# shg8/3DGS.cpp

Hardware: AMD Instinct MI355X
Metric: frames/sec at 1920×1080, 1M Gaussians (higher is better)
Workload: dtype f32

## Files before the change

3dgs.cpp_amd/binding.py:

```python
import ctypes as C
import os

import numpy as np

_HERE = os.path.dirname(os.path.abspath(__file__))
LIB_PATH = os.environ.get("GS3D_HIP_LIB", os.path.join(_HERE, "libgs3d_hip.so"))

UNIFORMS_DT = np.dtype([("camera_position", "<f4", 4), ("proj_mat", "<f4", 16), ("view_mat", "<f4", 16),
                        ("width", "<u4"), ("height", "<u4"), ("tan_fovx", "<f4"), ("tan_fovy", "<f4")])
CAMERA_DT = np.dtype([("position", "<f4", 3), ("rotation", "<f4", 4), ("fov", "<f4"),
                      ("near_plane", "<f4"), ("far_plane", "<f4")])
VERTEX_FLOATS = 60
RECORD_FLOATS = 62
BLOB_PLANES = 59


KERNEL_SOURCES = ("gs_device.h", "gs_bin.h", "gs_scene.hip", "gs_preprocess.hip", "gs_radix.hip", "gs_bin_l1.hip", "gs_bin_l2.hip",
                  "gs_blend.hip", "gs_contrib.hip", "gs_features.hip", "gs_kernels.h")


def library_source_hash():
    import hashlib
    import re
    h = hashlib.sha256()
    for name in KERNEL_SOURCES + ("Makefile",):
        with open(os.path.join(_HERE, "csrc", name), "r") as f:
            text = f.read()
        if name != "Makefile":
            text = re.sub(r"/\*.*?\*/", " ", text, flags=re.S)
            text = re.sub(r"//[^\n]*", " ", text)
        else:
            text = re.sub(r"#[^\n]*", " ", text)
        h.update(name.encode() + b"\0" + " ".join(text.split()).encode())
    return h.hexdigest()


STAGES = dict(tiles=(0, np.uint32), depth=(1, np.float32), radius=(2, np.float32), aabb=(3, np.uint16),
              conic_opacity=(4, np.float32), uv_rg=(5, np.float32), b=(6, np.float32),
              depth_order=(7, np.uint32), alpha_cut=(8, np.float32), sorted_tile=(11, np.uint32), sorted_gid=(12, np.uint32),
              ranges=(13, np.uint32), lists_raw=(14, np.uint32), ranges_raw=(15, np.uint32))

SYMBOLS = ["gs_last_error", "gs_device_count", "gs_read_ply", "gs_activate_records", "gs_scene_load_ply", "gs_scene_from_records",
           "gs_scene_from_vertices", "gs_scene_from_device_blob", "gs_scene_blob_floats", "gs_scene_blob",
           "gs_scene_from_device_arrays", "gs_scene_update_from_device_arrays", "gs_debug_activation_expf_scan",
           "gs_scene_transform", "gs_transform_sh_matrices", "gs_transform_camera",
           "gs_scene_num_vertices", "gs_scene_quantize_sh", "gs_scene_sh_bits", "gs_scene_download_vertex_range",
           "gs_scene_download_vertices", "gs_scene_download_cov3d",
           "gs_deactivate_vertices", "gs_write_ply", "gs_scene_to_device_arrays", "gs_scene_download_records", "gs_scene_save_ply",
           "gs_scene_destroy", "gs_renderer_create", "gs_renderer_destroy", "gs_camera_uniforms",
           "gs_render", "gs_render_host", "gs_synchronize", "gs_set_timing", "gs_set_frames_in_flight", "gs_set_sort_path", "gs_set_exp_mode", "gs_set_graph_mode", "gs_set_blend_lockstep", "gs_get_blend_lockstep", "gs_set_blend_contraction", "gs_set_antialiased", "gs_get_antialiased", "gs_get_timing_totals",
           "gs_get_frame_intervals", "gs_get_stats", "gs_poll_stats", "gs_debug_download", "gs_accumulate_contributions", "gs_blend_features", "gs_debug_expf_scan", "gs_debug_alpha_cut_scan", "gs_renderer_stream",
           "gs_dist_unique_id", "gs_dist_create", "gs_dist_rank", "gs_dist_world", "gs_dist_pose_count",
           "gs_dist_broadcast_scene", "gs_dist_broadcast_scene_ex", "gs_dist_verify", "gs_dist_destroy"]


class FrameStats(C.Structure):
    _fields_ = [("num_gaussians", C.c_uint64), ("num_visible", C.c_uint64), ("num_instances", C.c_uint64),
                ("instance_capacity", C.c_uint64), ("ms_preprocess", C.c_float), ("ms_prefix_sum", C.c_float),
                ("ms_preprocess_sort", C.c_float), ("ms_sort", C.c_float), ("ms_tile_boundary", C.c_float),
                ("ms_render", C.c_float), ("ms_total", C.c_float), ("retries", C.c_uint32),
                ("num_bin_entries", C.c_uint32), ("max_bin_entries", C.c_uint32), ("sort_path", C.c_uint32),
                ("bin_tiles", C.c_uint32), ("sort_level", C.c_uint32), ("blend_redo", C.c_uint32), ("blend_resolved", C.c_uint32), ("pad_", C.c_uint32)]

    def as_dict(self):
        return {k: getattr(self, k) for k, _ in self._fields_}


def debug_alpha_cut_scan(first_bits, count, device=0):
    bad, first = C.c_uint64(0), C.c_uint32(0)
    _check(lib().gs_debug_alpha_cut_scan(C.c_int(device), C.c_uint32(first_bits), C.c_uint64(count), C.byref(bad), C.byref(first)))
    return int(bad.value), (None if bad.value == 0 else int(first.value))


def debug_expf_scan(first_bits, count, device=0):
    blocks = (count + (1 << 20) - 1) >> 20
    sums = np.zeros(blocks, np.uint64)
    guard = np.zeros(4, np.float64)
    _check(lib().gs_debug_expf_scan(C.c_int(device), C.c_uint32(first_bits), C.c_uint64(count), _p(sums), C.c_uint64(blocks), _p(guard)))
    return sums, guard


def debug_activation_expf_scan(first_bits, count, device=0):
    blocks = (count + (1 << 20) - 1) >> 20
    sums = np.zeros(blocks, np.uint64)
    _check(lib().gs_debug_activation_expf_scan(C.c_int(device), C.c_uint32(first_bits), C.c_uint64(count), _p(sums), C.c_uint64(blocks)))
    return sums


class DeviceArrays(C.Structure):
    _fields_ = [("means", C.c_void_p), ("log_scales", C.c_void_p), ("quats", C.c_void_p), ("opacity_logits", C.c_void_p),
                ("sh_dc", C.c_void_p), ("sh_rest", C.c_void_p), ("sh_rest_coeffs", C.c_uint32)]


class Transform(C.Structure):
    _fields_ = [("rotation", C.c_float * 4), ("translation", C.c_float * 3), ("scale", C.c_float)]


def _transform(rotation, translation, scale):
    t = Transform()
    t.rotation[:] = [float(v) for v in rotation]
    t.translation[:] = [float(v) for v in translation]
    t.scale = float(scale)
    return t


def _tensor_rows(name, t, trailing, device):
    if not all(hasattr(t, a) for a in ("data_ptr", "shape", "dtype", "is_contiguous", "device")):
        raise TypeError(f"{name}: a device tensor is needed (data_ptr, shape, dtype, is_contiguous, device), got {type(t).__name__}")
    if str(t.dtype).rsplit(".", 1)[-1] != "float32":
        raise TypeError(f"{name}: dtype must be float32, not {t.dtype}")
    shape = tuple(int(d) for d in t.shape)
    if len(shape) < 1:
        raise ValueError(f"{name}: shape {shape} has no row axis")
    if not t.is_contiguous():
        raise ValueError(f"{name}: the tensor must be contiguous (dense rows); call .contiguous()")
    rows, rest = shape[0], tuple(d for d in shape[1:] if d != 1) if trailing is not None else shape[1:]
    if trailing is None:
        if len(rest) != 2 or rest[1] != 3 or rest[0] not in (0, 3, 8, 15):
            raise ValueError(f"{name}: shape {shape} is not (rows, k, 3) with k in 0, 3, 8, 15")
        rows = (rows, rest[0])
    elif rest != tuple(d for d in trailing if d != 1):
        raise ValueError(f"{name}: shape {shape} is not (rows, {', '.join(map(str, trailing))})")
    dev = t.device
    kind, index = getattr(dev, "type", str(dev).split(":")[0]), getattr(dev, "index", None)
    if kind == "cpu":
        raise ValueError(f"{name}: the tensor is on the CPU; Scene.from_records takes host data")
    if (0 if index is None else int(index)) != int(device):
        raise ValueError(f"{name}: the tensor is on device {index}, the scene on device {device}")
    return rows


def _device_arrays(tensors, device, require):
    trailing = dict(means=(3,), log_scales=(3,), quats=(4,), opacity_logits=(1,), sh_dc=(3,), sh_rest=None)
    a, rows = DeviceArrays(), None
    for name, t in tensors.items():
        if t is None:
            if require and name != "sh_rest":
                raise TypeError(f"{name} is required")
            continue
        r = _tensor_rows(name, t, trailing[name], device)
        if name == "sh_rest":
            r, a.sh_rest_coeffs = r
            if a.sh_rest_coeffs == 0:
                continue
        if rows is not None and r != rows:
            raise ValueError(f"{name} has {r} rows, the arrays before it {rows}")
        rows = r
        setattr(a, name, t.data_ptr() if r else None)
    return a, (rows or 0)


class Contributions(C.Structure):
    _fields_ = [("mask", C.c_void_p), ("weight", C.c_void_p), ("pixels", C.c_void_p), ("top_id", C.c_void_p)]


class FeatureMaps(C.Structure):
    _fields_ = [("features", C.c_void_p), ("channels", C.c_uint32), ("out_features", C.c_void_p), ("out_alpha", C.c_void_p),
                ("out_depth", C.c_void_p), ("out_depth_median", C.c_void_p)]


FEATURE_CHANNELS_MAX = 256


def _tensor_exact(name, t, dtypes, shape, device, owner="Renderer.contributions"):
    if not all(hasattr(t, a) for a in ("data_ptr", "shape", "dtype", "is_contiguous", "device")):
        raise TypeError(f"{name}: a device tensor is needed (data_ptr, shape, dtype, is_contiguous, device), got {type(t).__name__}")
    if str(t.dtype).rsplit(".", 1)[-1] not in dtypes:
        raise TypeError(f"{name}: dtype must be {' or '.join(dtypes)}, not {t.dtype}")
    got = tuple(int(d) for d in t.shape)
    if len(got) != len(shape) or any(w is not None and g != w for g, w in zip(got, shape)):
        raise ValueError(f"{name}: shape {got} is not ({', '.join('?' if w is None else str(w) for w in shape)})")
    if not t.is_contiguous():
        raise ValueError(f"{name}: the tensor must be contiguous; call .contiguous()")
    dev = t.device
    kind, index = getattr(dev, "type", str(dev).split(":")[0]), getattr(dev, "index", None)
    if kind == "cpu":
        raise ValueError(f"{name}: the tensor is on the CPU; the arrays of {owner} live on the renderer's device")
    if (0 if index is None else int(index)) != int(device):
        raise ValueError(f"{name}: the tensor is on device {index}, the renderer on device {device}")
    return t.data_ptr() if all(got) else None


def _stream_handle(stream):
    import sys
    if stream is None:
        torch = sys.modules.get("torch")
        if torch is None or not torch.cuda.is_available():
            return None
        stream = torch.cuda.current_stream()
    return C.c_void_p(int(getattr(stream, "cuda_stream", stream)) or None)


class GsError(RuntimeError):
    def __init__(self, code, msg):
        super().__init__(f"[{code}] {msg}")
        self.code = code


_LIB = None


def lib():
    global _LIB
# ... 179 lines not shown
        return lib().gs_scene_num_vertices(self._h)

    def blob(self):
        p = C.c_void_p()
        n = C.c_uint64()
        _check(lib().gs_scene_blob(self._h, C.byref(p), C.byref(n)))
        return p.value, n.value

    def download_vertices(self):
        out = np.zeros((self.num_vertices, VERTEX_FLOATS), np.float32)
        _check(lib().gs_scene_download_vertices(self._h, _p(out)))
        return out

    def quantize_sh(self):
        _check(lib().gs_scene_quantize_sh(self._h))

    @property
    def sh_bits(self):
        return lib().gs_scene_sh_bits(self._h)

    def download_vertex_range(self, first, count):
        out = np.zeros((count, VERTEX_FLOATS), np.float32)
        _check(lib().gs_scene_download_vertex_range(self._h, C.c_uint64(first), C.c_uint64(count), _p(out)))
        return out

    def download_cov3d(self):
        out = np.zeros((self.num_vertices, 6), np.float32)
        _check(lib().gs_scene_download_cov3d(self._h, _p(out)))
        return out

    def close(self):
        if self._h:
            lib().gs_scene_destroy(self._h)
            self._h = None

    def __del__(self):
        try:
            self.close()
        except Exception:
            pass


class Renderer:

    def __init__(self, scene):
        self.scene = scene
        self._h = C.c_void_p()
        self._frame_hw = None
        _check(lib().gs_renderer_create(scene._h, C.byref(self._h)))

    def render(self, uniforms, rgba_ptr=0, bgra_ptr=0):
        _check(lib().gs_render(self._h, _p(uniforms), C.c_void_p(rgba_ptr), C.c_void_p(bgra_ptr)))
        self._frame_hw = (int(uniforms["height"][0]), int(uniforms["width"][0]))

    def contributions(self, weight=None, pixels=None, top_id=None, mask=None):
        n = int(self.scene.num_vertices)
        h, w = self._frame_hw if self._frame_hw is not None else (None, None)
        dev = self.scene.device
        c = Contributions()
        if weight is not None:
            c.weight = _tensor_exact("weight", weight, ("int64",), (n,), dev)
        if pixels is not None:
            c.pixels = _tensor_exact("pixels", pixels, ("int32",), (n,), dev)
        if top_id is not None:
            c.top_id = _tensor_exact("top_id", top_id, ("int32",), (h, w), dev)
        if mask is not None:
            c.mask = _tensor_exact("mask", mask, ("uint8", "bool"), (h, w), dev)
        _check(lib().gs_accumulate_contributions(self._h, C.byref(c)))

    def feature_maps(self, features=None, out=None, alpha=None, depth=None, median_depth=None):
        owner = "Renderer.feature_maps"
        n = int(self.scene.num_vertices)
        dev = self.scene.device
        asked = dict(out=out, alpha=alpha, depth=depth, median_depth=median_depth)
        if self._frame_hw is None and any(v is True for v in asked.values()):
            _check(lib().gs_blend_features(self._h, C.byref(FeatureMaps())))
        h, w = self._frame_hw if self._frame_hw is not None else (None, None)
        m = FeatureMaps()
        channels = 0
        if features is not None:
            m.features = _tensor_exact("features", features, ("float32",), (n, None), dev, owner)
            channels = int(features.shape[1])
            if channels > FEATURE_CHANNELS_MAX:
                raise ValueError(f"features: {channels} channels, at most {FEATURE_CHANNELS_MAX} are blended in one call")
            if out is None:
                raise ValueError("out: features are given but no output for them (pass a tensor or True)")
        elif out is not None:
            raise ValueError("out: an output for blended features needs features")
        m.channels = channels
        shapes = dict(out=(h, w, channels), alpha=(h, w), depth=(h, w), median_depth=(h, w))
        members = dict(out="out_features", alpha="out_alpha", depth="out_depth", median_depth="out_depth_median")
        result = {}
        for name, t in asked.items():
            if t is None:
                continue
            if t is True:
                import torch
                t = torch.empty(shapes[name], dtype=torch.float32, device=f"cuda:{int(dev)}")
            setattr(m, members[name], _tensor_exact(name, t, ("float32",), shapes[name], dev, owner))
            result[name] = t
        _check(lib().gs_blend_features(self._h, C.byref(m)))
        return result

    def render_host(self, uniforms, want_rgba=True, want_bgra=False):
        h, w = int(uniforms["height"][0]), int(uniforms["width"][0])
        rgba = np.zeros((h, w, 4), np.float32) if want_rgba else None
        bgra = np.zeros((h, w, 4), np.uint8) if want_bgra else None
        _check(lib().gs_render_host(self._h, _p(uniforms), _p(rgba) if want_rgba else None,
                                    _p(bgra) if want_bgra else None))
        self._frame_hw = (h, w)
        return rgba, bgra

    def synchronize(self):
        _check(lib().gs_synchronize(self._h))

    def set_timing(self, enabled):
        _check(lib().gs_set_timing(self._h, C.c_int(int(enabled))))

    def set_frames_in_flight(self, frames):
        _check(lib().gs_set_frames_in_flight(self._h, C.c_int(int(frames))))

    def set_exp_mode(self, mode):
        _check(lib().gs_set_exp_mode(self._h, C.c_int(int(mode))))

    def set_blend_contraction(self, enabled):
        _check(lib().gs_set_blend_contraction(self._h, C.c_int(int(bool(enabled)))))

    def set_antialiased(self, enabled):
        _check(lib().gs_set_antialiased(self._h, C.c_int(int(bool(enabled)))))

    @property
    def antialiased(self):
        rc = lib().gs_get_antialiased(self._h)
        _check(min(rc, 0))
        return bool(rc)

    def set_fast_blend(self, fast):
        self.set_exp_mode(0 if fast else 2)
        self.set_blend_contraction(bool(fast))

    def set_graph_mode(self, enabled):
        _check(lib().gs_set_graph_mode(self._h, C.c_int(int(bool(enabled)))))

    def set_blend_lockstep(self, mode):
        _check(lib().gs_set_blend_lockstep(self._h, C.c_int(int(mode))))

    def blend_lockstep(self):
        settled = C.c_int(0)
        now = lib().gs_get_blend_lockstep(self._h, C.byref(settled))
        if now < 0:
            _check(now)
        return bool(now), bool(settled.value)

    def set_sort_path(self, mode):
        _check(lib().gs_set_sort_path(self._h, C.c_int(int(mode))))

    def timing_totals(self, reset=True):
        st = FrameStats()
        n = C.c_uint64()
        _check(lib().gs_get_timing_totals(self._h, C.byref(st), C.byref(n), C.c_int(int(reset))))
        return st, n.value

    def frame_intervals(self, reset=True, capacity=8192):
        out = np.zeros(capacity, np.float32)
        n = C.c_uint64()
        _check(lib().gs_get_frame_intervals(self._h, _p(out), C.c_uint64(capacity), C.byref(n), C.c_int(int(reset))))
        return out[:min(capacity, n.value)].copy()

    def stats(self):
        st = FrameStats()
        _check(lib().gs_get_stats(self._h, C.byref(st)))
        return st

    def poll_stats(self):
        st = FrameStats()
        n = C.c_uint64()
        _check(lib().gs_poll_stats(self._h, C.byref(st), C.byref(n)))
        return st, n.value

    def stage(self, name, uniforms=None):
        code, dt = STAGES[name]
        st = self.stats()
        n, v, d = st.num_gaussians, st.num_visible, min(st.num_instances, st.instance_capacity)
        count = {"tiles": n, "depth": n, "radius": n, "aabb": 4 * n, "conic_opacity": 4 * n, "uv_rg": 4 * n,
                 "b": n, "alpha_cut": n, "depth_order": v, "sorted_tile": d, "sorted_gid": d, "lists_raw": d}.get(name)
        if name in ("ranges", "ranges_raw"):
            w, h = int(uniforms["width"][0]), int(uniforms["height"][0])
            count = 2 * ((w + 15) // 16) * ((h + 15) // 16)
        out = np.zeros(max(int(count), 1), dt)
        _check(lib().gs_debug_download(self._h, C.c_int(code), _p(out), C.c_uint64(int(count) * out.itemsize)))
        return out[:int(count)]

    @property
    def stream(self):
        return lib().gs_renderer_stream(self._h)

    def close(self):
        if self._h:
            lib().gs_renderer_destroy(self._h)
            self._h = None

    def __del__(self):
        try:
            self.close()
        except Exception:
            pass


class Dist:

    ID_BYTES = 128

    @staticmethod
    def unique_id():
        buf = (C.c_uint8 * Dist.ID_BYTES)()
        _check(lib().gs_dist_unique_id(buf))
        return bytes(buf)

    def __init__(self, unique_id, rank, world, device=0):
        h = C.c_void_p()
        buf = (C.c_uint8 * Dist.ID_BYTES).from_buffer_copy(unique_id)
        _check(lib().gs_dist_create(buf, C.c_int(rank), C.c_int(world), C.c_int(device), C.byref(h)))
        self._h = h
        lib().gs_dist_pose_count.restype = C.c_uint64

    @property
    def rank(self):
        return lib().gs_dist_rank(self._h)

    @property
    def world(self):
        return lib().gs_dist_world(self._h)

    def pose_count(self, poses):
        return int(lib().gs_dist_pose_count(self._h, C.c_uint64(poses)))

    def broadcast_scene(self, scene=None, root=0, copy_on_root=False):
        out = C.c_void_p()
        _check(lib().gs_dist_broadcast_scene_ex(self._h, scene._h if scene is not None else None, C.c_int(root),
                                                C.c_uint(1 if copy_on_root else 0), C.byref(out)))
        if scene is not None and out.value == scene._h.value:
            return scene
        return Scene(out)

    def close(self):
        if self._h:
            lib().gs_dist_destroy(self._h)
            self._h = None

    def __del__(self):
        try:
            self.close()
        except Exception:
            pass
```

3dgs.cpp_amd/csrc/gs_bin_l2.hip:

```cpp
#include "gs_bin.h"

namespace gs {

struct SlabDesc {
    uint32_t off, c_total;
    uint32_t kmin;
    int32_t sh;
    uint32_t b_lo, b_hi;
    uint32_t ready;
    uint32_t pad;
    uint32_t cur[64];
};
static_assert(sizeof(SlabDesc) == 288, "descriptor layout");

struct BuildArgs {
    BinGrid g;
    uint32_t* cand;
    const uint32_t* bin_count;
    const float* depth;
    const ushort4* aabb;
    uint32_t* ranges;
    uint32_t* sorted_gid;
    Counters* counters;
    uint32_t capacity;
    uint32_t cand_capacity;
    SlabDesc* slabs;
    uint32_t slab_capacity;
    uint32_t epoch;
    uint64_t* stamps;
};

__device__ __forceinline__ uint32_t bin_local_box(const BinGrid& g, uint32_t bin, ushort4 box) {
    const int S = 1 << g.bin_shift;
    const int ox = (int)(bin & ((1u << g.grid_shift) - 1u)) << g.bin_shift, oy = (int)(bin >> g.grid_shift) << g.bin_shift;
    const int lx0 = max((int)box.x, ox) - ox, ly0 = max((int)box.y, oy) - oy;
    const int lx1 = min((int)box.z, ox + S) - ox, ly1 = min((int)box.w, oy + S) - oy;
    return (uint32_t)lx0 | ((uint32_t)ly0 << 8) | ((uint32_t)lx1 << 16) | ((uint32_t)ly1 << 24);
}

constexpr int kBuildSlots = 16;

#ifdef GS_BUILD_TIMING
__device__ unsigned long long g_build_t[1024][10];
#define BUILD_ROW(v) uint32_t build_row = (v)
#define BUILD_ROW_SET(v) build_row = (v)
#define BUILD_T(i) do { if (threadIdx.x == 0) g_build_t[build_row][i] = wall_clock64(); } while (0)
#else
#define BUILD_ROW(v) do { } while (0)
#define BUILD_ROW_SET(v) do { } while (0)
#define BUILD_T(i) do { } while (0)
#endif

template <int R2, int THREADS, bool SORT>
struct BuildLayout {
    static constexpr int NW = THREADS / WAVE;
    static constexpr int MAXC = SORT ? THREADS * 16 : 0;
    static constexpr int SS = 64 * R2;
    static constexpr bool CACHE_BOX = SORT && R2 <= 4;
    static constexpr int TABLES = 3 * SS + kBuildSlots * SS / 2 + (SORT ? 0 : kBuildSlots * WAVE);
    static constexpr int WCNT = SORT ? NW * 256 : 0;
    static constexpr int T_OFF = (SORT && (CACHE_BOX || TABLES > MAXC)) ? 2 * MAXC : 0;
    static constexpr int WORDS = (T_OFF + TABLES > 2 * MAXC + WCNT) ? T_OFF + TABLES : 2 * MAXC + WCNT;
};

template <int R2, int THREADS, bool SORT>
__global__ __launch_bounds__(THREADS) void k_bin_build(BuildArgs a) {
    frame_stamp(a.stamps, ST_L2);
    BUILD_ROW(blockIdx.x);
    using L = BuildLayout<R2, THREADS, SORT>;
    constexpr int NW = L::NW, MAXC = L::MAXC, SS = L::SS, PER = kBuildSlots / NW;
    extern __shared__ uint32_t smem[];
    uint32_t* const s_key = smem;
    uint32_t* const s_id = smem + MAXC;
    uint32_t (*const s_wcnt)[256] = reinterpret_cast<uint32_t(*)[256]>(smem + 2 * MAXC);
    uint32_t* const t_cnt = smem + L::T_OFF;
    uint32_t* const t_cur = t_cnt + SS;
    uint16_t (*const r_cnt)[SS] = reinterpret_cast<uint16_t(*)[SS]>(t_cnt + 3 * SS);
    uint32_t* const w_ids = t_cnt + 3 * SS + kBuildSlots * SS / 2;
    __shared__ uint32_t scratch[NW];
    __shared__ uint32_t s_seg;

    const int tid = threadIdx.x, lane = tid & (WAVE - 1), w = tid / WAVE;
    const uint32_t bin = ((blockIdx.x / a.g.bins_x) << a.g.grid_shift) | (blockIdx.x % a.g.bins_x);
    BUILD_T(0);
    uint32_t c, off;
    c = a.bin_count[bin];
    off = a.bin_count[kBinOffsets + bin];
    if ((uint64_t)off + c > a.cand_capacity) c = 0;
    if (SORT && c > (uint32_t)MAXC) {
        if (tid == 0) atomicOr(&a.counters->overflow, 2u);
        c = 0;
    }
    BUILD_T(1);
    if (SORT && c != 0) {
        constexpr int kRounds = 16;
        {
            uint32_t g[kRounds], k[kRounds];
#pragma unroll
            for (int r = 0; r < kRounds; ++r) {
                const uint32_t e = r * THREADS + tid;
                g[r] = e < c ? a.cand[off + e] : 0u;
            }
#pragma unroll
            for (int r = 0; r < kRounds; ++r) {
                const uint32_t e = r * THREADS + tid;
                k[r] = e < c ? __float_as_uint(a.depth[g[r]]) : 0u;
            }
#pragma unroll
            for (int r = 0; r < kRounds; ++r) {
                const uint32_t e = r * THREADS + tid;
                if (e < c) {
                    s_id[e] = g[r];
                    s_key[e] = k[r];
                }
            }
        }
        BUILD_T(2);
        const uint64_t lt_mask = (1ull << lane) - 1ull;
        const int rounds = (int)((c + THREADS - 1) / THREADS);
        const uint32_t wbase = (uint32_t)w * (uint32_t)rounds * WAVE;
#pragma unroll 1
        for (int pass = 0; pass < 4; ++pass) {
            const int shift = pass * 8;
            for (int k = tid; k < NW * 256; k += THREADS) s_wcnt[k >> 8][k & 255] = 0;
            __syncthreads();
            uint32_t key[kRounds], id[kRounds], rank[kRounds];
#pragma unroll
            for (int r = 0; r < kRounds; ++r) {
                key[r] = 0;
                id[r] = 0;
                rank[r] = 0;
                if (r < rounds) {
                    const uint32_t e = wbase + r * WAVE + lane;
                    const bool ok = e < c;
                    if (ok) {
                        key[r] = s_key[e];
                        id[r] = s_id[e];
                    }
                    const uint32_t d = (key[r] >> shift) & 255u;
                    const uint64_t okm = __ballot(ok);
                    uint32_t mlo = (uint32_t)okm, mhi = (uint32_t)(okm >> 32);
#pragma unroll
                    for (int bit = 0; bit < 8; ++bit) {
                        const uint32_t mine = (d >> bit) & 1u;
                        const uint64_t b = __builtin_amdgcn_ballot_w64(mine != 0);
                        const uint32_t splat = 0u - mine;
                        mlo &= ~((uint32_t)b ^ splat);
                        mhi &= ~((uint32_t)(b >> 32) ^ splat);
                    }
                    const uint64_t m = ((uint64_t)mhi << 32) | mlo;
                    uint32_t old = 0;
                    const int leader = m ? (__ffsll((unsigned long long)m) - 1) : 0;
                    if (ok && lane == leader) {
                        old = s_wcnt[w][d];
                        s_wcnt[w][d] = old + (uint32_t)__popcll(m);
                    }
                    old = __shfl(old, leader, WAVE);
                    rank[r] = old + (uint32_t)__popcll(m & lt_mask);
                }
            }
            __syncthreads();
            {
                uint32_t cw[NW], cnt = 0;
                if (tid < 256) {
#pragma unroll
                    for (int k = 0; k < NW; ++k) {
                        cw[k] = s_wcnt[k][tid];
                        cnt += cw[k];
                    }
                }
                uint32_t all;
                uint32_t excl = block_excl_scan<THREADS>(cnt, scratch, &all);
                if (tid < 256) {
#pragma unroll
                    for (int k = 0; k < NW; ++k) {
                        s_wcnt[k][tid] = excl;
                        excl += cw[k];
                    }
                }
            }
            __syncthreads();
#pragma unroll
            for (int r = 0; r < kRounds; ++r) {
                if (r < rounds) {
                    const uint32_t e = wbase + r * WAVE + lane;
                    if (e < c) {
                        const uint32_t d = (key[r] >> shift) & 255u;
                        const uint32_t pos = s_wcnt[w][d] + rank[r];
                        s_key[pos] = key[r];
                        s_id[pos] = id[r];
                    }
                }
            }
            __syncthreads();
        }
        BUILD_T(3);
        if (L::CACHE_BOX) {
            ushort4 box[kRounds];
#pragma unroll
            for (int r = 0; r < kRounds; ++r) {
                const uint32_t e = r * THREADS + tid;
                box[r] = e < c ? a.aabb[s_id[e]] : make_ushort4(0, 0, 0, 0);
            }
#pragma unroll
            for (int r = 0; r < kRounds; ++r) {
                const uint32_t e = r * THREADS + tid;
                if (e < c) s_key[e] = bin_local_box(a.g, bin, box[r]);
            }
        }
    }
    BUILD_T(4);
    for (int t = tid; t < SS; t += THREADS) t_cnt[t] = 0;
    __syncthreads();
    const uint32_t nch = (c + WAVE - 1) / WAVE;
    auto chunk_columns = [&](uint32_t ch, uint64_t (&col)[R2], uint32_t& gid) {
        const uint32_t e = ch * WAVE + lane;
        uint32_t box = 0;
        gid = 0;
        if (e < c) {
            gid = SORT ? s_id[e] : a.cand[off + e];
            box = L::CACHE_BOX ? s_key[e] : bin_local_box(a.g, bin, a.aabb[gid]);
        }
        packed_cover_masks<R2>(a.g.bin_shift, box, col);
#pragma unroll
        for (int r = 0; r < R2; ++r)
            col[r] = (R2 == 1 || __builtin_amdgcn_ballot_w64(col[r] != 0) != 0) ? wave_transpose64(col[r], lane) : 0ull;
    };
    {
        uint32_t acc[R2];
#pragma unroll
        for (int r = 0; r < R2; ++r) acc[r] = 0;
        for (uint32_t ch = w; ch < nch; ch += NW) {
            uint64_t col[R2];
            uint32_t gid;
            chunk_columns(ch, col, gid);
#pragma unroll
            for (int r = 0; r < R2; ++r) acc[r] += (uint32_t)__popcll(col[r]);
        }
#pragma unroll
        for (int r = 0; r < R2; ++r)
            if (acc[r]) atomicAdd(&t_cnt[r * 64 + lane], acc[r]);
    }
    __syncthreads();
    BUILD_T(5);
    {
        uint32_t v[(SS + THREADS - 1) / THREADS], sum = 0;
#pragma unroll
        for (int k = 0; k < (SS + THREADS - 1) / THREADS; ++k) {
            const int t = tid * ((SS + THREADS - 1) / THREADS) + k;
            v[k] = t < SS ? t_cnt[t] : 0u;
            sum += v[k];
        }
        uint32_t d_bin;
        uint32_t excl = block_excl_scan<THREADS>(sum, scratch, &d_bin);
        if (tid == 0) {
            const uint32_t seg = d_bin ? atomicAdd(&a.counters->instances, d_bin) : 0u;
            s_seg = seg;
            if ((uint64_t)seg + d_bin > a.capacity) atomicOr(&a.counters->overflow, 1u);
        }
        __syncthreads();
        const uint32_t S = 1u << a.g.bin_shift;
        const uint32_t ox = (bin & ((1u << a.g.grid_shift) - 1u)) << a.g.bin_shift, oy = (bin >> a.g.grid_shift) << a.g.bin_shift;
#pragma unroll
        for (int k = 0; k < (SS + THREADS - 1) / THREADS; ++k) {
            const int t = tid * ((SS + THREADS - 1) / THREADS) + k;
            if (t < SS) {
                const uint32_t lx = (uint32_t)t & (S - 1), ly = (uint32_t)t >> a.g.bin_shift;
                const uint32_t x = ox + lx, y = oy + ly;
                const uint64_t start64 = (uint64_t)s_seg + excl;
                const uint32_t start = start64 > a.capacity ? a.capacity : (uint32_t)start64;
                const uint32_t end = start64 + v[k] > a.capacity ? a.capacity : (uint32_t)(start64 + v[k]);
                if (ly < S && x < a.g.tiles_x && y < a.g.tiles_y) {
                    a.ranges[2 * (y * a.g.tiles_x + x)] = v[k] ? start : 0u;
                    a.ranges[2 * (y * a.g.tiles_x + x) + 1] = v[k] ? end : 0u;
                }
                t_cur[t] = start;
            }
            excl += v[k];
        }
    }
    __syncthreads();
    BUILD_T(6);
    const __amdgpu_buffer_rsrc_t out = __builtin_amdgcn_make_buffer_rsrc(a.sorted_gid, 0, a.capacity * 4u, 0x27000);
    int par = 0;
    for (uint32_t rb = 0; rb < nch; rb += kBuildSlots, par ^= 1) {
        uint64_t col[PER][R2];
#pragma unroll
        for (int j = 0; j < PER; ++j) {
            const int slot = w * PER + j;
            uint32_t gid;
            chunk_columns(rb + slot, col[j], gid);
#pragma unroll
            for (int r = 0; r < R2; ++r) r_cnt[slot][r * 64 + lane] = (uint16_t)__popcll(col[j][r]);
            if (!SORT) w_ids[slot * WAVE + lane] = gid;
        }
        __syncthreads();
        for (int t = tid; t < SS; t += THREADS) {
            uint32_t run = 0;
#pragma unroll
            for (int k = 0; k < kBuildSlots; ++k) {
                const uint32_t v = r_cnt[k][t];
                r_cnt[k][t] = (uint16_t)run;
                run += v;
            }
            t_cur[(par ^ 1) * SS + t] = t_cur[par * SS + t] + run;
        }
        __syncthreads();
#pragma unroll
        for (int j = 0; j < PER; ++j) {
            const int slot = w * PER + j;
            const uint32_t ch = rb + slot;
            const uint32_t* ids = SORT ? s_id + (ch < nch ? ch : 0u) * WAVE : w_ids + slot * WAVE;
#pragma unroll
            for (int r = 0; r < R2; ++r) {
                if (__builtin_amdgcn_ballot_w64(col[j][r] != 0) == 0) continue;
                walk_column(col[j][r], t_cur[par * SS + r * 64 + lane] + r_cnt[slot][r * 64 + lane], out, ids);
            }
        }
    }
    BUILD_T(7);
}

#ifdef GS_BUILD_TIMING
extern "C" int gs_debug_build_timing(unsigned long long* out ) {
    return hipMemcpyFromSymbol(out, HIP_SYMBOL(g_build_t), sizeof(unsigned long long) * 1024 * 10) == hipSuccess ? 0 : -1;
}
#endif

__device__ __forceinline__ __amdgpu_buffer_rsrc_t uniform_rsrc(const void* p, uint32_t bytes) {
    const uint64_t addr = reinterpret_cast<uint64_t>(p);
    const uint32_t lo = (uint32_t)__builtin_amdgcn_readfirstlane((int)(uint32_t)addr);
    const uint32_t hi = (uint32_t)__builtin_amdgcn_readfirstlane((int)(uint32_t)(addr >> 32));
    return __builtin_amdgcn_make_buffer_rsrc(reinterpret_cast<void*>(((uint64_t)hi << 32) | lo), 0,
                                             __builtin_amdgcn_readfirstlane((int)bytes), 0x27000);
}

__device__ __forceinline__ uint32_t cover16(uint32_t pb) {
    const uint32_t lx0 = pb & 15u, ly0 = (pb >> 4) & 15u, lx1 = (pb >> 8) & 15u, ly1 = (pb >> 12) & 15u;
    const uint32_t xm = ((2u << lx1) - (1u << lx0)) & 15u;
    const uint32_t rows = (16u << (4u * ly1)) - (1u << (4u * ly0));
    return (xm * 0x1111u) & rows;
}

template <int ROUNDS>
struct FastLayout {
    static constexpr int THREADS = 1024, NW = THREADS / WAVE, MAXC = THREADS * ROUNDS;
    static constexpr int WCNT_WORDS = NW * 512 / 2;
    static constexpr int MISC_WORDS = 64 + 64 + NW * 64;
    static constexpr int TAIL = WCNT_WORDS > MISC_WORDS ? WCNT_WORDS : MISC_WORDS;
    static constexpr int WORDS = 2 * MAXC + TAIL;
};

template <int ROUNDS, int MODE = 0>
__device__ __forceinline__ void bin_fast_body(const BuildArgs& a) {
    constexpr bool SLABS = MODE != 0;
    using L = FastLayout<ROUNDS>;
    constexpr int THREADS = L::THREADS, NW = L::NW, MAXC = L::MAXC;
    extern __shared__ uint32_t smem[];
    uint32_t* const s_pay = smem;
    uint32_t* const s_key = smem + MAXC;
    uint16_t (*const s_wcnt)[512] = reinterpret_cast<uint16_t(*)[512]>(smem + 2 * MAXC);
    uint32_t* const s_id = smem + MAXC;
    uint16_t* const s_box = reinterpret_cast<uint16_t*>(smem);
    uint16_t (*const s_tbl)[64] = reinterpret_cast<uint16_t(*)[64]>(smem + MAXC / 2);
    uint32_t* const t_cnt = smem + 2 * MAXC;
    uint32_t* const t_cur = t_cnt + 64;
    uint32_t (*const s_seg)[64] = reinterpret_cast<uint32_t(*)[64]>(t_cnt + 128);
    __shared__ uint32_t scratch[NW], scratch_hi[NW];
    __shared__ uint32_t s_seg0, s_flag;
    constexpr int kSlotBits = SLABS ? 16 : 14;
    constexpr uint32_t kSlotMask = (1u << kSlotBits) - 1u;
    constexpr uint32_t kMaxInBin = SLABS ? 65535u : (uint32_t)MAXC;
    constexpr int kMaxSlabs = 16;
    __shared__ uint32_t g_cur[SLABS ? 64 : 1], t_tot[SLABS ? 64 : 1];
    __shared__ uint32_t slab_first[SLABS ? kMaxSlabs + 1 : 1];
    __shared__ uint32_t cnt2[(MODE == 1 || MODE == 3) ? kMaxSlabs : 1][64];
    __shared__ uint32_t s_fill;
    __shared__ uint16_t q_order[MODE == 3 ? 1024 : 1];
    __shared__ uint32_t q_item, q_planned;

    BUILD_ROW(MODE == 2 ? 1023u : blockIdx.x);
    if constexpr (MODE != 2) frame_stamp(a.stamps, ST_L2);
    int tid = threadIdx.x, lane = tid & (WAVE - 1), w = tid / WAVE;
    auto screen_bin = [&](uint32_t i) { return ((i / a.g.bins_x) << a.g.grid_shift) | (i % a.g.bins_x); };
    uint32_t bin = screen_bin(MODE == 3 ? 0u : blockIdx.x);
    bool slab_item = MODE == 2;
    BUILD_T(0);
    uint32_t c_total = 0, off = 0;
    auto bin_extent = [&]() {
        c_total = (uint32_t)__builtin_amdgcn_readfirstlane((int)a.bin_count[bin]);
        off = (uint32_t)__builtin_amdgcn_readfirstlane((int)a.bin_count[kBinOffsets + bin]);
        if ((uint64_t)off + c_total > a.cand_capacity) c_total = 0;
        if (c_total > kMaxInBin) {
            if (tid == 0) atomicOr(&a.counters->overflow, 2u);
            c_total = 0;
        }
    };
    if constexpr (MODE == 0 || MODE == 1) bin_extent();
    if (tid == 0) s_flag = 0;
    BUILD_T(1);
#define multi (MODE == 2 ? true : (MODE == 1 ? c_total > (uint32_t)MAXC : (MODE == 3 ? (slab_item || c_total > (uint32_t)MAXC) : false)))
    uint32_t c = multi ? 0u : c_total;
    int rounds = (int)((c + THREADS - 1) / THREADS);
    typedef uint32_t u32x3 __attribute__((ext_vector_type(3)));
#define recs uniform_rsrc(a.cand + (size_t)kCandWords * off, c_total * 12u)
    uint64_t lt_mask = (1ull << lane) - 1ull;
    uint32_t wbase = (uint32_t)w * (uint32_t)rounds * WAVE;
    auto refresh = [&]() {
        int t = threadIdx.x;
        asm volatile("" : "+v"(t));
        tid = t;
        lane = t & (WAVE - 1);
        w = t / WAVE;
        lt_mask = (1ull << lane) - 1ull;
        wbase = (uint32_t)w * (uint32_t)rounds * WAVE;
    };
    auto radix_pass = [&](int shift, int db, uint32_t sub) {
        const uint32_t dmask = (1u << db) - 1u;
        for (int k = tid; k < NW * 512 / 2; k += THREADS) reinterpret_cast<uint32_t*>(&s_wcnt[0][0])[k] = 0;
        __syncthreads();
        uint32_t key[ROUNDS], pay[ROUNDS], rank[ROUNDS];
#pragma unroll
        for (int r = 0; r < ROUNDS; ++r) {
            key[r] = 0;
            pay[r] = 0;
            rank[r] = 0;
            if (r < rounds) {
                const uint32_t e = wbase + r * WAVE + lane;
                const bool ok = e < c;
                if (ok) {
                    key[r] = s_key[e] - sub;
                    pay[r] = s_pay[e];
                }
                const uint32_t d = (key[r] >> shift) & dmask;
                const uint64_t okm = __ballot(ok);
                uint32_t mlo = (uint32_t)okm, mhi = (uint32_t)(okm >> 32);
#pragma unroll
                for (int bit = 0; bit < 9; ++bit) {
                    if (bit < db) {
                        const uint32_t mine = (d >> bit) & 1u;
                        const uint64_t b = __builtin_amdgcn_ballot_w64(mine != 0);
                        const uint32_t splat = 0u - mine;
                        mlo &= ~((uint32_t)b ^ splat);
                        mhi &= ~((uint32_t)(b >> 32) ^ splat);
                    }
                }
                const uint64_t m = ((uint64_t)mhi << 32) | mlo;
                uint32_t old = 0;
                const int leader = m ? (__ffsll((unsigned long long)m) - 1) : 0;
                if (ok && lane == leader) {
                    old = s_wcnt[w][d];
                    s_wcnt[w][d] = (uint16_t)(old + (uint32_t)__popcll(m));
                }
                old = __shfl(old, leader, WAVE);
                rank[r] = old + (uint32_t)__popcll(m & lt_mask);
            }
        }
        __syncthreads();
        {
            uint32_t cw[NW], cnt = 0;
            if (tid < 512) {
#pragma unroll
                for (int k = 0; k < NW; ++k) {
                    cw[k] = s_wcnt[k][tid];
                    cnt += cw[k];
                }
            }
            uint32_t all;
            uint32_t excl = block_excl_scan<THREADS>(cnt, scratch, &all);
            if (tid < 512) {
#pragma unroll
                for (int k = 0; k < NW; ++k) {
                    s_wcnt[k][tid] = (uint16_t)excl;
                    excl += cw[k];
                }
            }
        }
        __syncthreads();
#pragma unroll
        for (int r = 0; r < ROUNDS; ++r) {
            if (r < rounds) {
                const uint32_t e = wbase + r * WAVE + lane;
                if (e < c) {
                    const uint32_t d = (key[r] >> shift) & dmask;
                    const uint32_t pos = (uint32_t)s_wcnt[w][d] + rank[r];
                    s_key[pos] = key[r];
                    s_pay[pos] = pay[r];
                }
            }
        }
        __syncthreads();
    };
    auto block_minmax = [&](uint32_t lo, uint32_t hi, uint32_t& kmin, uint32_t& span) {
#pragma unroll
        for (int d = 1; d < WAVE; d <<= 1) {
            lo = min(lo, (uint32_t)__shfl_xor((int)lo, d, WAVE));
            hi = max(hi, (uint32_t)__shfl_xor((int)hi, d, WAVE));
        }
        __syncthreads();
        if (lane == 0) {
            scratch[w] = lo;
            scratch_hi[w] = hi;
        }
        __syncthreads();
#pragma unroll
        for (int k = 0; k < NW; ++k) {
            lo = min(lo, scratch[k]);
            hi = max(hi, scratch_hi[k]);
        }
        kmin = (uint32_t)__builtin_amdgcn_readfirstlane((int)lo);
        span = (uint32_t)__builtin_amdgcn_readfirstlane((int)hi) - kmin;
    };
    auto key_range = [&](uint32_t& kmin, uint32_t& span) {
        uint32_t lo = 0xFFFFFFFFu, hi = 0u;
#pragma unroll
        for (int r = 0; r < ROUNDS; ++r) {
            const uint32_t e = r * THREADS + tid;
            if (r < rounds && e < c) {
                const uint32_t k = s_key[e];
                lo = min(lo, k);
                hi = max(hi, k);
            }
        }
        block_minmax(lo, hi, kmin, span);
    };
    auto sort_by_key_lsd = [&](uint32_t kmin, uint32_t span) {
        const int bits = span ? 32 - __builtin_clz(span) : 0;
        const int npass = (bits + 8) / 9;
        const int db = npass ? (bits + npass - 1) / npass : 0;
#pragma unroll 1
        for (int pass = 0; pass < npass; ++pass) radix_pass(pass * db, db, pass == 0 ? kmin : 0u);
        return npass ? kmin : 0u;
    };
    constexpr uint32_t kMsdBuckets = 4096, kMsdBucketMax = 64;
    uint32_t* const m_cnt = smem + 2 * MAXC;
    uint16_t* const m_start = reinterpret_cast<uint16_t*>(smem + 2 * MAXC + kMsdBuckets / 2);
    static_assert(kMsdBuckets * 4 <= L::TAIL * 4, "the bucket tables live in the counters' area");
    auto sort_by_key_msd = [&](uint32_t kmin, uint32_t span) -> bool {
        const int bits = 32 - __builtin_clz(span);
        const int sh = bits > 12 ? bits - 12 : 0;
        for (uint32_t k = tid; k < kMsdBuckets / 2; k += THREADS) m_cnt[k] = 0;
        __syncthreads();
        uint32_t key[ROUNDS], pay[ROUNDS];
#pragma unroll
// ... 391 lines not shown
                        s_pay[j] = vp;
                    }
                }
            }
            __syncthreads();
            break;
        }
        const uint32_t id_base = sort_by_key(false);
        uint32_t nk[ROUNDS], ni[ROUNDS], nb[ROUNDS];
#pragma unroll
        for (int r = 0; r < ROUNDS; ++r) {
            const uint32_t e = r * THREADS + tid;
            nk[r] = ni[r] = nb[r] = 0;
            if (r < rounds && e < c) {
                const uint32_t pw = s_pay[e];
                nk[r] = __builtin_amdgcn_raw_buffer_load_b32(recs, (pw & kSlotMask) * 12u, 0, 0);
                ni[r] = s_id[e] + id_base;
                nb[r] = pw >> kSlotBits;
            }
        }
        __syncthreads();
#pragma unroll
        for (int r = 0; r < ROUNDS; ++r) {
            const uint32_t e = r * THREADS + tid;
            if (r < rounds && e < c) {
                u32x3 rec = {nk[r], ni[r], nb[r]};
                __builtin_amdgcn_raw_buffer_store_b96(rec, recs, e * 12u, 0, 0);
            }
        }
        __threadfence_block();
        if (tid == 0) s_flag = 0;
        __syncthreads();
    }
#undef recs
    BUILD_T(3);
    refresh();
    const uint32_t nch = (c + WAVE - 1) / WAVE;
    {
        uint32_t pb16[ROUNDS];
#pragma unroll
        for (int r = 0; r < ROUNDS; ++r) {
            const uint32_t e = r * THREADS + tid;
            pb16[r] = e < c ? s_pay[e] >> kSlotBits : 0u;
        }
        __syncthreads();
        for (uint32_t k = tid; k < (uint32_t)MAXC / 2; k += THREADS) smem[MAXC / 2 + k] = 0;
        if (tid < 64) t_cnt[tid] = 0;
        __syncthreads();
#pragma unroll
        for (int r = 0; r < ROUNDS; ++r) {
            const uint32_t e = r * THREADS + tid;
            const uint32_t pb = pb16[r];
            if (e < c) s_box[e] = (uint16_t)pb;
            if (S == 4) {
                const uint32_t ch = (uint32_t)r * NW + (uint32_t)__builtin_amdgcn_readfirstlane(w);
                if (ch < nch) {
                    const uint32_t cm = e < c ? cover16(pb) : 0u;
                    uint32_t mine = 0;
#pragma unroll
                    for (int t = 0; t < 16; ++t) {
                        const uint64_t bal = __builtin_amdgcn_ballot_w64(((cm >> t) & 1u) != 0);
                        mine = lane == t ? (uint32_t)__popcll(bal) : mine;
                    }
                    s_tbl[ch][lane] = (uint16_t)mine;
                }
            }
        }
        if (S != 4) {
            __syncthreads();
            for (uint32_t ch = w; ch < nch; ch += NW) {
                const uint32_t e = ch * WAVE + lane;
                const uint32_t pb = e < c ? (uint32_t)s_box[e] : 0xFFFFu;
                uint64_t m[1];
                cover_masks<1>(3, (int)(pb & 15u), (int)((pb >> 4) & 15u), (int)((pb >> 8) & 15u) + 1, (int)(pb >> 12) + 1, m);
                if (e >= c) m[0] = 0;
                s_tbl[ch][lane] = (uint16_t)__popcll(wave_transpose64(m[0], lane));
            }
        }
    }
    __syncthreads();
    BUILD_T(4);
    {
        const int t = tid & 63, g = tid >> 6;
        const uint32_t per = (nch + NW - 1) / NW;
        const uint32_t q0 = min(nch, (uint32_t)g * per), q1 = min(nch, q0 + per);
        uint32_t sum = 0;
        for (uint32_t q = q0; q < q1; ++q) sum += s_tbl[q][t];
        s_seg[g][t] = sum;
        __syncthreads();
        if (tid < 64) {
            uint32_t run = 0;
#pragma unroll
            for (int k = 0; k < NW; ++k) {
                const uint32_t v = s_seg[k][tid];
                s_seg[k][tid] = run;
                run += v;
            }
            t_cnt[tid] = run;
        }
        __syncthreads();
        uint32_t run = s_seg[g][t];
        for (uint32_t q = q0; q < q1; ++q) {
            const uint32_t v = s_tbl[q][t];
            s_tbl[q][t] = (uint16_t)run;
            run += v;
        }
    }
    __syncthreads();
    BUILD_T(5);
    if (!multi) {
        place_lists(tid < 64 ? t_cnt[tid] : 0u, t_cur);
    } else if (tid < 64) {
        t_cur[tid] = g_cur[tid];
    }
    __syncthreads();
    BUILD_T(6);
    refresh();
    const __amdgpu_buffer_rsrc_t out = __builtin_amdgcn_make_buffer_rsrc(a.sorted_gid, 0, a.capacity * 4u, 0x27000);
    for (uint32_t ch = w; ch < nch; ch += NW) {
        const uint32_t e = ch * WAVE + lane;
        const bool valid = e < c;
        const uint32_t id = valid ? s_id[e] : 0u;
        const uint32_t pb = valid ? (uint32_t)s_box[e] : 0u;
        const int lx0 = (int)(pb & 15u), ly0 = (int)((pb >> 4) & 15u), lx1 = (int)((pb >> 8) & 15u), ly1 = (int)(pb >> 12);
        const uint32_t base = t_cur[lane] + (uint32_t)s_tbl[ch][lane];
        if (S == 4) {
            const uint32_t cm = valid ? cover16(pb) : 0u;
#pragma unroll
            for (int t = 0; t < 16; ++t) {
                const bool covered = ((cm >> t) & 1u) != 0;
                const uint64_t bal = __builtin_amdgcn_ballot_w64(covered);
                if (bal == 0) continue;
                const uint32_t rank = __builtin_amdgcn_mbcnt_hi((uint32_t)(bal >> 32), __builtin_amdgcn_mbcnt_lo((uint32_t)bal, 0u));
                const uint32_t pos = (uint32_t)__builtin_amdgcn_readlane((int)base, t) + rank;
                __builtin_amdgcn_raw_buffer_store_b32(id, out, covered ? pos * 4u : 0xFFFFFFFFu, 0, 0);
            }
        } else {
            uint64_t m[1];
            cover_masks<1>(3, lx0, ly0, lx1 + 1, ly1 + 1, m);
            if (!valid) m[0] = 0;
            walk_column(wave_transpose64(m[0], lane), base, out, s_id + ch * WAVE);
        }
    }
    if (multi && tid < 64) g_cur[tid] += t_cnt[tid];
    };
    if constexpr (MODE == 0) {
        slab_body(0u);
    } else if constexpr (MODE == 1) {
        if (n_slabs != 0) slab_body(0u);
    } else if constexpr (MODE == 3) {
        const uint32_t n_bins = a.g.bins_x * a.g.bins_y;
        {
            uint32_t* const cnt = smem;
            const uint32_t mine = (uint32_t)tid < n_bins ? a.bin_count[screen_bin((uint32_t)tid)] : 0u;
            cnt[tid] = mine;
            if (tid == 0) q_planned = 0;
            __syncthreads();
            if (mine > (uint32_t)MAXC) atomicAdd(&q_planned, 1u);
            if ((uint32_t)tid < n_bins) {
                uint32_t before = 0;
                for (uint32_t j = 0; j < n_bins; ++j) {
                    const uint32_t v = cnt[j];
                    before += (v > mine || (v == mine && j < (uint32_t)tid)) ? 1u : 0u;
                }
                q_order[before] = (uint16_t)tid;
            }
            __syncthreads();
        }
        const uint32_t n_planned = (uint32_t)__builtin_amdgcn_readfirstlane((int)q_planned);
        for (;;) {
            __syncthreads();
            refresh();
            if (tid == 0) {
                q_item = atomicAdd(&a.counters->q_head, 1u);
                s_flag = 0;
            }
            __syncthreads();
            const uint32_t item = (uint32_t)__builtin_amdgcn_readfirstlane((int)q_item);
            if (item < n_bins) {
                slab_item = false;
                bin = screen_bin((uint32_t)q_order[item]);
                bin_extent();
                c = multi ? 0u : c_total;
                rounds = (int)((c + THREADS - 1) / THREADS);
                wbase = (uint32_t)w * (uint32_t)rounds * WAVE;
                n_slabs = 1;
                g_kmin = 0;
                g_sh = 0;
                plan_bin();
            } else {
            const uint32_t d = item - n_bins;
            if (tid == 0) {
                uint32_t have = 0;
                if (d < a.slab_capacity) {
                    for (uint32_t spin = 0;; ++spin) {
                        if (__hip_atomic_load(&a.slabs[d].ready, __ATOMIC_RELAXED, __HIP_MEMORY_SCOPE_AGENT) == a.epoch) {
                            have = 1;
                            break;
                        }
                        if (__hip_atomic_load(&a.counters->q_bins_done, __ATOMIC_RELAXED, __HIP_MEMORY_SCOPE_AGENT) >= n_planned) {
                            asm volatile("s_waitcnt vmcnt(0)" ::: "memory");
                            have = __hip_atomic_load(&a.slabs[d].ready, __ATOMIC_RELAXED, __HIP_MEMORY_SCOPE_AGENT) == a.epoch ? 1u : 0u;
                            if (!have && d < min(__hip_atomic_load(&a.counters->slabs, __ATOMIC_RELAXED, __HIP_MEMORY_SCOPE_AGENT), a.slab_capacity) &&
                                !(__hip_atomic_load(&a.counters->overflow, __ATOMIC_RELAXED, __HIP_MEMORY_SCOPE_AGENT) & 2u))
                                atomicOr(&a.counters->overflow, 2u);
                            break;
                        }
                        if (spin > (1u << 20)) {
                            atomicOr(&a.counters->overflow, 2u);
                            break;
                        }
                        __builtin_amdgcn_s_sleep(64);
                    }
                }
                q_item = have;
            }
            __syncthreads();
            if (__builtin_amdgcn_readfirstlane((int)q_item) == 0) break;
            SlabDesc* desc = a.slabs + d;
            slab_item = true;
            auto get = [&](uint32_t* p) { return __hip_atomic_load(p, __ATOMIC_RELAXED, __HIP_MEMORY_SCOPE_AGENT); };
            off = (uint32_t)__builtin_amdgcn_readfirstlane((int)get(&desc->off));
            c_total = (uint32_t)__builtin_amdgcn_readfirstlane((int)get(&desc->c_total));
            g_kmin = (uint32_t)__builtin_amdgcn_readfirstlane((int)get(&desc->kmin));
            g_sh = __builtin_amdgcn_readfirstlane((int)get(reinterpret_cast<uint32_t*>(&desc->sh)));
            if (tid < 64) g_cur[tid] = get(&desc->cur[tid]);
            if (tid == 0) {
                slab_first[0] = get(&desc->b_lo);
                slab_first[1] = get(&desc->b_hi);
            }
            __syncthreads();
            c = 0;
            n_slabs = 1;
            }
            if (!slab_item && item < n_planned) {
                __syncthreads();
                if (tid == 0) __hip_atomic_fetch_add(&a.counters->q_bins_done, 1u, __ATOMIC_RELAXED, __HIP_MEMORY_SCOPE_AGENT);
            }
            if (n_slabs != 0) slab_body(0u);
        }
    } else {
        const uint32_t n_desc = min(a.counters->slabs, a.slab_capacity);
        for (uint32_t d = blockIdx.x; d < n_desc; d += gridDim.x) {
            const SlabDesc* desc = a.slabs + d;
            __syncthreads();
            refresh();
            off = (uint32_t)__builtin_amdgcn_readfirstlane((int)desc->off);
            c_total = (uint32_t)__builtin_amdgcn_readfirstlane((int)desc->c_total);
            g_kmin = (uint32_t)__builtin_amdgcn_readfirstlane((int)desc->kmin);
            g_sh = __builtin_amdgcn_readfirstlane(desc->sh);
            if (tid < 64) g_cur[tid] = desc->cur[tid];
            if (tid == 0) {
                slab_first[0] = desc->b_lo;
                slab_first[1] = desc->b_hi;
                s_flag = 0;
            }
            __syncthreads();
            BUILD_ROW_SET(512u + (d & 511u));
            BUILD_T(1);
            slab_body(0u);
            BUILD_T(7);
        }
        BUILD_ROW_SET(1023u);
    }
    BUILD_T(7);
}
#undef multi
template <int ROUNDS> __global__ void k_bin_fast(BuildArgs a);
template <> __global__ __launch_bounds__(1024, 4) void k_bin_fast<4>(BuildArgs a) { bin_fast_body<4>(a); }
template <> __global__ __launch_bounds__(1024, 4) void k_bin_fast<8>(BuildArgs a) { bin_fast_body<8>(a); }
template <> __global__ __launch_bounds__(1024, 4) void k_bin_fast<12>(BuildArgs a) { bin_fast_body<12>(a); }
template <> __global__ __launch_bounds__(1024, 4) void k_bin_fast<16>(BuildArgs a) { bin_fast_body<16>(a); }
constexpr int kSlabRounds = 12;
__global__ __launch_bounds__(1024, 4) void k_bin_slabs(BuildArgs a) { bin_fast_body<kSlabRounds, 1>(a); }
__global__ __launch_bounds__(1024, 4) void k_slab_work(BuildArgs a) { bin_fast_body<kSlabRounds, 2>(a); }
__global__ __launch_bounds__(1024, 4) void k_bin_queue(BuildArgs a) { bin_fast_body<kSlabRounds, 3>(a); }

template <int R2, int THREADS, bool SORT>
static hipError_t build_prepare() {
    return hipFuncSetAttribute(reinterpret_cast<const void*>(&k_bin_build<R2, THREADS, SORT>),
                               hipFuncAttributeMaxDynamicSharedMemorySize,
                               (int)(BuildLayout<R2, THREADS, SORT>::WORDS * sizeof(uint32_t)));
}
template <int ROUNDS>
static hipError_t fast_prepare() {
    return hipFuncSetAttribute(reinterpret_cast<const void*>(&k_bin_fast<ROUNDS>), hipFuncAttributeMaxDynamicSharedMemorySize,
                               (int)(FastLayout<ROUNDS>::WORDS * sizeof(uint32_t)));
}
void bin_debug_occupancy() {
    int n4 = -1, n8 = -1, n16 = -1;
    (void)hipOccupancyMaxActiveBlocksPerMultiprocessor(&n4, reinterpret_cast<const void*>(&k_bin_fast<4>), 1024,
                                                       FastLayout<4>::WORDS * sizeof(uint32_t));
    (void)hipOccupancyMaxActiveBlocksPerMultiprocessor(&n8, reinterpret_cast<const void*>(&k_bin_fast<8>), 1024,
                                                       FastLayout<8>::WORDS * sizeof(uint32_t));
    (void)hipOccupancyMaxActiveBlocksPerMultiprocessor(&n16, reinterpret_cast<const void*>(&k_bin_fast<16>), 1024,
                                                       FastLayout<16>::WORDS * sizeof(uint32_t));
    hipFuncAttributes a4{}, a8{};
    (void)hipFuncGetAttributes(&a4, reinterpret_cast<const void*>(&k_bin_fast<4>));
    (void)hipFuncGetAttributes(&a8, reinterpret_cast<const void*>(&k_bin_fast<8>));
    std::fprintf(stderr, "[occupancy] k_bin_fast<4>: %d blocks/CU (regs %d, static lds %zu, dyn %zu); <8>: %d (regs %d); <16>: %d\n", n4,
                 a4.numRegs, a4.sharedSizeBytes, FastLayout<4>::WORDS * sizeof(uint32_t), n8, a8.numRegs, n16);
}

hipError_t bin_prepare_device() {
    hipError_t e = build_prepare<4, 1024, true>();
    if (e == hipSuccess) e = build_prepare<16, 1024, true>();
    if (e == hipSuccess) e = fast_prepare<8>();
    if (e == hipSuccess) e = fast_prepare<12>();
    if (e == hipSuccess) e = fast_prepare<16>();
    if (e == hipSuccess)
        e = hipFuncSetAttribute(reinterpret_cast<const void*>(&k_bin_slabs), hipFuncAttributeMaxDynamicSharedMemorySize,
                                (int)(FastLayout<kSlabRounds>::WORDS * sizeof(uint32_t)));
    if (e == hipSuccess)
        e = hipFuncSetAttribute(reinterpret_cast<const void*>(&k_slab_work), hipFuncAttributeMaxDynamicSharedMemorySize,
                                (int)(FastLayout<kSlabRounds>::WORDS * sizeof(uint32_t)));
    if (e == hipSuccess)
        e = hipFuncSetAttribute(reinterpret_cast<const void*>(&k_bin_queue), hipFuncAttributeMaxDynamicSharedMemorySize,
                                (int)(FastLayout<kSlabRounds>::WORDS * sizeof(uint32_t)));
    return e;
}

template <int R2>
static void launch_build(const BuildArgs& a, bool sort, uint32_t bins, hipStream_t s) {
    constexpr size_t lds1 = BuildLayout<R2, 1024, true>::WORDS * sizeof(uint32_t);
    constexpr size_t lds2 = BuildLayout<R2, 1024, false>::WORDS * sizeof(uint32_t);
    if (sort) hipLaunchKernelGGL((k_bin_build<R2, 1024, true>), dim3(bins), dim3(1024), lds1, s, a);
    else hipLaunchKernelGGL((k_bin_build<R2, 1024, false>), dim3(bins), dim3(1024), lds2, s, a);
}

void launch_bin_level2(const BinLaunch& b, int level, hipStream_t s) {
    BuildArgs a;
    a.g = BinGrid{b.tiles_x, b.tiles_y, b.bins_x, b.bins_y, b.bin_shift, b.grid_shift};
    a.cand = b.cand;
    a.bin_count = b.bin_count;
    a.depth = b.depth;
    a.aabb = b.aabb;
    a.ranges = b.ranges;
    a.sorted_gid = b.sorted_gid;
    a.counters = b.counters;
    a.capacity = b.capacity;
    a.cand_capacity = b.cand_capacity;
    a.slabs = reinterpret_cast<SlabDesc*>(b.slabs);
    a.slab_capacity = b.slab_capacity;
    a.epoch = b.slab_epoch;
    a.stamps = b.stamps;
    const uint32_t bins = b.bins_x * b.bins_y;
    const bool sort = level < kBinSortLevels;
    if (sort && b.bin_shift <= 3) {
        if (level == 0) hipLaunchKernelGGL(k_bin_fast<4>, dim3(bins), dim3(1024), FastLayout<4>::WORDS * sizeof(uint32_t), s, a);
        else if (level == 1) hipLaunchKernelGGL(k_bin_fast<8>, dim3(bins), dim3(1024), FastLayout<8>::WORDS * sizeof(uint32_t), s, a);
        else if (level == 2) hipLaunchKernelGGL(k_bin_fast<12>, dim3(bins), dim3(1024), FastLayout<12>::WORDS * sizeof(uint32_t), s, a);
        else if (level == 3) hipLaunchKernelGGL(k_bin_fast<16>, dim3(bins), dim3(1024), FastLayout<16>::WORDS * sizeof(uint32_t), s, a);
        else if (b.slab_epoch != 0) {
            hipLaunchKernelGGL(k_bin_queue, dim3(bins < kQueueWorkGroups ? bins : kQueueWorkGroups), dim3(1024), FastLayout<kSlabRounds>::WORDS * sizeof(uint32_t), s, a);
        } else {
            hipLaunchKernelGGL(k_bin_slabs, dim3(bins), dim3(1024), FastLayout<kSlabRounds>::WORDS * sizeof(uint32_t), s, a);
            hipLaunchKernelGGL(k_slab_work, dim3(kSlabWorkGroups), dim3(1024), FastLayout<kSlabRounds>::WORDS * sizeof(uint32_t), s, a);
        }
    } else if (b.bin_shift <= 3) {
        launch_build<1>(a, sort, bins, s);
    } else if (b.bin_shift == 4) {
        launch_build<4>(a, sort, bins, s);
    } else {
        launch_build<16>(a, sort, bins, s);
    }
}
}
```

3dgs.cpp_amd/csrc/gs_blend.hip:

```cpp
#include "gs_device.h"

namespace gs {



#if defined(GS_BLEND_STATS) || defined(GS_BLEND_CLOCK)
__device__ unsigned long long g_blend_stats[12];
constexpr uint32_t kClockSlots = 1u << 18;
__device__ uint2 g_blend_clock[kClockSlots];
#endif
#ifdef GS_BLEND_STATS
#define STAT_ADD(i, v) do { const unsigned long long v_ = (unsigned long long)(v); const bool first_ = (__ffsll((unsigned long long)__ballot(true)) - 1) == lane; if (first_) atomicAdd(&g_blend_stats[i], v_); } while (0)
#else
#define STAT_ADD(i, v) do { } while (0)
#endif

struct BlendEntry {
    float4 co;
    float4 uv;
    float4 bc;
};

__device__ __forceinline__ void blend_fetch(BlendEntry& e, uint32_t g, const AttrRecord* __restrict__ rec) {
    const AttrRecord* r = rec + g;
// ... 371 lines not shown
            float power;
            if (CONTRACT) {
                const float s = __builtin_fmaf(co.z * dy, dy, co.x * dx * dx);
                power = __builtin_fmaf(co.y * dx, dy, s);
            } else {
                const float s = co.x * dx * dx + co.z * dy * dy;
                power = s + co.y * dx * dy;
            }
            const uint64_t m2 = alive & __builtin_amdgcn_ballot_w64(power <= 0.0f) &
                                __builtin_amdgcn_ballot_w64(!(power < bp.y));
            if (m2 != 0) {
                STAT_ADD(4, 1);
                STAT_ADD(5, __popcll(m2));
                const float ex = EXP == 1   ? __builtin_amdgcn_exp2f(power * 1.44269502162933349609375f)
                                 : EXP == 2 ? gs_expf_libm(power, exptab)
                                            : gs_exp_blend(power);
                const float alpha = fminf(0.99f, co.w * ex);
                const float test_T = T * (1 - alpha);
                const uint64_t mk = m2 & __builtin_amdgcn_ballot_w64(test_T < 0.0001f);
                STAT_ADD(8, __popcll(m2 & ~mk));
                STAT_ADD(7, (unsigned long long)__popcll(mk) * ((base - range.x) + (uint32_t)k + 1u));
                const bool upd = __builtin_amdgcn_inverse_ballot_w64(m2 & ~mk);
                if (upd) {
                    if (CONTRACT) {
                        c0 = __builtin_fmaf(uv.z * alpha, T, c0);
                        c1 = __builtin_fmaf(uv.w * alpha, T, c1);
                        c2 = __builtin_fmaf(bp.x * alpha, T, c2);
                    } else {
                        c0 = c0 + uv.z * alpha * T;
                        c1 = c1 + uv.w * alpha * T;
                        c2 = c2 + bp.x * alpha * T;
                    }
                    T = test_T;
                }
                asm volatile("s_andn2_b64 %0, %0, %2\n\ts_cmp_eq_u64 %0, 0\n\ts_cselect_b64 %1, 0, %1" : "+s"(alive), "+s"(bm) : "s"(mk) : "scc");
            }
        }
        }
        if (alive == 0) break;
        if (GUARD) {
            S += __builtin_fmaf(T_cs * 1.00001f, __builtin_amdgcn_rcpf(T), -1.0f);
            T_cs = T;
        }
    }
    STAT_ADD(7, (unsigned long long)__popcll(alive) * (range.y - range.x));
    return !abandon;
}

template <int EXP, bool CONTRACT, bool GUARD>
__global__ __launch_bounds__(BLOCK) __attribute__((amdgpu_waves_per_eu(8, 8))) void k_blend(const uint2* __restrict__ ranges,
                                                 const uint32_t* __restrict__ sorted_gid,
                                                 const uint32_t* __restrict__ tile_order,
                                                 const AttrRecord* __restrict__ rec,
                                                 uint32_t width, uint32_t height, uint32_t tiles_x,
                                                 float4* __restrict__ rgba, uchar4* __restrict__ bgra,
                                                 Counters* __restrict__ counters, Counters* host_counters,
                                                 const FrameParams* __restrict__ fp, uint32_t* __restrict__ vis_count, uint32_t lockstep,
                                                 uint64_t* __restrict__ stamps) {
    frame_stamp(stamps, ST_BLEND);
#if defined(GS_BLEND_STATS) || defined(GS_BLEND_CLOCK)
    const long long stat_c0 = clock64();
    const unsigned long long stat_w0 = wall_clock64();
#endif
    static_assert(!GUARD || (EXP != 2 && !CONTRACT), "the guard belongs to a fast exp on the uncontracted arithmetic");
    if (fp) host_counters = fp->host_counters;
    __shared__ float4 s_rec[4][3][WAVE];
    __shared__ uint2 s_exptab[(EXP == 2 || GUARD) ? 4 : 1][32];
    __shared__ uint32_t s_klist[GUARD ? 4 : 1][GUARD ? kGuardList : 1];

    const int tid = threadIdx.x, lane = tid & (WAVE - 1), w = tid / WAVE;
    if (EXP == 2) {
        if (lane < 32) {
            const uint64_t v = kExpfTab[lane];
            s_exptab[w][lane] = make_uint2((uint32_t)v, (uint32_t)(v >> 32));
        }
        __builtin_amdgcn_wave_barrier();
    }
    if (host_counters && blockIdx.x == 0 && tid == 0) *host_counters = *counters;
    if (vis_count && blockIdx.x == 0 && (uint32_t)tid < kVisRegions) {
        vis_count[(uint32_t)tid * kVisCounterStride + 1] = vis_count[(uint32_t)tid * kVisCounterStride];
        vis_count[(uint32_t)tid * kVisCounterStride] = 0;
    }
    const uint32_t tile = tile_order[blockIdx.x];
    const uint32_t tile_x = tile % tiles_x, tile_y = tile / tiles_x;
    const uint32_t qx0 = tile_x * kTile + (w & 1) * 8, qy0 = tile_y * kTile + (w >> 1) * 8;
    const uint32_t px = qx0 + (lane & 7), py = qy0 + (lane >> 3);
    const bool inside = px < width && py < height;
    const float fx = (float)px, fy = (float)py;
    const float rx0 = (float)qx0, ry0 = (float)qy0, rx1 = (float)qx0 + 7.0f, ry1 = (float)qy0 + 7.0f;

    const uint2 range = ranges[tile];
    float c0 = 0.0f, c1 = 0.0f, c2 = 0.0f;
    const uint64_t alive = __builtin_amdgcn_ballot_w64(inside);

    if (alive != 0 && range.x < range.y) {
        uint32_t resolved = 0, unused;
        bool table_ready = EXP == 2;
        const bool done = blend_walk<EXP, CONTRACT, GUARD>(range, sorted_gid, rec, s_rec[w], s_exptab[(EXP == 2 || GUARD) ? w : 0],
                                                           s_klist[GUARD ? w : 0], lane, fx, fy, rx0, rx1, ry0, ry1, alive, c0, c1, c2, resolved,
                                                           table_ready, lockstep != 0);
        if (GUARD && resolved != 0 && lane == 0) atomicAdd(&counters->blend_resolved, resolved);
        if (GUARD && !done) {
            if (!table_ready) {
                if (lane < 32) {
                    const uint64_t v = kExpfTab[lane];
                    s_exptab[w][lane] = make_uint2((uint32_t)v, (uint32_t)(v >> 32));
                }
                __builtin_amdgcn_wave_barrier();
                table_ready = true;
            }
            if (lane == 0) atomicAdd(&counters->blend_redo, 1u);
            uint2 range_again = range;
            asm volatile("" : "+s"(range_again.x), "+s"(range_again.y));
            (void)blend_walk<2, false, false>(range_again, sorted_gid, rec, s_rec[w], s_exptab[w], nullptr, lane, fx, fy, rx0, rx1, ry0, ry1, alive, c0, c1,
                                              c2, unused, table_ready, false);
        }
    }
#if defined(GS_BLEND_STATS) || defined(GS_BLEND_CLOCK)
    {
        const uint32_t slot = blockIdx.x * (BLOCK / WAVE) + threadIdx.x / WAVE;
        if ((threadIdx.x & (WAVE - 1)) == 0 && slot < kClockSlots)
            g_blend_clock[slot] = make_uint2((uint32_t)(clock64() - stat_c0), (uint32_t)(wall_clock64() - stat_w0));
    }
#endif
    if (fp) {
        rgba = reinterpret_cast<float4*>(fp->rgba);
        bgra = reinterpret_cast<uchar4*>(fp->bgra);
    }
    float fx_end = fx, fy_end = fy;
    asm volatile("" : "+v"(fx_end), "+v"(fy_end));
    const uint32_t px_end = (uint32_t)fx_end, py_end = (uint32_t)fy_end;
    if (px_end < width && py_end < height) {
        const size_t p = (size_t)py_end * width + px_end;
        if (rgba) rgba[p] = make_float4(c0, c1, c2, 1.0f);
        if (bgra) {
            const float r = fminf(fmaxf(c0, 0.0f), 1.0f), g = fminf(fmaxf(c1, 0.0f), 1.0f),
                        b = fminf(fmaxf(c2, 0.0f), 1.0f);
            bgra[p] = make_uchar4((unsigned char)(int)__builtin_rintf(b * 255.0f),
                                  (unsigned char)(int)__builtin_rintf(g * 255.0f),
                                  (unsigned char)(int)__builtin_rintf(r * 255.0f), 255);
        }
    }
}

template <int EXP, bool CONTRACT, bool GUARD>
static void launch_blend_as(const uint32_t* ranges, const uint32_t* sorted_gid, const uint32_t* tile_order, const AttrView& av,
                            uint32_t width, uint32_t height, uint32_t tx, uint32_t ty, float* rgba, uint8_t* bgra,
                            Counters* counters, Counters* host_counters, const FrameParams* fp, bool lockstep, uint64_t* stamps, hipStream_t s) {
    hipLaunchKernelGGL((k_blend<EXP, CONTRACT, GUARD>), dim3(tx * ty), dim3(BLOCK), 0, s, reinterpret_cast<const uint2*>(ranges),
                       sorted_gid, tile_order, av.rec, width, height, tx, reinterpret_cast<float4*>(rgba),
                       reinterpret_cast<uchar4*>(bgra), counters, host_counters, fp, av.vis_count, lockstep ? 1u : 0u, stamps);
}

__global__ __launch_bounds__(WAVE) void k_frame_end(uint64_t* __restrict__ stamps, uint64_t* host_stamps, const FrameParams* __restrict__ fp) {
    if (fp) host_stamps = fp->host_stamps;
    const uint64_t now = wall_clock64();
    const int t = threadIdx.x;
    if (t < ST_COUNT) {
        const uint64_t v = t == ST_END ? now : stamps[t];
        if (t == ST_END) stamps[t] = now;
        if (host_stamps) host_stamps[t] = v;
    }
}
void launch_frame_end(uint64_t* stamps, uint64_t* host_stamps, const FrameParams* fp, hipStream_t s) {
    if (!stamps) return;
    hipLaunchKernelGGL(k_frame_end, dim3(1), dim3(WAVE), 0, s, stamps, host_stamps, fp);
}

void launch_blend(const uint32_t* ranges, const uint32_t* sorted_gid, const uint32_t* tile_order, const AttrView& av,
                  uint32_t width,
                  uint32_t height, float* rgba, uint8_t* bgra, Counters* counters,
                  Counters* host_counters, int exp_mode, bool contract, const FrameParams* fp, bool lockstep, uint64_t* stamps, hipStream_t s) {
    if (width == 0 || height == 0) return;
    const uint32_t tx = (width + kTile - 1) / kTile, ty = (height + kTile - 1) / kTile;
    if (exp_mode == 3 && !contract)
        return launch_blend_as<1, false, true>(ranges, sorted_gid, tile_order, av, width, height, tx, ty, rgba, bgra, counters,
                                               host_counters, fp, lockstep, stamps, s);
    if (exp_mode == 3) exp_mode = 1;
#define GS_BLEND_CASE(E, C)                                                                                              \
    if (exp_mode == E && contract == C)                                                                                  \
        return launch_blend_as<E, C, false>(ranges, sorted_gid, tile_order, av, width, height, tx, ty, rgba, bgra,       \
                                            counters, host_counters, fp, lockstep, stamps, s)
    GS_BLEND_CASE(0, true);
    GS_BLEND_CASE(0, false);
    GS_BLEND_CASE(1, true);
    GS_BLEND_CASE(1, false);
    GS_BLEND_CASE(2, true);
    GS_BLEND_CASE(2, false);
#undef GS_BLEND_CASE
}


__global__ __launch_bounds__(BLOCK) void k_expf_scan(uint32_t first_bits, uint64_t count, unsigned long long* __restrict__ block_sums,
                                                     unsigned long long* __restrict__ guard_max ) {
    const uint64_t base = (uint64_t)blockIdx.x << 20;
    unsigned long long sum = 0;
    double worst = 0.0, worst_near = 0.0;
    for (uint32_t j = threadIdx.x; j < (1u << 20); j += BLOCK) {
        const uint64_t at = base + j;
        if (at >= count) break;
        const uint32_t xb = first_bits + (uint32_t)at;
        const float x = __uint_as_float(xb);
        const float y = gs_expf_libm_full(x, reinterpret_cast<const uint2*>(kExpfTab));
        sum += (unsigned long long)__float_as_uint(y) * (unsigned long long)((xb * 0x9E3779B1u) | 1u);
        if (x >= -16.0f && x <= 0.0f) {
            const float fast = __builtin_amdgcn_exp2f(x * 1.44269502162933349609375f);
            const double rel = fabs((double)fast - (double)y) / (double)y;
            worst = fmax(worst, rel - (double)kGuardE1 * fabs((double)x));
            if (x >= -1.0f) worst_near = fmax(worst_near, rel);
        }
    }
    for (int d = 32; d >= 1; d >>= 1) {
        sum += __shfl_xor(sum, d, WAVE);
        worst = fmax(worst, __shfl_xor(worst, d, WAVE));
        worst_near = fmax(worst_near, __shfl_xor(worst_near, d, WAVE));
    }
    if ((threadIdx.x & (WAVE - 1)) == 0) {
        atomicAdd(&block_sums[blockIdx.x], sum);
        atomicMax(&guard_max[0], (unsigned long long)__double_as_longlong(worst));
        atomicMax(&guard_max[1], (unsigned long long)__double_as_longlong(worst_near));
    }
}

extern "C" int gs_debug_expf_scan(int device, uint32_t first_bits, uint64_t count, uint64_t* block_sums, uint64_t blocks_capacity,
                                  double* guard ) {
    const uint64_t blocks = (count + (1u << 20) - 1) >> 20;
    if (blocks == 0 || blocks > blocks_capacity || !block_sums || blocks > 0x7FFFFFFFull) return GS_ERR_INVALID;
    if (hipSetDevice(device) != hipSuccess) return GS_ERR_DEVICE;
    unsigned long long* d = nullptr;
    if (hipMalloc(reinterpret_cast<void**>(&d), (blocks + 2) * sizeof(unsigned long long)) != hipSuccess) return GS_ERR_NOMEM;
    int rc = GS_OK;
    if (hipMemset(d, 0, (blocks + 2) * sizeof(unsigned long long)) != hipSuccess) rc = GS_ERR_DEVICE;
    if (rc == GS_OK) {
        hipLaunchKernelGGL(k_expf_scan, dim3((uint32_t)blocks), dim3(BLOCK), 0, nullptr, first_bits, count, d, d + blocks);
        if (hipGetLastError() != hipSuccess || hipDeviceSynchronize() != hipSuccess) rc = GS_ERR_DEVICE;
    }
    unsigned long long g[2] = {0, 0};
    if (rc == GS_OK && (hipMemcpy(block_sums, d, blocks * sizeof(unsigned long long), hipMemcpyDeviceToHost) != hipSuccess ||
                        hipMemcpy(g, d + blocks, sizeof g, hipMemcpyDeviceToHost) != hipSuccess))
        rc = GS_ERR_DEVICE;
    (void)hipFree(d);
    if (rc == GS_OK && guard) {
        guard[0] = __builtin_bit_cast(double, g[0]);
        guard[1] = __builtin_bit_cast(double, g[1]);
        guard[2] = (double)kGuardE0;
        guard[3] = (double)kGuardE1;
    }
    return rc;
}

#if defined(GS_BLEND_STATS) || defined(GS_BLEND_CLOCK)
extern "C" int gs_debug_blend_stats(unsigned long long* out, int reset) {
    unsigned long long z[12] = {0, 0, 0, 0, 0, 0, 0, 0, 0, 0, 0, 0};
    if (hipMemcpyFromSymbol(out, HIP_SYMBOL(g_blend_stats), sizeof z) != hipSuccess) return -1;
    if (reset && hipMemcpyToSymbol(HIP_SYMBOL(g_blend_stats), z, sizeof z) != hipSuccess) return -1;
    return 0;
}
extern "C" int gs_debug_blend_clock(unsigned long long* out, unsigned waves) {
    if (waves > kClockSlots) waves = kClockSlots;
    uint2* h = new uint2[waves];
    const hipError_t e = hipMemcpyFromSymbol(h, HIP_SYMBOL(g_blend_clock), sizeof(uint2) * waves);
    out[0] = out[1] = 0;
    for (unsigned i = 0; e == hipSuccess && i < waves; ++i) {
        out[0] += h[i].x;
        out[1] += h[i].y;
    }
    delete[] h;
    return e == hipSuccess ? 0 : -1;
}
#endif

}
```

3dgs.cpp_amd/csrc/gs_depth_policy.h:

```cpp
#pragma once

#include <algorithm>
#include <cstdint>

#include "gs_levels.h"

namespace gs_host {

inline uint32_t tiles_across(uint32_t pixels) { return (pixels + gs::kTile - 1) / gs::kTile; }

struct BinGeometry {
    int bin_shift, grid_shift;
    uint32_t bins_x, bins_y;
};

struct DepthPolicy {
    static constexpr int kGlobalLevel = gs::kBinSortLevels;
    static constexpr int kOneSizeShift = 4;
    static uint32_t level_limit(int lv) { return gs::kBinSortLimit[lv]; }

    int sort_mode = 0;
    int level = 0;
    uint32_t frames_since_fallback = 0;
    uint32_t slab_hold = 32, slab_clean_frames = 0;
    int min_bin_shift = 3;
    bool refined = false;
    bool settle_level = false;

    int frame_level() const { return sort_mode == 1 ? kGlobalLevel : level; }
    void set_sort_mode(int mode) {
        sort_mode = mode;
        level = 0;
        refined = false;
        frames_since_fallback = 0;
    }

    static bool grid_fits(uint32_t tx, uint32_t ty, int s) { return (((tx - 1) >> s) + 1) <= 32 && (((ty - 1) >> s) + 1) <= 32; }
    static int base_shift(uint32_t tx, uint32_t ty, int min_shift) {
        int s = std::max(2, min_shift);
        while (!grid_fits(tx, ty, s)) ++s;
        return s;
    }
    int bin_shift(uint32_t tx, uint32_t ty) const {
        int s = base_shift(tx, ty, min_bin_shift);
        if (refined && s > 2 && grid_fits(tx, ty, s - 1)) --s;
        return s;
    }
    bool bin_geometry(uint32_t tx, uint32_t ty, BinGeometry* g) const {
        if (base_shift(tx, ty, min_bin_shift) > 5) return false;
        const int s = bin_shift(tx, ty);
        g->bin_shift = s;
        g->bins_x = ((tx - 1) >> s) + 1;
        g->bins_y = ((ty - 1) >> s) + 1;
        g->grid_shift = (g->bins_x <= 16 && g->bins_y <= 16) ? 4 : 5;
        return true;
    }
    bool can_refine(uint32_t width, uint32_t height) const {
        const uint32_t tx = tiles_across(width), ty = tiles_across(height);
        const int s = base_shift(tx, ty, min_bin_shift);
        return !refined && s > 2 && s <= 5 && grid_fits(tx, ty, s - 1);
    }

    struct QueuedFrame {
        int level, bin_shift;
        uint32_t width, height;
        uint32_t overflow;
        uint32_t max_bin;
    };
    enum Verdict { kRerun = 0, kBinTooFull, kDepthsTooCrowded };
    Verdict frames_overflowed(const QueuedFrame* frames, int count) {
        bool bin_too_big = false;
        uint32_t fullest = 0;
        for (int k = 0; k < count; ++k) {
            const QueuedFrame& q = frames[k];
            const bool current = q.level == frame_level() && q.bin_shift == bin_shift(tiles_across(q.width), tiles_across(q.height));
            if (q.level < kGlobalLevel && (q.overflow & 2u) && current) bin_too_big = true;
            if (current) fullest = std::max(fullest, q.max_bin);
        }
        if (!bin_too_big) return kRerun;
        const int failed_level = frames[0].level;
        const bool one_size = frames[0].bin_shift >= kOneSizeShift;
        const bool slabs_unsuitable = !one_size && failed_level == gs::kBinSlabLevel && fullest <= level_limit(gs::kBinSlabLevel);
        if (slabs_unsuitable) {
            slab_hold = std::min<uint32_t>(slab_hold * 2, 8192);
            slab_clean_frames = 0;
        }
        int wanted = failed_level + 1;
        while (wanted < kGlobalLevel && fullest > level_limit(wanted)) ++wanted;
        if (one_size) wanted = kGlobalLevel;
        if (wanted >= gs::kBinSlabLevel && can_refine(frames[0].width, frames[0].height)) {
            refined = true;
            wanted = gs::kBinSlabLevel - 1;
            settle_level = true;
        } else {
            if (sort_mode == 2 && wanted >= kGlobalLevel) return slabs_unsuitable ? kDepthsTooCrowded : kBinTooFull;
            level = std::max(level, wanted);
        }
        if (refined) level = std::max(level, wanted);
        frames_since_fallback = 0;
        return kRerun;
    }

    void frame_retired(int ran_level, uint32_t max_bin, int ran_bin_shift = 3) {
        if (ran_level == gs::kBinSlabLevel && ++slab_clean_frames >= 64) slab_hold = 32;
        if (settle_level && sort_mode != 1 && ran_level == level && level < kGlobalLevel) {
            while (level > 0 && max_bin <= level_limit(level - 1) * 7 / 8) --level;
            frames_since_fallback = 0;
            settle_level = false;
        }
        if (sort_mode != 1 && level > 0) {
            const bool no_slabs_below = level == kGlobalLevel && ran_bin_shift >= kOneSizeShift;
            if (max_bin <= level_limit(no_slabs_below ? gs::kBinSlabLevel - 1 : level - 1) * 7 / 8) {
                if (++frames_since_fallback >= (level == kGlobalLevel ? slab_hold : 32u)) {
                    --level;
                    frames_since_fallback = 0;
                }
            } else {
                frames_since_fallback = 0;
            }
        } else if (sort_mode != 1 && refined) {
            if (max_bin <= level_limit(0) / 2) {
                if (++frames_since_fallback >= 32) {
                    refined = false;
                    level = gs::kBinSlabLevel - 1;
                    frames_since_fallback = 0;
                }
            } else {
                frames_since_fallback = 0;
            }
        }
    }
};

}
```

3dgs.cpp_amd/csrc/gs_kernels.h:

```cpp
#pragma once
#include <hip/hip_runtime.h>
#include <stdint.h>

#include "../../include/gs3d_hip.h"
#include "gs_levels.h"

namespace gs {

constexpr int kSortTileKeys = 2048;
constexpr int kSortMaxBlocks = 1024;

enum ScenePlane { P_POS = 0, P_SCALE = 3, P_ROT = 6, P_OPACITY = 10, P_SH = 11, P_COUNT = 59 };
constexpr uint64_t blob_stride(uint64_t n) { return (n + 15) & ~uint64_t(15); }
constexpr uint64_t blob_floats(uint64_t n) { return P_SH * blob_stride(n) + 48 * n; }

struct SceneView {
    const float* blob;
    const float* cov3d;
    uint32_t n;
    uint32_t stride;
    const uint16_t* sh16;
    const float* acut;
    const uint32_t* perm;
};

struct AttrRecord {
    float4 conic_op;
    float4 uv_rg;
    float4 b_cut_r;
    float4 depth_radius;
};
static_assert(sizeof(AttrRecord) == 64, "one line per Gaussian");

struct AttrView {
    uint32_t* tiles;
    float* depth;
    ushort4* aabb;
    AttrRecord* rec;
    uint4* vis;
    uint32_t* vis_count;
    uint32_t vis_region_slots;
};
constexpr uint32_t kVisRegions = 256, kVisCounterStride = 32;
uint32_t vis_region_slots(uint32_t n);

struct Counters {
    uint32_t visible;
    uint32_t instances;
    uint32_t overflow;
    uint32_t bin_entries;
    uint32_t max_bin;
    uint32_t slabs;
    uint32_t blend_resolved;
    uint32_t blend_redo;
    uint32_t q_head, q_bins_done;
};
enum FrameStamp { ST_PREPROCESS = 0, ST_ORDER = 1, ST_L1_COUNT = 2, ST_L1_SCATTER = 3, ST_L2 = 4, ST_BLEND = 5, ST_END = 6, ST_COUNT = 8 };

struct FrameParams {
    gs_uniforms u;
    float* rgba;
    uint8_t* bgra;
    Counters* host_counters;
    uint64_t* host_stamps;
};

constexpr int kBinSortMax = 16384;
constexpr uint32_t kSlabDescBytes = 288, kSlabCapacity = 8192, kSlabWorkGroups = 512, kQueueWorkGroups = 256;

void launch_cov3d(const float* blob, float* cov3d, uint32_t n, uint32_t stride, uint32_t first, uint32_t count, hipStream_t s);
void launch_alpha_cut(const float* blob, float* cut, uint32_t n, uint32_t stride, uint32_t* beyond_unit, hipStream_t s);
void launch_permute_blob(const float* src, const uint32_t* perm, float* dst, uint32_t n, uint32_t stride, hipStream_t s);
void launch_blob_checksum(const float* blob, uint64_t floats, uint64_t* out, hipStream_t s);
void launch_sh_to_half(const float* blob, uint16_t* sh16, uint32_t stride, uint32_t first, uint32_t count, hipStream_t s);
void launch_ingest_arrays(const gs_device_arrays& a, float* blob, uint32_t stride, uint32_t first, uint32_t count, bool replace_rest,
                          hipStream_t s);
struct SceneTransform {
    float R[9];
    float t[3];
    float s;
    float q[4];
    float M[9 + 25 + 49];
};
void launch_scene_transform(const SceneTransform& x, float* blob, uint32_t stride, uint32_t first, uint32_t count, hipStream_t s);
void launch_scene_export(const gs_device_arrays_out& a, const float* blob, uint32_t stride, uint32_t first, uint32_t count, hipStream_t s);
void launch_scene_export_records(float* records, const float* blob, uint32_t stride, uint32_t first, uint32_t count, hipStream_t s);
void launch_preprocess(const SceneView& sv, const gs_uniforms& u, const AttrView& av, Counters* counters,
                       const FrameParams* fp, uint64_t* stamps, bool antialiased, hipStream_t s);
void launch_frame_end(uint64_t* stamps, uint64_t* host_stamps, const FrameParams* fp, hipStream_t s);

struct RadixPass {
    const uint32_t* keys_in;
    const uint32_t* vals_in;
    uint32_t* keys_out;
    uint32_t* vals_out;
    const uint32_t* n_in;
    uint32_t n_static;
    const uint32_t* tiles;
    uint32_t* n_out;
    uint32_t* block_hist;
    uint32_t* digit_total;
    int shift;
    int bits;
    int blocks;
    int first;
    uint64_t* stamps;
};
void launch_radix_pass(const RadixPass& p, hipStream_t s);

struct BinLaunch {
    const uint32_t* order;
    const uint32_t* n_items;
    uint32_t n_bound;
    const uint32_t* tiles;
    const ushort4* aabb;
    const float* depth;
    const uint4* vis;
    uint32_t* vis_count;
    uint32_t vis_region_slots;
    uint32_t* hist;
    uint32_t* bin_count;
    uint32_t* cand;
    uint32_t* ranges;
    uint32_t* sorted_gid;
    Counters* counters;
    uint32_t capacity;
    uint32_t cand_capacity;
    void* slabs;
    uint32_t slab_capacity;
    uint32_t slab_epoch;
    uint32_t tiles_x, tiles_y, bins_x, bins_y;
    int bin_shift;
    int grid_shift;
    uint64_t* stamps;
};
void launch_vis_to_planes(const AttrView& av, uint32_t n, hipStream_t s);
uint32_t bin_level1_blocks(uint32_t n_items);
uint32_t bin_level1_columns(uint32_t n_items);
void bin_debug_occupancy();
hipError_t bin_prepare_device();
void launch_bin_level1_count(const BinLaunch& b, hipStream_t s);
void launch_bin_level1_scatter(const BinLaunch& b, bool any_order, hipStream_t s);
void launch_bin_level2(const BinLaunch& b, int level, hipStream_t s);

void launch_blend(const uint32_t* ranges, const uint32_t* sorted_gid, const uint32_t* tile_order, const AttrView& av,
                  uint32_t width,
                  uint32_t height, float* rgba, uint8_t* bgra, Counters* counters,
                  Counters* host_counters ,
                  int exp_mode ,
                  bool contract ,
                  const FrameParams* fp,
                  bool lockstep ,
                  uint64_t* stamps ,
                  hipStream_t s);

void launch_contributions(const uint32_t* ranges, const uint32_t* sorted_gid, const uint32_t* tile_order, const AttrRecord* rec,
                          uint32_t width, uint32_t height, const uint8_t* mask, uint64_t* weight, uint32_t* pixels, uint32_t* top_id,
                          hipStream_t s);

constexpr int kFeatureGroup = 16;
void launch_features(const uint32_t* ranges, const uint32_t* sorted_gid, const uint32_t* tile_order, const AttrRecord* rec,
                     uint32_t width, uint32_t height, const float* features, uint32_t channels, float* out_features, float* out_alpha,
                     float* out_depth, float* out_median, hipStream_t s);

}
```

3dgs.cpp_amd/csrc/gs_preprocess.hip:

```cpp
#include "gs_device.h"

namespace gs {

constexpr float SH_C0 = 0.28209479177387814f;
constexpr float SH_C1 = 0.4886025119029199f;

__device__ __forceinline__ float ndc2pix(float v, int S) { return ((v + 1.0f) * (float)S - 1.0f) * 0.5f; }

struct PreUniforms {
    gs_uniforms u;
    Counters* counters;
    const FrameParams* fp;
    uint64_t* stamps;
};

constexpr int kPrePlane = 68, kPreStage = 4 * kPrePlane + 16;
constexpr int kPreShHalf = 32;
constexpr int kPreWaveLds = kPreShHalf * 12 + 4;
static_assert(kPreWaveLds >= kPreStage, "the record stage must fit the wave's LDS slab");

template <class SH>
__device__ __forceinline__ void sh_to_rgb(const SH& S, float x, float y, float z, float (&rgb)[3]) {
    const float C2_0 = 1.0925484305920792f, C2_1 = -1.0925484305920792f, C2_2 = 0.31539156525252005f,
                C2_3 = -1.0925484305920792f, C2_4 = 0.5462742152960396f;
    const float C3_0 = -0.5900435899266435f, C3_1 = 2.890611442640554f, C3_2 = -0.4570457994644658f,
                C3_3 = 0.3731763325901154f, C3_4 = -0.4570457994644658f, C3_5 = 1.445305721320277f,
                C3_6 = -0.5900435899266435f;
    float c[3];
#define GS_SH_FENCE() asm volatile("" : "+v"(c[0]), "+v"(c[1]), "+v"(c[2]) :: "memory")
#pragma unroll
    for (int k = 0; k < 3; ++k) c[k] = SH_C0 * S(0, k);
#pragma unroll
    for (int k = 0; k < 3; ++k) c[k] -= SH_C1 * S(1, k) * y;
#pragma unroll
    for (int k = 0; k < 3; ++k) c[k] += SH_C1 * S(2, k) * z;
#pragma unroll
    for (int k = 0; k < 3; ++k) c[k] -= SH_C1 * S(3, k) * x;
    GS_SH_FENCE();
#pragma unroll
    for (int k = 0; k < 3; ++k) c[k] += C2_0 * S(4, k) * x * y;
#pragma unroll
    for (int k = 0; k < 3; ++k) c[k] += C2_1 * S(5, k) * y * z;
#pragma unroll
    for (int k = 0; k < 3; ++k) c[k] += C2_2 * S(6, k) * (2.0f * z * z - x * x - y * y);
#pragma unroll
    for (int k = 0; k < 3; ++k) c[k] += C2_3 * S(7, k) * z * x;
    GS_SH_FENCE();
#pragma unroll
    for (int k = 0; k < 3; ++k) c[k] += C2_4 * S(8, k) * (x * x - y * y);
#pragma unroll
    for (int k = 0; k < 3; ++k) c[k] += C3_0 * S(9, k) * (3.0f * x * x - y * y) * y;
#pragma unroll
    for (int k = 0; k < 3; ++k) c[k] += C3_1 * S(10, k) * x * y * z;
#pragma unroll
    for (int k = 0; k < 3; ++k) c[k] += C3_2 * S(11, k) * (4.0f * z * z - x * x - y * y) * y;
    GS_SH_FENCE();
#pragma unroll
    for (int k = 0; k < 3; ++k) c[k] += C3_3 * S(12, k) * z * (2.0f * z * z - 3.0f * x * x - 3.0f * y * y);
#pragma unroll
    for (int k = 0; k < 3; ++k) c[k] += C3_4 * S(13, k) * x * (4.0f * z * z - x * x - y * y);
#pragma unroll
    for (int k = 0; k < 3; ++k) c[k] += C3_5 * S(14, k) * (x * x - y * y) * z;
#pragma unroll
    for (int k = 0; k < 3; ++k) c[k] += C3_6 * S(15, k) * x * (x * x - 3.0f * y * y);
#pragma unroll
    for (int k = 0; k < 3; ++k) rgb[k] = c[k] + 0.5f;
#undef GS_SH_FENCE
    if (rgb[0] < 0.0f) rgb[0] = 0.0f;
}
struct ShFromLds {
    const float* p;
    __device__ __forceinline__ float operator()(int j, int k) const { return p[j * 3 + k]; }
};
struct ShFromLds16 {
    const uint16_t* p;
    __device__ __forceinline__ float operator()(int j, int k) const { return __half2float(__ushort_as_half(p[j * 3 + k])); }
};

template <bool AA>
__device__ __forceinline__ void preprocess_one(const SceneView& sv, const gs_uniforms& u, const AttrView& av, uint32_t i,
                                               bool valid, float4* __restrict__ stage) {
    const size_t N = sv.stride, NC = sv.n;
    const float* __restrict__ blob = sv.blob;
    const uint32_t lane = threadIdx.x & (WAVE - 1);
    const uint32_t oid = sv.perm ? (valid ? sv.perm[i] : 0u) : i;

    const int tile_w = (int)((u.width + kTile - 1) / kTile);
    const int tile_h = (int)((u.height + kTile - 1) / kTile);

    uint32_t num_tiles = 0;
    float px = 0, py = 0, pz = 0, depth = 0, c00 = 0, c01 = 0, c11 = 0, opacity = 0, acut = 0, radii = 0, uvx = 0, uvy = 0;
    int bx0 = 0, by0 = 0, bx1 = 0, by1 = 0;
    if (valid) do {
        px = blob[(P_POS + 0) * N + i];
        py = blob[(P_POS + 1) * N + i];
        pz = blob[(P_POS + 2) * N + i];
        float p_hom[4], p_view[3];
#pragma unroll
        for (int r = 0; r < 4; ++r) {
            float s = u.proj_mat[0 * 4 + r] * px;
            s = s + u.proj_mat[1 * 4 + r] * py;
            s = s + u.proj_mat[2 * 4 + r] * pz;
            s = s + u.proj_mat[3 * 4 + r] * 1.0f;
            p_hom[r] = s;
        }
#pragma unroll
        for (int r = 0; r < 3; ++r) {
            float s = u.view_mat[0 * 4 + r] * px;
            s = s + u.view_mat[1 * 4 + r] * py;
            s = s + u.view_mat[2 * 4 + r] * pz;
            s = s + u.view_mat[3 * 4 + r] * 1.0f;
            p_view[r] = s;
        }
        const float p_w = 1.0f / p_hom[3];
        const float ndc_x = p_hom[0] * p_w, ndc_y = p_hom[1] * p_w;
        if (p_view[2] <= 0.2f) break;

        float tx = p_view[0], ty = p_view[1];
        const float tz = p_view[2];
        const float limx = 1.3f * u.tan_fovx;
        const float limy = 1.3f * u.tan_fovy;
        const float txtz = tx / tz;
        const float tytz = ty / tz;
        tx = fminf(limx, fmaxf(-limx, txtz)) * tz;
        ty = fminf(limy, fmaxf(-limy, tytz)) * tz;
        const float focal_x = (float)u.width / (2 * u.tan_fovx);
        const float focal_y = (float)u.height / (2 * u.tan_fovy);
        M3 J;
        J.c[0][0] = focal_x / tz;
        J.c[0][1] = 0;
        J.c[0][2] = -(focal_x * tx) / (tz * tz);
        J.c[1][0] = 0;
        J.c[1][1] = focal_y / tz;
        J.c[1][2] = -(focal_y * ty) / (tz * tz);
        J.c[2][0] = 0;
        J.c[2][1] = 0;
        J.c[2][2] = 0;

        M3 W;
#pragma unroll
        for (int c = 0; c < 3; ++c)
#pragma unroll
            for (int r = 0; r < 3; ++r) W.c[c][r] = u.view_mat[r * 4 + c];
        const float* __restrict__ cv = sv.cov3d;
        const float s0 = cv[0 * NC + i], s1 = cv[1 * NC + i], s2 = cv[2 * NC + i];
        const float s3 = cv[3 * NC + i], s4 = cv[4 * NC + i], s5 = cv[5 * NC + i];
        M3 Sigma;
        Sigma.c[0][0] = s0;
        Sigma.c[0][1] = s1;
        Sigma.c[0][2] = s2;
        Sigma.c[1][0] = s1;
        Sigma.c[1][1] = s3;
        Sigma.c[1][2] = s4;
        Sigma.c[2][0] = s2;
        Sigma.c[2][1] = s4;
        Sigma.c[2][2] = s5;
        M3 T = m3_mul(W, J);
        M3 cov = m3_mul(m3_mul(m3_transpose(T), Sigma), T);
        const float m00 = cov.c[0][0] + 0.3f;
        const float m11 = cov.c[1][1] + 0.3f;
        const float m01 = cov.c[0][1], m10 = cov.c[1][0];

        const float det = m00 * m11 - m10 * m01;
        if (det <= 0.0f) break;
        const float inv_det = 1.0f / det;
        c00 = m11 * inv_det;
        c01 = -m01 * inv_det;
        c11 = m00 * inv_det;

        const float mid = 0.5f * (m00 + m11);
        const float sq = sqrtf(fmaxf(0.1f, mid * mid - det));
        const float lambda1 = mid + sq;
        const float lambda2 = mid - sq;
        const float lambda = fmaxf(lambda1, lambda2);
        radii = ceilf(3.0f * sqrtf(lambda));

        uvx = ndc2pix(ndc_x, (int)u.width);
        uvy = ndc2pix(ndc_y, (int)u.height);

        bx0 = clampi(f2i_sat((uvx - radii) / kTile), 0, tile_w);
        by0 = clampi(f2i_sat((uvy - radii) / kTile), 0, tile_h);
        bx1 = clampi(f2i_sat((uvx + radii + kTile - 1) / kTile), 0, tile_w);
        by1 = clampi(f2i_sat((uvy + radii + kTile - 1) / kTile), 0, tile_h);
        const uint32_t nt = (uint32_t)(bx1 - bx0) * (uint32_t)(by1 - by0);
        if (nt == 0) break;
        depth = p_view[2];
        opacity = blob[(size_t)P_OPACITY * N + i];
        if (AA) {
            const float det_raw = cov.c[0][0] * cov.c[1][1] - cov.c[1][0] * cov.c[0][1];
            opacity = opacity * fminf(1.0f, sqrtf(fmaxf(0.0f, det_raw / det)));
            acut = alpha_cut_seeded(opacity, reinterpret_cast<const uint2*>(kExpfTab));
        } else {
            acut = sv.acut[i];
        }
        num_tiles = nt;
    } while (false);
    const bool vis = num_tiles != 0;

    uint32_t vis_base = 0;
    if (av.vis) {
        const uint64_t m = __ballot(vis);
        const uint32_t region = (i / BLOCK) % kVisRegions;
        if (lane == 0 && m != 0)
            vis_base = region * av.vis_region_slots + atomicAdd(av.vis_count + region * kVisCounterStride, (uint32_t)__popcll(m));
    }

    float rgb[3] = {0.0f, 0.0f, 0.0f};
    const uint64_t vm_sh = __ballot(vis);
    const uint32_t n_vis = (uint32_t)__popcll(vm_sh);
    const uint32_t my_rank = (uint32_t)__popcll(vm_sh & ((1ull << lane) - 1ull));
    uint8_t* const s_src = reinterpret_cast<uint8_t*>(stage + kPreShHalf * 12);
    if (vis) s_src[my_rank] = (uint8_t)lane;
    __builtin_amdgcn_wave_barrier();
    const int chunks = sv.sh16 ? 6 : 12;
    const uint32_t per_inst = sv.sh16 ? 10u : 5u;
    const uint32_t slot = sv.sh16 ? lane / 6u : lane / 12u, q = sv.sh16 ? lane % 6u : lane % 12u;
    const char* const sh_bytes = sv.sh16 ? reinterpret_cast<const char*>(sv.sh16) : reinterpret_cast<const char*>(blob + (size_t)P_SH * N);
    const size_t sh_stride = sv.sh16 ? 96 : 192;
    const uint32_t lds_base = (uint32_t)__builtin_amdgcn_readfirstlane((int)(uint32_t)(uintptr_t)stage);
    for (uint32_t half = 0; half * kPreShHalf < n_vis; ++half) {
        const uint32_t first = half * kPreShHalf, last = min(n_vis, first + (uint32_t)kPreShHalf);
        uint32_t dst = lds_base;
        for (uint32_t g0 = first; g0 < last; g0 += per_inst, dst += per_inst * (uint32_t)sh_stride) {
            const uint32_t g = g0 + slot;
            if (lane < 60u && g < last) {
                const uint32_t src_lane = s_src[g];
                const char* gsrc = sh_bytes + (size_t)(i - lane + src_lane) * sh_stride + q * 16u;
                unsigned keep;
                asm volatile("s_mov_b32 %0, m0\n\ts_mov_b32 m0, %2\n\ts_nop 0\n\tglobal_load_lds_dwordx4 %1, off\n\ts_mov_b32 m0, %0"
                             : "=&s"(keep) : "v"(gsrc), "s"(dst) : "memory");
            }
        }
        asm volatile("s_waitcnt vmcnt(0)" ::: "memory");
        __builtin_amdgcn_wave_barrier();
        if (vis && my_rank >= first && my_rank < last) {
            float dx = px - u.camera_position[0];
            float dy = py - u.camera_position[1];
            float dz = pz - u.camera_position[2];
            const float len = sqrtf(dx * dx + dy * dy + dz * dz);
            const float x = dx / len, y = dy / len, z = dz / len;
            const float4* blk = stage + (size_t)(my_rank - first) * chunks;
            if (sv.sh16) {
                sh_to_rgb(ShFromLds16{reinterpret_cast<const uint16_t*>(blk)}, x, y, z, rgb);
            } else {
                sh_to_rgb(ShFromLds{reinterpret_cast<const float*>(blk)}, x, y, z, rgb);
            }
            if (!av.vis) {
                av.depth[oid] = depth;
                av.aabb[oid] = make_ushort4((unsigned short)bx0, (unsigned short)by0, (unsigned short)bx1, (unsigned short)by1);
            }
        }
        __builtin_amdgcn_wave_barrier();
    }
    if (valid && !av.vis) av.tiles[oid] = num_tiles;

    const uint64_t vm = __ballot(vis);
    if (av.vis) {
        const uint32_t base = (uint32_t)__builtin_amdgcn_readfirstlane((int)vis_base);
        if (vis)
            av.vis[base + (uint32_t)__popcll(vm & ((1ull << lane) - 1ull))] =
                make_uint4(oid, __float_as_uint(depth), (uint32_t)bx0 | ((uint32_t)by0 << 16), (uint32_t)bx1 | ((uint32_t)by1 << 16));
    }
    if (vis) {
        stage[0 * kPrePlane + lane] = make_float4(c00, c01, c11, opacity);
        stage[1 * kPrePlane + lane] = make_float4(uvx, uvy, rgb[0], rgb[1]);
        const float r11 = -c01 * __builtin_amdgcn_rcpf(c11), r00 = -c01 * __builtin_amdgcn_rcpf(c00);
        stage[2 * kPrePlane + lane] = make_float4(rgb[2], acut, r11, r00);
        stage[3 * kPrePlane + lane] = make_float4(depth, radii, 0.0f, 0.0f);
    }
    uint32_t* const s_oid = reinterpret_cast<uint32_t*>(stage + 4 * kPrePlane);
    if (sv.perm) s_oid[lane] = oid;
    __builtin_amdgcn_wave_barrier();
    {
        float4* const rec0 = reinterpret_cast<float4*>(av.rec + (i - lane));
        const uint32_t c = lane & 3u;
#pragma unroll
        for (int t = 0; t < 4; ++t) {
            const uint32_t r = (uint32_t)t * 16u + (lane >> 2);
            if ((vm >> r) & 1ull) {
                const float4 val = stage[c * kPrePlane + r];
                float4* const dst = sv.perm ? reinterpret_cast<float4*>(av.rec + s_oid[r]) + c : rec0 + (size_t)r * 4 + c;
                *dst = val;
            }
        }
    }
}

template <bool AA>
__global__ __launch_bounds__(BLOCK) void k_preprocess(SceneView sv, PreUniforms pu, AttrView av) {
    __shared__ float4 s_stage[BLOCK / WAVE][kPreWaveLds];
    const gs_uniforms& u = pu.fp ? pu.fp->u : pu.u;
    const uint32_t i = blockIdx.x * BLOCK + threadIdx.x;
    frame_stamp(pu.stamps, ST_PREPROCESS);
    if (i == 0 && pu.counters) {
        pu.counters->visible = 0;
        pu.counters->instances = 0;
        pu.counters->overflow = 0;
        pu.counters->bin_entries = 0;
        pu.counters->max_bin = 0;
        pu.counters->slabs = 0;
        pu.counters->blend_resolved = 0;
        pu.counters->blend_redo = 0;
        pu.counters->q_head = 0;
        pu.counters->q_bins_done = 0;
    }
    preprocess_one<AA>(sv, u, av, i, i < sv.n, s_stage[threadIdx.x / WAVE]);
}

void launch_preprocess(const SceneView& sv, const gs_uniforms& u, const AttrView& av, Counters* counters,
                       const FrameParams* fp, uint64_t* stamps, bool antialiased, hipStream_t s) {
    if (sv.n == 0) return;
    PreUniforms pu;
    pu.u = u;
    pu.counters = counters;
    pu.fp = fp;
    pu.stamps = stamps;
    if (antialiased)
        hipLaunchKernelGGL(k_preprocess<true>, dim3((sv.n + BLOCK - 1) / BLOCK), dim3(BLOCK), 0, s, sv, pu, av);
    else
        hipLaunchKernelGGL(k_preprocess<false>, dim3((sv.n + BLOCK - 1) / BLOCK), dim3(BLOCK), 0, s, sv, pu, av);
}
}
```

3dgs.cpp_amd/csrc/gs_renderer.cpp:

```cpp
#include <algorithm>
#include <chrono>
#include <cstdio>
#include <cstdlib>
#include <cstring>
#include <limits>
#include <memory>
#include <vector>

#include "gs_blend_tuner.h"
#include "gs_depth_policy.h"
#include "gs_internal.h"

using namespace gs_host;

struct FrameBuffers {
    hipStream_t stream = nullptr;
    DevBuf<uint32_t> tiles;
    DevBuf<float> depth;
    DevBuf<ushort4> aabb;
    DevBuf<gs::AttrRecord> rec;
    DevBuf<uint4> vis;
    DevBuf<uint32_t> vis_count;
    bool planes_stale = false;
    uint32_t vis_region_slots = 0;
    DevBuf<uint32_t> dkeys[2], dvals[2];
    DevBuf<uint32_t> block_hist, digit_total;
    DevBuf<uint32_t> l1_hist, bin_count;
    DevBuf<uint32_t> cand;
    DevBuf<uint32_t> sorted;
    DevBuf<uint32_t> ranges;
    DevBuf<uint8_t> slabs;
    uint32_t slab_epoch = 0;
    DevBuf<gs::Counters> counters;
    DevBuf<uint64_t> stamps;
    DevBuf<gs::FrameParams> params;
    hipGraphExec_t graph_execs[2] = {nullptr, nullptr};
    struct GraphKey {
        int level = -1, bin_shift = -1, hw_exp = 0, contract = 1;
        bool antialiased = false, lockstep = false;
        uint32_t width = 0, height = 0, capacity = 0, cand_capacity = 0;
        const void *tile_order = nullptr, *ranges = nullptr, *sh16 = nullptr;
        bool operator==(const GraphKey& o) const {
            return level == o.level && bin_shift == o.bin_shift && hw_exp == o.hw_exp && contract == o.contract &&
                   antialiased == o.antialiased && lockstep == o.lockstep &&
                   width == o.width && height == o.height && capacity == o.capacity && cand_capacity == o.cand_capacity &&
                   tile_order == o.tile_order && ranges == o.ranges && sh16 == o.sh16;
        }
    } graph_keys[2];
    void drop_graph(int which) {
        if (graph_execs[which]) (void)hipGraphExecDestroy(graph_execs[which]);
        graph_execs[which] = nullptr;
        graph_keys[which] = GraphKey{};
    }
    void drop_graph() {
        drop_graph(0);
        drop_graph(1);
    }
    size_t n = 0;
    bool ready = false;

    void init(size_t n_, uint32_t capacity, uint32_t cand_capacity, bool dense_lists) {
        n = n_;
        HIP_CHECK(hipStreamCreateWithFlags(&stream, hipStreamNonBlocking));
        tiles.alloc(n);
        depth.alloc(n);
        aabb.alloc(n);
        rec.alloc(n);
        vis_region_slots = gs::vis_region_slots(static_cast<uint32_t>(n));
        if (dense_lists) ensure_dense_lists();
        l1_hist.alloc(1025 * static_cast<size_t>(gs::bin_level1_columns(static_cast<uint32_t>(n))));
        bin_count.alloc(2048);
        counters.alloc(1);
        stamps.alloc(gs::ST_COUNT);
        HIP_CHECK(hipMemset(stamps.p, 0, gs::ST_COUNT * sizeof(uint64_t)));
        params.alloc(1);
        set_capacity(capacity);
        set_cand_capacity(cand_capacity);
        ready = true;
    }
    void ensure_dense_lists() {
        if (vis.p) return;
        vis.alloc(static_cast<size_t>(gs::kVisRegions) * vis_region_slots);
        vis_count.alloc(gs::kVisRegions * gs::kVisCounterStride);
        HIP_CHECK(hipMemset(vis_count.p, 0, vis_count.n * sizeof(uint32_t)));
    }
    void ensure_depth_order() {
        if (dkeys[0].p) return;
        for (int k = 0; k < 2; ++k) {
            dkeys[k].alloc(n);
            dvals[k].alloc(n);
        }
        block_hist.alloc(256 * static_cast<size_t>(gs::kSortMaxBlocks));
        digit_total.alloc(256);
    }
    void set_capacity(uint32_t cap) {
        drop_graph();
        sorted.alloc(static_cast<size_t>(cap) + 4);
    }
    void set_cand_capacity(uint32_t ccap) {
        drop_graph();
        cand.alloc(3 * static_cast<size_t>(ccap));
        HIP_CHECK(hipMemset(cand.p, 0, 3 * static_cast<size_t>(ccap) * sizeof(uint32_t)));
    }
    void sync() const { HIP_CHECK(hipStreamSynchronize(stream)); }
    void sync_nothrow() const { (void)hipStreamSynchronize(stream); }
    ~FrameBuffers() {
        drop_graph();
        if (stream) (void)hipStreamDestroy(stream);
    }
};

struct FrameSlot {
    gs_uniforms u{};
    float* rgba = nullptr;
    uint8_t* bgra = nullptr;
    hipEvent_t done = nullptr;
    gs::Counters* h_counters = nullptr;
    uint64_t* h_stamps = nullptr;
    gs::FrameParams* h_params = nullptr;
    bool timed = false;
    int level = 0;
    int bin_shift = 3;
    bool lockstep = false;
    uint32_t tune_round = 0;
    int tune_shape = 0;
};

struct gs_renderer {
    static constexpr int kMaxInFlight = 8;
    static constexpr int kSlots = 2 * kMaxInFlight;

    gs_scene* scene = nullptr;
    bool timing = true;
    double tick_ms = 1e-5;

    FrameBuffers sets[kMaxInFlight];
    int num_sets = 1;
    uint32_t capacity = 0;
    uint32_t cand_capacity = 0;
    FrameBuffers* last_set = nullptr;
    uint32_t last_width = 0, last_height = 0;

    FrameSlot slots[kSlots];
    int in_flight_limit = 1;
    uint64_t frames_enqueued = 0;
    int pending = 0;

    gs_frame_stats last{};

    DepthPolicy policy;
    static constexpr int kGlobalLevel = DepthPolicy::kGlobalLevel;
    bool graph_mode = false;
    int exp_mode = 3;
    int blend_exp_mode() const { return exp_mode == 3 && !contract && !scene->unit_opacity ? 2 : exp_mode; }
    bool contract = false;
    bool antialiased = false;
    BlendTunerBank tuners;
    uint64_t dense_min = 4u << 20;
    bool debug_levels = std::getenv("GS_DEBUG_LEVELS") != nullptr;
    bool level2_queue = !(std::getenv("GS_L2_QUEUE") && std::atoi(std::getenv("GS_L2_QUEUE")) == 0);
    double stall_ms = std::getenv("GS_DEBUG_STALLS") ? std::atof(std::getenv("GS_DEBUG_STALLS")) : 0.0;
    static constexpr int kLaps = 10;
    std::chrono::steady_clock::time_point laps[kLaps];
    void lap(int k) {
        if (stall_ms > 0.0) laps[k] = std::chrono::steady_clock::now();
    }
    void report_stall() {
        if (stall_ms <= 0.0) return;
        auto ms = [&](int a, int b) { return std::chrono::duration<double, std::milli>(laps[b] - laps[a]).count(); };
        if (ms(0, 9) < stall_ms) return;
        std::fprintf(stderr, "[gs3d] stall: frame %llu held the host %.3f ms: wait-for-slot %.3f, setup %.3f, preprocess %.3f, order %.3f, level1 %.3f, "
                             "level2 %.3f, blend %.3f, closing events %.3f\n", (unsigned long long)(frames_enqueued - 1), ms(0, 9), ms(0, 1), ms(1, 2), ms(2, 3),
                     ms(3, 4), ms(4, 5), ms(5, 6), ms(6, 7), ms(7, 9));
    }
    bool have_frame = false;
    uint32_t retries = 0;
    uint32_t redo_chain = 0;
    double total_ms[7] = {0, 0, 0, 0, 0, 0, 0};
    uint64_t total_frames = 0;
    uint64_t lifetime_frames = 0;
    static constexpr size_t kIntervalRing = 8192;
    std::vector<float> intervals;
    bool prev_retired = false;
    uint64_t latest_done = 0;

    uint32_t* sorted_gid = nullptr;
    uint32_t* depth_order = nullptr;
    uint64_t num_tiles = 0;

    ~gs_renderer() {
        for (auto& sl : slots) {
            if (sl.done) (void)hipEventDestroy(sl.done);
            if (sl.h_counters) (void)hipHostFree(sl.h_counters);
            if (sl.h_stamps) (void)hipHostFree(sl.h_stamps);
            if (sl.h_params) (void)hipHostFree(sl.h_params);
        }
    }

    void set_capacity(uint32_t cap) {
        capacity = cap;
        for (auto& fb : sets)
            if (fb.ready) fb.set_capacity(cap);
    }
    void set_cand_capacity(uint32_t ccap) {
        cand_capacity = ccap;
        for (auto& fb : sets)
            if (fb.ready) fb.set_cand_capacity(ccap);
    }

    void init() {
        if (const char* e = std::getenv("GS_BLEND_LOCKSTEP")) tuners.pin(std::atoi(e) < 0 ? -1 : (std::atoi(e) != 0 ? 1 : 0));
        HIP_CHECK(hipSetDevice(scene->device));
        {
            int khz = 0;
            if (hipDeviceGetAttribute(&khz, hipDeviceAttributeWallClockRate, scene->device) == hipSuccess && khz > 0) tick_ms = 1.0 / khz;
        }
        HIP_CHECK(gs::bin_prepare_device());
        if (std::getenv("GS_DEBUG_OCCUPANCY")) gs::bin_debug_occupancy();
        for (auto& sl : slots) {
            HIP_CHECK(hipEventCreateWithFlags(&sl.done, hipEventDisableTiming));
            HIP_CHECK(hipHostMalloc(reinterpret_cast<void**>(&sl.h_stamps), gs::ST_COUNT * sizeof(uint64_t), hipHostMallocDefault));
            std::memset(sl.h_stamps, 0, gs::ST_COUNT * sizeof(uint64_t));
            HIP_CHECK(hipHostMalloc(reinterpret_cast<void**>(&sl.h_counters), sizeof(gs::Counters), hipHostMallocDefault));
            *sl.h_counters = gs::Counters{};
            HIP_CHECK(hipHostMalloc(reinterpret_cast<void**>(&sl.h_params), sizeof(gs::FrameParams), hipHostMallocDefault));
        }
        uint64_t want = std::max<uint64_t>(1u << 20, 8 * static_cast<uint64_t>(scene->n));
        if (const char* e = std::getenv("GS_INITIAL_CAPACITY")) want = std::max<uint64_t>(256, std::strtoull(e, nullptr, 10));
        capacity = static_cast<uint32_t>(std::min<uint64_t>(want, kMaxInstances));
        uint64_t want_cand = std::max<uint64_t>(1u << 18, 2 * static_cast<uint64_t>(scene->n));
        if (const char* e = std::getenv("GS_INITIAL_CAND_CAPACITY")) want_cand = std::max<uint64_t>(256, std::strtoull(e, nullptr, 10));
        else if (std::getenv("GS_INITIAL_CAPACITY")) want_cand = std::min<uint64_t>(want_cand, want);
        cand_capacity = static_cast<uint32_t>(std::min<uint64_t>(want_cand, capacity));
        sets[0].init(scene->n, capacity, cand_capacity, scene->n >= dense_min);
    }

    void set_num_sets(int k) {
        for (int i = 0; i < k; ++i)
            if (!sets[i].ready) sets[i].init(scene->n, capacity, cand_capacity, scene->n >= dense_min);
        num_sets = k;
    }

    DevBuf<uint32_t> tile_order;
    uint32_t order_tx = 0, order_ty = 0;
    void ensure_tile_order(uint32_t tx, uint32_t ty) {
        if (tx == order_tx && ty == order_ty && tile_order.p) return;
        drain();
        constexpr uint32_t B = 4;
        const uint64_t nt = static_cast<uint64_t>(tx) * ty;
        std::vector<std::vector<uint32_t>> per_xcd(8);
        const uint32_t nbx = (tx + B - 1) / B, nby = (ty + B - 1) / B;
        for (uint32_t by = 0; by < nby; ++by)
            for (uint32_t bx = 0; bx < nbx; ++bx) {
                auto& list = per_xcd[(bx + 3 * by) % 8];
                for (uint32_t y = by * B; y < std::min(ty, (by + 1) * B); ++y)
                    for (uint32_t x = bx * B; x < std::min(tx, (bx + 1) * B); ++x) list.push_back(y * tx + x);
            }
        std::vector<uint32_t> order(nt);
        size_t cursor[8] = {0, 0, 0, 0, 0, 0, 0, 0};
        for (uint64_t b = 0; b < nt; ++b) {
            int x = static_cast<int>(b % 8);
            if (cursor[x] >= per_xcd[x].size()) {
                size_t best = 0;
                for (int k = 0; k < 8; ++k)
                    if (per_xcd[k].size() - cursor[k] > best) best = per_xcd[k].size() - cursor[k], x = k;
            }
            order[b] = per_xcd[x][cursor[x]++];
        }
        tile_order.ensure(nt);
        if (nt) HIP_CHECK(hipMemcpy(tile_order.p, order.data(), nt * sizeof(uint32_t), hipMemcpyHostToDevice));
        order_tx = tx;
        order_ty = ty;
    }

    BinGeometry bin_geometry(uint32_t tx, uint32_t ty) const {
        BinGeometry g;
        if (!policy.bin_geometry(tx, ty, &g)) throw Error(GS_ERR_INVALID, "resolution too large for the tile binning (max 16384 x 16384)");
        return g;
    }

    void enqueue(const gs_uniforms& u, float* d_rgba, uint8_t* d_bgra) {
        HIP_CHECK(hipSetDevice(scene->device));
        FrameSlot& sl = slots[frames_enqueued % kSlots];
        FrameBuffers& fb = sets[frames_enqueued % num_sets];
        hipStream_t stream = fb.stream;
        const uint32_t n = static_cast<uint32_t>(scene->n);
        const uint32_t tx = tiles_across(u.width), ty = tiles_across(u.height);
        if (tx > 65535 || ty > 65535) throw Error(GS_ERR_INVALID, "resolution too large (tile box is 16-bit)");
        const uint64_t nt = static_cast<uint64_t>(tx) * ty;
        auto lacks_buffers = [&](int at_level) {
            return 2 * nt > fb.ranges.n || (at_level >= kGlobalLevel && !fb.dkeys[0].p) || (at_level == gs::kBinSlabLevel && !fb.slabs.p);
        };
        if (lacks_buffers(policy.frame_level())) {
            drain();
            const int at_level = policy.frame_level();
            fb.ranges.ensure(2 * nt);
            if (at_level >= kGlobalLevel) fb.ensure_depth_order();
            if (at_level == gs::kBinSlabLevel && !fb.slabs.p) {
                fb.slabs.alloc(static_cast<size_t>(gs::kSlabCapacity) * gs::kSlabDescBytes);
                HIP_CHECK(hipMemset(fb.slabs.p, 0, fb.slabs.n));
            }
        }
        last_set = &fb;
        last_width = u.width;
        last_height = u.height;
        const int tune_shape = tuners.select(u.width, u.height);
        const BlendTuner& tuner = tuners.current();
        const bool lockstep = tuner.current();
        const BinGeometry geo = bin_geometry(tx, ty);
        const int lv = policy.frame_level();
        const bool bin_local = lv < kGlobalLevel;
        num_tiles = nt;
        ensure_tile_order(tx, ty);
        lap(2);

        gs::SceneView sv{scene->render_blob(), scene->cov3d.p, n, static_cast<uint32_t>(gs::blob_stride(n)),
                          scene->sh_half ? scene->sh16.p : nullptr, scene->acut.p, scene->perm.p};
        gs::Counters* cnt = fb.counters.p;
        const bool l1_any_order = bin_local && geo.bin_shift <= 3;
        const bool dense_list = l1_any_order && n != 0 && n >= dense_min && fb.vis.p && u.width != 0 && u.height != 0;
        gs::AttrView av{fb.tiles.p, fb.depth.p, fb.aabb.p, fb.rec.p, dense_list ? fb.vis.p : nullptr, dense_list ? fb.vis_count.p : nullptr,
                        fb.vis_region_slots};
        fb.planes_stale = dense_list;

        const bool fused_counters = n != 0 && u.width != 0 && u.height != 0;
        if (!fused_counters) {
            HIP_CHECK(hipMemsetAsync(cnt, 0, sizeof(gs::Counters), stream));
            HIP_CHECK(hipMemsetAsync(fb.ranges.p, 0, 2 * nt * sizeof(uint32_t), stream));
        }
        uint64_t* const stamps = fb.stamps.p;
        auto passes = [&](const gs::FrameParams* fp) {
            gs::launch_preprocess(sv, u, av, cnt, fp, stamps, antialiased, stream);
            lap(3);
            if (!bin_local && n != 0) {
                const int blocks = std::max(1, std::min<int>(gs::kSortMaxBlocks, (n + gs::kSortTileKeys - 1) / gs::kSortTileKeys));
                const uint32_t* kin = reinterpret_cast<const uint32_t*>(fb.depth.p);
                const uint32_t* vin = nullptr;
                for (int pass = 0; pass < 4; ++pass) {
                    gs::RadixPass p{};
                    const int dst = pass & 1;
                    p.keys_in = kin;
                    p.vals_in = vin;
                    p.keys_out = fb.dkeys[dst].p;
                    p.vals_out = fb.dvals[dst].p;
                    p.n_in = &cnt->visible;
                    p.n_static = n;
                    p.tiles = fb.tiles.p;
                    p.n_out = &cnt->visible;
                    p.block_hist = fb.block_hist.p;
                    p.digit_total = fb.digit_total.p;
                    p.shift = pass * 8;
                    p.bits = 8;
                    p.blocks = blocks;
                    p.first = pass == 0;
                    p.stamps = pass == 0 ? stamps : nullptr;
                    gs::launch_radix_pass(p, stream);
                    kin = fb.dkeys[dst].p;
                    vin = fb.dvals[dst].p;
                }
            }
            lap(4);
            if (n != 0) {
                gs::BinLaunch b{};
                b.order = bin_local ? nullptr : fb.dvals[1].p;
                b.n_items = bin_local ? nullptr : &cnt->visible;
                b.n_bound = n;
                b.tiles = fb.tiles.p;
                b.aabb = fb.aabb.p;
                b.depth = fb.depth.p;
                b.vis = av.vis;
                b.vis_count = av.vis_count;
                b.vis_region_slots = av.vis_region_slots;
                b.hist = fb.l1_hist.p;
                b.bin_count = fb.bin_count.p;
                b.cand = fb.cand.p;
                b.ranges = fb.ranges.p;
                b.sorted_gid = fb.sorted.p;
                b.counters = cnt;
                b.capacity = capacity;
                b.cand_capacity = cand_capacity;
                b.slabs = fb.slabs.p;
                b.slab_capacity = fb.slabs.p ? gs::kSlabCapacity : 0u;
                b.slab_epoch = 0;
                if (level2_queue && !fp && lv == gs::kBinSlabLevel) {
                    if (++fb.slab_epoch == 0) ++fb.slab_epoch;
                    b.slab_epoch = fb.slab_epoch;
                }
                b.tiles_x = tx;
                b.tiles_y = ty;
                b.bins_x = geo.bins_x;
                b.bins_y = geo.bins_y;
                b.bin_shift = geo.bin_shift;
                b.grid_shift = geo.grid_shift;
                b.stamps = stamps;
                gs::launch_bin_level1_count(b, stream);
                gs::launch_bin_level1_scatter(b, l1_any_order, stream);
                lap(5);
                gs::launch_bin_level2(b, lv, stream);
            }
            lap(6);
            gs::launch_blend(fb.ranges.p, fb.sorted.p, tile_order.p, av, u.width, u.height, d_rgba, d_bgra, cnt,
                             fused_counters ? sl.h_counters : nullptr, blend_exp_mode(), contract, fp, lockstep, stamps, stream);
            gs::launch_frame_end(stamps, sl.h_stamps, fp, stream);
            lap(7);
        };
        depth_order = bin_local ? nullptr : fb.dvals[1].p;
        sorted_gid = fb.sorted.p;
        const bool replay = graph_mode && fused_counters;
        if (replay) {
            *sl.h_params = gs::FrameParams{u, d_rgba, d_bgra, sl.h_counters, sl.h_stamps};
            HIP_CHECK(hipMemcpyAsync(fb.params.p, sl.h_params, sizeof(gs::FrameParams), hipMemcpyHostToDevice, stream));
            const FrameBuffers::GraphKey key{lv, geo.bin_shift, blend_exp_mode(), contract ? 1 : 0,
                                             antialiased, lockstep,
                                             u.width, u.height, capacity, cand_capacity,
                                             tile_order.p, fb.ranges.p, sv.sh16};
            const int gi = lockstep ? 1 : 0;
            if (!fb.graph_execs[gi] || !(key == fb.graph_keys[gi])) {
                fb.drop_graph(gi);
                hipGraph_t graph = nullptr;
                HIP_CHECK(hipStreamBeginCapture(stream, hipStreamCaptureModeThreadLocal));
                try {
                    passes(fb.params.p);
                } catch (...) {
                    (void)hipStreamEndCapture(stream, &graph);
                    if (graph) (void)hipGraphDestroy(graph);
                    throw;
                }
                HIP_CHECK(hipStreamEndCapture(stream, &graph));
                const hipError_t e = hipGraphInstantiate(&fb.graph_execs[gi], graph, nullptr, nullptr, 0);
                (void)hipGraphDestroy(graph);
                HIP_CHECK(e);
                fb.graph_keys[gi] = key;
            }
            HIP_CHECK(hipGraphLaunch(fb.graph_execs[gi], stream));
        } else {
            passes(nullptr);
        }
        if (!fused_counters) HIP_CHECK(hipMemcpyAsync(sl.h_counters, cnt, sizeof(gs::Counters), hipMemcpyDeviceToHost, stream));
        HIP_CHECK(hipEventRecord(sl.done, stream));
        HIP_CHECK(hipGetLastError());

        sl.level = lv;
        sl.bin_shift = geo.bin_shift;
        sl.lockstep = lockstep;
        sl.tune_round = tuner.round;
        sl.tune_shape = tune_shape;
        sl.u = u;
        sl.rgba = d_rgba;
        sl.bgra = d_bgra;
        sl.timed = fused_counters;
        ++frames_enqueued;
        ++pending;
        lap(9);
    }

    FrameSlot& oldest() { return slots[(frames_enqueued - pending) % kSlots]; }
    FrameSlot& queued(int k) { return slots[(frames_enqueued - pending + k) % kSlots]; }

    void retire_oldest() {
        FrameSlot& sl = oldest();
        HIP_CHECK(hipEventSynchronize(sl.done));
        if (sl.h_counters->overflow) {
            rerun_queued();
            return;
        }
        redo_chain = 0;
        policy.frame_retired(sl.level, sl.h_counters->max_bin, sl.bin_shift);
        last = frame_stats(sl);
        have_frame = true;
        const float v[7] = {last.ms_preprocess, last.ms_prefix_sum, last.ms_preprocess_sort, last.ms_sort,
                            last.ms_tile_boundary, last.ms_render, last.ms_total};
        for (int k = 0; k < 7; ++k) total_ms[k] += v[k];
        ++total_frames;
        ++lifetime_frames;
        note_completion(sl, last.ms_total);
        --pending;
    }

    void rerun_queued() {
        for (auto& fb : sets)
            if (fb.ready) fb.sync();
        struct Redo {
            gs_uniforms u;
            float* rgba;
            uint8_t* bgra;
        };
        std::vector<Redo> redo;
        std::vector<DepthPolicy::QueuedFrame> ran;
        uint64_t need = 0, need_cand = 0;
        for (int k = 0; k < pending; ++k) {
            const FrameSlot& q = queued(k);
            const gs::Counters& c = *q.h_counters;
            redo.push_back({q.u, q.rgba, q.bgra});
            ran.push_back({q.level, q.bin_shift, q.u.width, q.u.height, c.overflow, c.max_bin});
            if (c.overflow & 1u) {
                if (c.bin_entries > cand_capacity) need_cand = std::max<uint64_t>(need_cand, c.bin_entries);
                else need = std::max<uint64_t>(need, c.instances);
            }
        }
        if (debug_levels) report_overflow();
        frames_enqueued -= pending;
        pending = 0;
        prev_retired = false;
        switch (policy.frames_overflowed(ran.data(), static_cast<int>(ran.size()))) {
            case DepthPolicy::kDepthsTooCrowded:
                throw Error(GS_ERR_OVERFLOW, "a bin's depths are too crowded for the bin-local order (one depth bucket beyond a slab, or more than 65 equal depths in one): needs the global depth-order path");
            case DepthPolicy::kBinTooFull:
                throw Error(GS_ERR_OVERFLOW, "a bin holds more candidates than the bin-local sort can order");
            case DepthPolicy::kRerun:
                break;
        }
        if (++redo_chain > 8) throw Error(GS_ERR_OVERFLOW, "instance buffers overflowed repeatedly");
        if (need_cand > cand_capacity) {
            need_cand = need_cand + need_cand / 2 + 4096;
            if (need_cand > kMaxInstances) throw Error(GS_ERR_OVERFLOW, "more than 2^30 level-1 candidates");
            set_cand_capacity(static_cast<uint32_t>(need_cand));
        }
        if (need > capacity) {
            need = need + need / 2 + 4096;
            if (need > kMaxInstances) throw Error(GS_ERR_OVERFLOW, "more than 2^30 tile instances");
            set_capacity(static_cast<uint32_t>(need));
        }
        ++retries;
        for (const Redo& f : redo) enqueue(f.u, f.rgba, f.bgra);
    }

    void report_overflow() {
        std::fprintf(stderr, "[gs3d] frame %llu overflowed at level %d (refined %d, hold %u):", (unsigned long long)(frames_enqueued - pending),
                     oldest().level, (int)policy.refined, policy.slab_hold);
        for (int k = 0; k < pending; ++k) {
            const FrameSlot& q = queued(k);
            std::fprintf(stderr, " [lvl %d bin 2^%d ovf %u max_bin %u E1 %u D %u slabs %u]", q.level, q.bin_shift, q.h_counters->overflow,
                         q.h_counters->max_bin, q.h_counters->bin_entries, q.h_counters->instances, q.h_counters->slabs);
        }
        std::fprintf(stderr, " capacity %u candidates %u\n", capacity, cand_capacity);
    }

    gs_frame_stats frame_stats(const FrameSlot& sl) const {
        gs_frame_stats st{};
        st.num_gaussians = scene->n;
        st.num_visible = sl.h_counters->visible;
        st.num_instances = sl.h_counters->instances;
        st.num_bin_entries = sl.h_counters->bin_entries;
        st.max_bin_entries = sl.h_counters->max_bin;
        st.sort_path = sl.level < kGlobalLevel ? 2u : 1u;
        st.sort_level = static_cast<uint32_t>(sl.level);
        st.bin_tiles = 1u << sl.bin_shift;
        st.instance_capacity = capacity;
        const uint64_t* const ts = sl.h_stamps;
        auto span = [&](int a, int b) {
            const int64_t d = static_cast<int64_t>(ts[b] - ts[a]);
            return d > 0 ? static_cast<float>(static_cast<double>(d) * tick_ms) : 0.0f;
        };
        if (sl.timed) st.ms_total = span(gs::ST_PREPROCESS, gs::ST_END);
        if (sl.timed && timing) {
            const bool global = sl.level >= kGlobalLevel;
            st.ms_preprocess = span(gs::ST_PREPROCESS, global ? gs::ST_ORDER : gs::ST_L1_COUNT);
            st.ms_prefix_sum = span(gs::ST_L1_COUNT, gs::ST_L1_SCATTER);
            st.ms_preprocess_sort = span(gs::ST_L1_SCATTER, gs::ST_L2);
            st.ms_sort = (global ? span(gs::ST_ORDER, gs::ST_L1_COUNT) : 0.0f) + span(gs::ST_L2, gs::ST_BLEND);
            st.ms_tile_boundary = 0.0f;
            st.ms_render = span(gs::ST_BLEND, gs::ST_END);
        }
        st.retries = retries;
        return st;
    }

    void note_completion(const FrameSlot& sl, float ms_total) {
        const uint64_t idx = frames_enqueued - pending;
        if (prev_retired) {
            const int64_t dticks = static_cast<int64_t>(sl.h_stamps[gs::ST_END] - slots[latest_done % kSlots].h_stamps[gs::ST_END]);
            const float dt = dticks > 0 ? static_cast<float>(static_cast<double>(dticks) * tick_ms) : 0.0f;
            if (intervals.size() >= kIntervalRing) intervals.erase(intervals.begin(), intervals.begin() + kIntervalRing / 2);
            intervals.push_back(dt);
            tuners.sample(sl.tune_shape, sl.u.width, sl.u.height, dt, ms_total, sl.lockstep, sl.tune_round);
            if (dt > 0.0f) latest_done = idx;
        } else {
            latest_done = idx;
        }
        prev_retired = true;
    }

    void latest_stats(gs_frame_stats* out) const {
        *out = last;
        out->num_gaussians = scene->n;
        out->instance_capacity = capacity;
        out->retries = retries;
        out->blend_redo = out->blend_resolved = 0;
    }

    void make_room() {
        while (pending >= in_flight_limit) retire_oldest();
    }
    void drain() {
        while (pending > 0) retire_oldest();
    }
};

extern "C" {

int gs_renderer_create(gs_scene* scene, gs_renderer** out) {
    return guarded([&] {
        if (!scene || !out) throw Error(GS_ERR_INVALID, "null argument");
        auto r = std::make_unique<gs_renderer>();
        r->scene = scene;
        if (const char* e = std::getenv("GS_L1_DENSE_MIN")) r->dense_min = std::strtoull(e, nullptr, 10);
        r->init();
        if (const char* e = std::getenv("GS_GRAPH")) r->graph_mode = std::atoi(e) != 0;
        if (const char* e = std::getenv("GS_EXP_MODE")) r->exp_mode = std::min(3, std::max(0, std::atoi(e)));
        if (const char* e = std::getenv("GS_BLEND_CONTRACTION")) r->contract = std::atoi(e) != 0;
        if (const char* e = std::getenv("GS_ANTIALIASED")) r->antialiased = std::atoi(e) != 0;
        if (const char* e = std::getenv("GS_BIN_SHIFT")) r->policy.min_bin_shift = std::min(5, std::max(2, std::atoi(e)));
        if (const char* e = std::getenv("GS_SORT_PATH")) {
            const int mode = std::atoi(e);
            if (mode < 0 || mode > 2) throw Error(GS_ERR_INVALID, "GS_SORT_PATH must be 0 (auto), 1 (global) or 2 (bin-local)");
            r->policy.sort_mode = mode;
        }
        *out = r.release();
    });
}

void gs_renderer_destroy(gs_renderer* r) {
    if (r)
        for (auto& fb : r->sets)
            if (fb.ready) fb.sync_nothrow();
    delete r;
}

int gs_render(gs_renderer* r, const gs_uniforms* u, float* d_rgba, uint8_t* d_bgra) {
    return guarded([&] {
        if (!r || !u) throw Error(GS_ERR_INVALID, "null argument");
        if (u->width == 0 || u->height == 0) throw Error(GS_ERR_INVALID, "empty framebuffer");
        r->lap(0);
        r->make_room();
        r->lap(1);
        if (r->stall_ms > 0.0)
            for (int k = 2; k < gs_renderer::kLaps; ++k) r->laps[k] = r->laps[1];
        r->enqueue(*u, d_rgba, d_bgra);
        r->report_stall();
    });
}

int gs_render_host(gs_renderer* r, const gs_uniforms* u, float* h_rgba, uint8_t* h_bgra) {
    return guarded([&] {
        if (!r || !u) throw Error(GS_ERR_INVALID, "null argument");
        if (u->width == 0 || u->height == 0) throw Error(GS_ERR_INVALID, "empty framebuffer");
        HIP_CHECK(hipSetDevice(r->scene->device));
        const size_t px = static_cast<size_t>(u->width) * u->height;
        DevBuf<float> d_rgba;
        DevBuf<uint8_t> d_bgra;
        if (h_rgba) d_rgba.alloc(px * 4);
        if (h_bgra) d_bgra.alloc(px * 4);
        r->drain();
        r->enqueue(*u, h_rgba ? d_rgba.p : nullptr, h_bgra ? d_bgra.p : nullptr);
        r->drain();
        if (h_rgba) HIP_CHECK(hipMemcpy(h_rgba, d_rgba.p, px * 4 * sizeof(float), hipMemcpyDeviceToHost));
        if (h_bgra) HIP_CHECK(hipMemcpy(h_bgra, d_bgra.p, px * 4, hipMemcpyDeviceToHost));
    });
}

int gs_synchronize(gs_renderer* r) {
    return guarded([&] {
        if (!r) throw Error(GS_ERR_INVALID, "null argument");
        r->drain();
    });
}

int gs_set_timing(gs_renderer* r, int enabled) {
    return guarded([&] {
        if (!r) throw Error(GS_ERR_INVALID, "null argument");
        r->drain();
        r->timing = enabled != 0;
    });
}

int gs_set_frames_in_flight(gs_renderer* r, int frames) {
    return guarded([&] {
        if (!r) throw Error(GS_ERR_INVALID, "null argument");
        if (frames < 1 || frames > gs_renderer::kMaxInFlight) throw Error(GS_ERR_INVALID, "frames in flight must be 1..8");
        r->drain();
        r->in_flight_limit = frames;
        r->set_num_sets(frames);
    });
}

int gs_get_stats(gs_renderer* r, gs_frame_stats* out) {
    return guarded([&] {
        if (!r || !out) throw Error(GS_ERR_INVALID, "null argument");
        r->drain();
        r->latest_stats(out);
        if (r->have_frame && r->last_set && r->last_set->counters.p) {
            gs::Counters c{};
            HIP_CHECK(hipMemcpy(&c, r->last_set->counters.p, sizeof c, hipMemcpyDeviceToHost));
            out->blend_redo = c.blend_redo;
            out->blend_resolved = c.blend_resolved;
        }
    });
}

int gs_poll_stats(gs_renderer* r, gs_frame_stats* out, uint64_t* frames_retired) {
    return guarded([&] {
        if (!r || !out) throw Error(GS_ERR_INVALID, "null argument");
        HIP_CHECK(hipSetDevice(r->scene->device));
        while (r->pending > 0) {
            const hipError_t e = hipEventQuery(r->oldest().done);
            if (e == hipErrorNotReady) break;
            HIP_CHECK(e);
            r->retire_oldest();
        }
        r->latest_stats(out);
        if (frames_retired) *frames_retired = r->lifetime_frames;
    });
}

int gs_get_timing_totals(gs_renderer* r, gs_frame_stats* sum, uint64_t* frames, int reset) {
    return guarded([&] {
        if (!r || !sum || !frames) throw Error(GS_ERR_INVALID, "null argument");
        r->drain();
        *sum = r->last;
        sum->ms_preprocess = static_cast<float>(r->total_ms[0]);
        sum->ms_prefix_sum = static_cast<float>(r->total_ms[1]);
        sum->ms_preprocess_sort = static_cast<float>(r->total_ms[2]);
        sum->ms_sort = static_cast<float>(r->total_ms[3]);
        sum->ms_tile_boundary = static_cast<float>(r->total_ms[4]);
        sum->ms_render = static_cast<float>(r->total_ms[5]);
        sum->ms_total = static_cast<float>(r->total_ms[6]);
        *frames = r->total_frames;
        if (reset) {
            for (double& v : r->total_ms) v = 0.0;
            r->total_frames = 0;
        }
    });
}

int gs_get_frame_intervals(gs_renderer* r, float* out_ms, uint64_t capacity, uint64_t* n_out, int reset) {
    return guarded([&] {
        if (!r || !n_out || (!out_ms && capacity)) throw Error(GS_ERR_INVALID, "null argument");
        r->drain();
        const uint64_t n = std::min<uint64_t>(capacity, r->intervals.size());
        if (n) std::memcpy(out_ms, r->intervals.data() + (r->intervals.size() - n), n * sizeof(float));
        *n_out = r->intervals.size();
        if (reset) {
            r->intervals.clear();
            r->prev_retired = false;
        }
    });
}

int gs_set_sort_path(gs_renderer* r, int mode) {
    return guarded([&] {
        if (!r) throw Error(GS_ERR_INVALID, "renderer is null");
        if (mode < 0 || mode > 2) throw Error(GS_ERR_INVALID, "sort path must be 0 (auto), 1 (global) or 2 (bin-local)");
        r->drain();
        r->policy.set_sort_mode(mode);
    });
}

int gs_set_exp_mode(gs_renderer* r, int mode) {
    return guarded([&] {
        if (!r) throw Error(GS_ERR_INVALID, "renderer is null");
        if (mode < 0 || mode > 3)
            throw Error(GS_ERR_INVALID, "exp mode must be 0 (pipeline polynomial), 1 (hardware v_exp_f32), 2 (libm's expf in binary64) or 3 (guarded v_exp_f32)");
        r->drain();
        r->exp_mode = mode;
    });
}

int gs_set_blend_contraction(gs_renderer* r, int enabled) {
    return guarded([&] {
        if (!r) throw Error(GS_ERR_INVALID, "renderer is null");
        r->drain();
        r->contract = enabled != 0;
    });
}

int gs_set_antialiased(gs_renderer* r, int enabled) {
    return guarded([&] {
        if (!r) throw Error(GS_ERR_INVALID, "renderer is null");
        r->drain();
        r->antialiased = enabled != 0;
    });
}

int gs_get_antialiased(gs_renderer* r) {
    int on = 0;
    const int rc = guarded([&] {
        if (!r) throw Error(GS_ERR_INVALID, "renderer is null");
        on = r->antialiased ? 1 : 0;
    });
    return rc != 0 ? rc : on;
}

int gs_set_blend_lockstep(gs_renderer* r, int mode) {
    return guarded([&] {
        if (!r) throw Error(GS_ERR_INVALID, "null argument");
        if (mode < -1 || mode > 1) throw Error(GS_ERR_INVALID, "blend lockstep: -1 automatic, 0 off, 1 on");
        r->drain();
        r->tuners.pin(mode);
    });
}

int gs_get_blend_lockstep(gs_renderer* r, int* settled) {
    int now = 0;
    const int rc = guarded([&] {
        if (!r) throw Error(GS_ERR_INVALID, "null argument");
        const BlendTuner& t = r->tuners.current();
        now = t.current() ? 1 : 0;
        if (settled) *settled = (t.forced >= 0 || t.phase == 3) ? 1 : 0;
    });
    return rc != 0 ? rc : now;
}

int gs_set_graph_mode(gs_renderer* r, int enabled) {
    return guarded([&] {
        if (!r) throw Error(GS_ERR_INVALID, "renderer is null");
        r->drain();
        r->graph_mode = enabled != 0;
        if (!r->graph_mode)
            for (auto& fb : r->sets) fb.drop_graph();
    });
}

int gs_debug_download(gs_renderer* r, int stage, void* dst, uint64_t bytes) {
    return guarded([&] {
        if (!r || !dst) throw Error(GS_ERR_INVALID, "null argument");
        r->drain();
        if (!r->have_frame) throw Error(GS_ERR_INVALID, "no frame rendered yet");
        if (stage == GS_STAGE_DEPTH_ORDER && !r->depth_order)
            throw Error(GS_ERR_INVALID, "the depth-order tap exists only on the global depth-order path (gs_set_sort_path(r, 1))");
        const uint64_t n = r->scene->n, v = r->last.num_visible;
        const uint64_t d = std::min<uint64_t>(r->last.num_instances, r->capacity);
        const void* src = nullptr;
        uint64_t size = 0;
        if (r->last_set->planes_stale && (stage == GS_STAGE_TILES || stage == GS_STAGE_DEPTH || stage == GS_STAGE_AABB)) {
            FrameBuffers& fb = *r->last_set;
            gs::launch_vis_to_planes(gs::AttrView{fb.tiles.p, fb.depth.p, fb.aabb.p, fb.rec.p, fb.vis.p, fb.vis_count.p, fb.vis_region_slots},
                                     static_cast<uint32_t>(n), fb.stream);
            HIP_CHECK(hipGetLastError());
            HIP_CHECK(hipStreamSynchronize(fb.stream));
            fb.planes_stale = false;
        }
        switch (stage) {
            case GS_STAGE_TILES: src = r->last_set->tiles.p; size = n * 4; break;
            case GS_STAGE_DEPTH: src = r->last_set->depth.p; size = n * 4; break;
            case GS_STAGE_RADIUS:
            case GS_STAGE_CONIC_OPACITY:
            case GS_STAGE_UV_RG:
            case GS_STAGE_B:
            case GS_STAGE_ALPHA_CUT:
                {
                    const size_t width = stage == GS_STAGE_RADIUS || stage == GS_STAGE_B || stage == GS_STAGE_ALPHA_CUT ? 1 : 4;
                    if (bytes < n * width * 4) throw Error(GS_ERR_INVALID, "destination too small for stage buffer");
                    std::vector<gs::AttrRecord> recs(n);
                    if (n) HIP_CHECK(hipMemcpy(recs.data(), r->last_set->rec.p, n * sizeof(gs::AttrRecord), hipMemcpyDeviceToHost));
                    float* out = static_cast<float*>(dst);
                    for (uint64_t i = 0; i < n; ++i) {
                        const gs::AttrRecord& a = recs[i];
                        if (stage == GS_STAGE_RADIUS) out[i] = a.depth_radius.y;
                        else if (stage == GS_STAGE_B) out[i] = a.b_cut_r.x;
                        else if (stage == GS_STAGE_ALPHA_CUT) out[i] = a.b_cut_r.y;
                        else std::memcpy(out + 4 * i, stage == GS_STAGE_CONIC_OPACITY ? &a.conic_op : &a.uv_rg, 16);
                    }
                    return;
                }
            case GS_STAGE_AABB: src = r->last_set->aabb.p; size = n * 8; break;
            case GS_STAGE_DEPTH_ORDER: src = r->depth_order; size = v * 4; break;
            case GS_STAGE_SORTED_TILE:
            case GS_STAGE_SORTED_GID:
            case GS_STAGE_RANGES:
                {
                    const uint64_t nt = r->num_tiles;
                    std::vector<uint32_t> rg(2 * nt);
                    if (nt) HIP_CHECK(hipMemcpy(rg.data(), r->last_set->ranges.p, rg.size() * 4, hipMemcpyDeviceToHost));
                    if (stage == GS_STAGE_RANGES) {
                        if (bytes < nt * 8) throw Error(GS_ERR_INVALID, "destination too small for stage buffer");
                        uint32_t* out = static_cast<uint32_t*>(dst);
                        uint64_t pos = 0;
                        for (uint64_t t = 0; t < nt; ++t) {
                            const uint32_t len = rg[2 * t + 1] - rg[2 * t];
                            out[2 * t] = len ? static_cast<uint32_t>(pos) : 0u;
                            out[2 * t + 1] = len ? static_cast<uint32_t>(pos + len) : 0u;
                            pos += len;
                        }
                        return;
                    }
                    if (bytes < d * 4) throw Error(GS_ERR_INVALID, "destination too small for stage buffer");
                    std::vector<uint32_t> lists;
                    if (stage == GS_STAGE_SORTED_GID) {
                        lists.resize(r->capacity);
                        HIP_CHECK(hipMemcpy(lists.data(), r->sorted_gid, lists.size() * 4, hipMemcpyDeviceToHost));
                    }
                    uint32_t* out = static_cast<uint32_t*>(dst);
                    uint64_t pos = 0;
                    for (uint64_t t = 0; t < nt; ++t)
                        for (uint64_t i = rg[2 * t]; i < rg[2 * t + 1] && pos < d; ++i)
                            out[pos++] = stage == GS_STAGE_SORTED_GID ? lists[i] : static_cast<uint32_t>(t);
                    return;
                }
            case GS_STAGE_LISTS_RAW: src = r->sorted_gid; size = d * 4; break;
            case GS_STAGE_RANGES_RAW: src = r->last_set->ranges.p; size = r->num_tiles * 8; break;
            default: throw Error(GS_ERR_INVALID, "unknown stage");
        }
        if (bytes < size) throw Error(GS_ERR_INVALID, "destination too small for stage buffer");
        if (size) HIP_CHECK(hipMemcpy(dst, src, size, hipMemcpyDeviceToHost));
    });
}

int gs_accumulate_contributions(gs_renderer* r, const gs_contributions* c) {
    return guarded([&] {
        if (!r || !c) throw Error(GS_ERR_INVALID, "null argument");
        if (reinterpret_cast<uintptr_t>(c->weight) % 8 != 0) throw Error(GS_ERR_INVALID, "weight must be 8-byte aligned");
        if (reinterpret_cast<uintptr_t>(c->pixels) % 4 != 0) throw Error(GS_ERR_INVALID, "pixels must be 4-byte aligned");
        if (reinterpret_cast<uintptr_t>(c->top_id) % 4 != 0) throw Error(GS_ERR_INVALID, "top_id must be 4-byte aligned");
        r->drain();
        if (!r->have_frame || !r->last_set) throw Error(GS_ERR_INVALID, "no frame rendered yet");
        if (!c->weight && !c->pixels && !c->top_id) return;
        HIP_CHECK(hipSetDevice(r->scene->device));
        const FrameBuffers& fb = *r->last_set;
        gs::launch_contributions(fb.ranges.p, fb.sorted.p, r->tile_order.p, fb.rec.p, r->last_width, r->last_height, c->mask, c->weight,
                                 c->pixels, c->top_id, fb.stream);
        HIP_CHECK(hipGetLastError());
        fb.sync();
    });
}

int gs_blend_features(gs_renderer* r, const gs_feature_maps* m) {
    return guarded([&] {
        if (!r || !m) throw Error(GS_ERR_INVALID, "null argument");
        if (m->channels > GS_FEATURE_CHANNELS_MAX) throw Error(GS_ERR_INVALID, "channels exceeds GS_FEATURE_CHANNELS_MAX (256)");
        if (m->channels > 0 && !m->features) throw Error(GS_ERR_INVALID, "channels > 0 needs features");
        if (m->channels > 0 && !m->out_features) throw Error(GS_ERR_INVALID, "features given without out_features");
        const struct { const void* p; const char* what; } ptrs[] = {
            {m->features, "features must be 4-byte aligned"},         {m->out_features, "out_features must be 4-byte aligned"},
            {m->out_alpha, "out_alpha must be 4-byte aligned"},       {m->out_depth, "out_depth must be 4-byte aligned"},
            {m->out_depth_median, "out_depth_median must be 4-byte aligned"}};
        for (const auto& q : ptrs)
            if (reinterpret_cast<uintptr_t>(q.p) % 4 != 0) throw Error(GS_ERR_INVALID, q.what);
        r->drain();
        if (!r->have_frame || !r->last_set) throw Error(GS_ERR_INVALID, "no frame rendered yet");
        float* out_features = m->channels > 0 ? m->out_features : nullptr;
        if (!out_features && !m->out_alpha && !m->out_depth && !m->out_depth_median) return;
        HIP_CHECK(hipSetDevice(r->scene->device));
        const FrameBuffers& fb = *r->last_set;
        gs::launch_features(fb.ranges.p, fb.sorted.p, r->tile_order.p, fb.rec.p, r->last_width, r->last_height, m->features, m->channels,
                            out_features, m->out_alpha, m->out_depth, m->out_depth_median, fb.stream);
        HIP_CHECK(hipGetLastError());
        fb.sync();
    });
}

void* gs_renderer_stream(gs_renderer* r) { return r ? r->sets[0].stream : nullptr; }

}
```

3dgs.cpp_amd/csrc/gs_scene_host.cpp:

```cpp
#include <cmath>
#include <cstdio>
#include <cstdlib>
#include <cstring>
#include <limits>
#include <memory>

#include "gs_internal.h"
#include "gs_sh_rotation.h"

using namespace gs_host;

void gs_scene::finish_load() {
    cov3d.alloc(6 * n);
    if (reinterpret_cast<uintptr_t>(blob) % 64 != 0)
        throw Error(GS_ERR_INVALID, "the scene blob must be 64-byte aligned (SH blocks are read as 16-byte vectors)");
    try {
        make_spatial_copy();
    } catch (const std::bad_alloc&) {
        drop_spatial_copy();
    } catch (const Error& e) {
        if (e.code != GS_ERR_NOMEM) throw;
        drop_spatial_copy();
    }
    gs::launch_cov3d(render_blob(), cov3d.p, static_cast<uint32_t>(n), static_cast<uint32_t>(gs::blob_stride(n)), 0, static_cast<uint32_t>(n), nullptr);
    acut.alloc(n);
    DevBuf<uint32_t> beyond;
    beyond.alloc(1);
    HIP_CHECK(hipMemset(beyond.p, 0, sizeof(uint32_t)));
    gs::launch_alpha_cut(render_blob(), acut.p, static_cast<uint32_t>(n), static_cast<uint32_t>(gs::blob_stride(n)), beyond.p, nullptr);
    HIP_CHECK(hipGetLastError());
    uint32_t flag = 0;
    HIP_CHECK(hipMemcpy(&flag, beyond.p, sizeof flag, hipMemcpyDeviceToHost));
    unit_opacity = flag == 0;
}

void gs_scene::drop_spatial_copy() {
    (void)hipGetLastError();
    perm.release();
    spatial_blob.release();
    std::fprintf(stderr, "[gs3d] no memory for the scene's copy in spatial order: rendering from the blob as loaded\n");
}
void gs_scene::make_spatial_copy() {
    uint64_t min_n = 4ull << 20;
    if (const char* e = std::getenv("GS_SPATIAL_MIN")) min_n = std::strtoull(e, nullptr, 10);
    if (n == 0 || n < min_n) return;
    const size_t st = gs::blob_stride(n);
    std::vector<float> pos(3 * n);
    for (int k = 0; k < 3; ++k)
        HIP_CHECK(hipMemcpy(pos.data() + static_cast<size_t>(k) * n, blob + static_cast<size_t>(gs::P_POS + k) * st, n * sizeof(float), hipMemcpyDeviceToHost));
    const float* const planes[3] = {pos.data(), pos.data() + n, pos.data() + 2 * n};
    const std::vector<uint32_t> order = gs::host::spatial_order(planes, n);
    perm.alloc(n);
    HIP_CHECK(hipMemcpy(perm.p, order.data(), n * sizeof(uint32_t), hipMemcpyHostToDevice));
    spatial_blob.alloc(gs::blob_floats(n));
    gs::launch_permute_blob(blob, perm.p, spatial_blob.p, static_cast<uint32_t>(n), static_cast<uint32_t>(st), nullptr);
    HIP_CHECK(hipGetLastError());
    HIP_CHECK(hipStreamSynchronize(nullptr));
}

namespace gs_host {

void quantize_sh(gs_scene* s) {
    if (s->sh_half) return;
    HIP_CHECK(hipSetDevice(s->device));
    s->sh16.alloc(48 * static_cast<size_t>(s->n));
    gs::launch_sh_to_half(s->render_blob(), s->sh16.p, static_cast<uint32_t>(gs::blob_stride(s->n)), 0, static_cast<uint32_t>(s->n), nullptr);
    HIP_CHECK(hipGetLastError());
    HIP_CHECK(hipStreamSynchronize(nullptr));
    s->sh_half = true;
}

void upload_vertices(gs_scene* s, const float* vertices, uint64_t n) {
    if (n >= kMaxGaussians) throw Error(GS_ERR_INVALID, "too many Gaussians (limit 2^31)");
    s->n = n;
    const size_t st = gs::blob_stride(n);
    std::vector<float> planes(gs::blob_floats(n));
    parallel_for(n, [&](uint64_t lo, uint64_t hi) {
        for (uint64_t i = lo; i < hi; ++i) {
            const float* v = vertices + i * gs::host::kVertexFloats;
            for (int k = 0; k < 3; ++k) planes[(gs::P_POS + k) * st + i] = v[k];
            for (int k = 0; k < 3; ++k) planes[(gs::P_SCALE + k) * st + i] = v[4 + k];
            for (int k = 0; k < 4; ++k) planes[(gs::P_ROT + k) * st + i] = v[8 + k];
            planes[static_cast<size_t>(gs::P_OPACITY) * st + i] = v[7];
            std::memcpy(&planes[static_cast<size_t>(gs::P_SH) * st + i * 48], v + 12, 48 * sizeof(float));
        }
    });
    s->owned_blob.alloc(planes.size());
    s->blob = s->owned_blob.p;
    if (n) HIP_CHECK(hipMemcpy(s->blob, planes.data(), planes.size() * sizeof(float), hipMemcpyHostToDevice));
    s->finish_load();
}

void activate_and_upload(gs_scene* s, const float* records, uint64_t n) {
    std::vector<float> verts(static_cast<size_t>(n) * gs::host::kVertexFloats);
    parallel_for(n, [&](uint64_t lo, uint64_t hi) {
        for (uint64_t i = lo; i < hi; ++i)
            gs::host::activate_record(records + i * gs::host::kRecordFloats, verts.data() + i * gs::host::kVertexFloats);
    });
    upload_vertices(s, verts.data(), n);
}

void check_device_arrays(const gs_device_arrays* a, uint64_t rows, bool build) {
    if (!a) throw Error(GS_ERR_INVALID, "null argument");
    const uint32_t k = a->sh_rest_coeffs;
    if (k != 0 && k != 3 && k != 8 && k != 15) throw Error(GS_ERR_INVALID, "sh_rest_coeffs must be 0, 3, 8 or 15 (SH degree 0..3)");
    const struct {
        const float* p;
        const char* name;
        bool required;
    } members[6] = {{a->means, "means", true},   {a->log_scales, "log_scales", true}, {a->quats, "quats", true}, {a->opacity_logits, "opacity_logits", true},
                    {a->sh_dc, "sh_dc", true}, {a->sh_rest, "sh_rest", k != 0}};
    for (const auto& m : members) {
        if (build && m.required && !m.p && rows) throw Error(GS_ERR_INVALID, std::string("device array `") + m.name + "` is null");
        if (reinterpret_cast<uintptr_t>(m.p) % 4 != 0) throw Error(GS_ERR_INVALID, std::string("device array `") + m.name + "` is not 4-byte aligned");
    }
}

void update_from_device_arrays(gs_scene* s, const gs_device_arrays& a, uint64_t first, uint64_t count, hipStream_t stream) {
    HIP_CHECK(hipSetDevice(s->device));
    const uint32_t n = static_cast<uint32_t>(s->n), st = static_cast<uint32_t>(gs::blob_stride(s->n));
    gs_device_arrays in = a;
    if (!in.sh_rest) in.sh_rest_coeffs = 0;
    gs::launch_ingest_arrays(in, s->blob, st, static_cast<uint32_t>(first), static_cast<uint32_t>(count), in.sh_rest != nullptr, stream);
    if (s->spatial_blob.p) gs::launch_permute_blob(s->blob, s->perm.p, s->spatial_blob.p, n, st, stream);
    if (a.log_scales || a.quats) gs::launch_cov3d(s->render_blob(), s->cov3d.p, n, st, 0, n, stream);
    if (s->sh_half && (a.sh_dc || a.sh_rest)) gs::launch_sh_to_half(s->render_blob(), s->sh16.p, st, 0, n, stream);
    if (a.opacity_logits) {
        DevBuf<uint32_t> beyond;
        beyond.alloc(1);
        HIP_CHECK(hipMemsetAsync(beyond.p, 0, sizeof(uint32_t), stream));
        gs::launch_alpha_cut(s->render_blob(), s->acut.p, n, st, beyond.p, stream);
        HIP_CHECK(hipGetLastError());
        uint32_t flag = 0;
        HIP_CHECK(hipMemcpyAsync(&flag, beyond.p, sizeof flag, hipMemcpyDeviceToHost, stream));
        HIP_CHECK(hipStreamSynchronize(stream));
        s->unit_opacity = flag == 0;
    }
    HIP_CHECK(hipGetLastError());
    HIP_CHECK(hipStreamSynchronize(stream));
}

void transform_scene(gs_scene* s, const gs_transform& t, uint64_t first, uint64_t count, hipStream_t stream) {
    HIP_CHECK(hipSetDevice(s->device));
    const ShRotation r = sh_rotation(t);
    gs::SceneTransform x;
    std::memcpy(x.R, r.R, sizeof x.R);
    std::memcpy(x.t, t.translation, sizeof x.t);
    x.s = t.scale;
    std::memcpy(x.q, r.q, sizeof x.q);
    std::memcpy(x.M, r.M, sizeof x.M);
    const uint32_t n = static_cast<uint32_t>(s->n), st = static_cast<uint32_t>(gs::blob_stride(s->n));
    uint32_t f = static_cast<uint32_t>(first), c = static_cast<uint32_t>(count);
    gs::launch_scene_transform(x, s->blob, st, f, c, stream);
    if (s->spatial_blob.p) {
        gs::launch_permute_blob(s->blob, s->perm.p, s->spatial_blob.p, n, st, stream);
        f = 0, c = n;
    }
    gs::launch_cov3d(s->render_blob(), s->cov3d.p, n, st, f, c, stream);
    if (s->sh_half) gs::launch_sh_to_half(s->render_blob(), s->sh16.p, st, f, c, stream);
    HIP_CHECK(hipGetLastError());
    HIP_CHECK(hipStreamSynchronize(stream));
}

void check_device_arrays_out(const gs_device_arrays_out* a) {
    if (!a) throw Error(GS_ERR_INVALID, "null argument");
    const uint32_t k = a->sh_rest_coeffs;
    if (k != 0 && k != 3 && k != 8 && k != 15) throw Error(GS_ERR_INVALID, "sh_rest_coeffs must be 0, 3, 8 or 15 (SH degree 0..3)");
    const struct {
        const float* p;
        const char* name;
    } members[6] = {{a->means, "means"}, {a->log_scales, "log_scales"}, {a->quats, "quats"}, {a->opacity_logits, "opacity_logits"},
                    {a->sh_dc, "sh_dc"}, {a->sh_rest, "sh_rest"}};
    for (const auto& m : members)
        if (reinterpret_cast<uintptr_t>(m.p) % 4 != 0) throw Error(GS_ERR_INVALID, std::string("device array `") + m.name + "` is not 4-byte aligned");
}

void export_records_streamed(const gs_scene* s, uint64_t first, uint64_t count, const std::function<void(const float*, uint64_t)>& sink) {
    if (count == 0) return;
    HIP_CHECK(hipSetDevice(s->device));
    uint64_t chunk = 1ull << 18;
    if (const char* e = std::getenv("GS_EXPORT_CHUNK")) chunk = std::max<uint64_t>(1, std::strtoull(e, nullptr, 10));
    chunk = std::min(chunk, count);
    const size_t floats = static_cast<size_t>(chunk) * gs::host::kRecordFloats;
    const uint32_t st = static_cast<uint32_t>(gs::blob_stride(s->n));
    DevBuf<float> dev[2];
    float* pinned[2] = {nullptr, nullptr};
    hipEvent_t arrived[2] = {nullptr, nullptr};
    hipStream_t down = nullptr;
    auto cleanup = [&] {
        if (down) (void)hipStreamSynchronize(down);
        for (int k = 0; k < 2; ++k) {
            if (pinned[k]) (void)hipHostFree(pinned[k]);
            if (arrived[k]) (void)hipEventDestroy(arrived[k]);
        }
        if (down) (void)hipStreamDestroy(down);
    };
// ... 260 lines not shown
```

include/gs3d_hip.h:

```cpp
#ifndef GS3D_HIP_H
#define GS3D_HIP_H

#include <stdint.h>

#ifdef __cplusplus
extern "C" {
#endif

typedef struct gs_scene gs_scene;
typedef struct gs_renderer gs_renderer;

enum gs_status {
    GS_OK = 0,
    GS_ERR_INVALID = -1,
    GS_ERR_IO = -2,
    GS_ERR_DEVICE = -3,
    GS_ERR_NOMEM = -4,
    GS_ERR_OVERFLOW = -5
};

typedef struct {
    float position[3];
    float rotation[4];
    float fov;
    float near_plane;
    float far_plane;
} gs_camera;

typedef struct {
    float camera_position[4];
    float proj_mat[16];
    float view_mat[16];
    uint32_t width;
    uint32_t height;
    float tan_fovx;
    float tan_fovy;
} gs_uniforms;

typedef struct {
    uint64_t num_gaussians;
    uint64_t num_visible;
    uint64_t num_instances;
    uint64_t instance_capacity;
    float ms_preprocess;
    float ms_prefix_sum;
    float ms_preprocess_sort;
    float ms_sort;
    float ms_tile_boundary;
    float ms_render;
    float ms_total;
    uint32_t retries;
    uint32_t num_bin_entries;
    uint32_t max_bin_entries;
    uint32_t sort_path;
    uint32_t bin_tiles;
    uint32_t sort_level;
    uint32_t blend_redo;
    uint32_t blend_resolved;
    uint32_t pad_;
} gs_frame_stats;

enum gs_stage {
    GS_STAGE_TILES = 0,
    GS_STAGE_DEPTH = 1,
    GS_STAGE_RADIUS = 2,
    GS_STAGE_AABB = 3,
    GS_STAGE_CONIC_OPACITY = 4,
    GS_STAGE_UV_RG = 5,
    GS_STAGE_B = 6,
    GS_STAGE_DEPTH_ORDER = 7,
    GS_STAGE_ALPHA_CUT = 8,
    GS_STAGE_SORTED_TILE = 11,
    GS_STAGE_SORTED_GID = 12,
    GS_STAGE_RANGES = 13,
    GS_STAGE_LISTS_RAW = 14,
    GS_STAGE_RANGES_RAW = 15
};

const char* gs_last_error(void);
int gs_device_count(int* count);


int gs_scene_load_ply(const char* path, int device, gs_scene** out);

int gs_read_ply(const char* path, float* records, uint64_t capacity, uint64_t* n_out);
int gs_activate_records(const float* records, uint64_t n, float* vertices);

int gs_scene_from_records(const float* records, uint64_t n, int device, gs_scene** out);

int gs_scene_from_vertices(const float* vertices, uint64_t n, int device, gs_scene** out);

int gs_scene_from_device_blob(float* d_blob, uint64_t n, int device, gs_scene** out);
uint64_t gs_scene_blob_floats(uint64_t n);
int gs_scene_blob(const gs_scene* s, float** d_blob, uint64_t* floats);

typedef struct {
    const float* means;
    const float* log_scales;
    const float* quats;
    const float* opacity_logits;
    const float* sh_dc;
    const float* sh_rest;
    uint32_t     sh_rest_coeffs;
} gs_device_arrays;

int gs_scene_from_device_arrays(const gs_device_arrays* a, uint64_t n, int device, void* stream, gs_scene** out);
int gs_scene_update_from_device_arrays(gs_scene* s, const gs_device_arrays* a, uint64_t first, uint64_t count, void* stream);

typedef struct {
    float rotation[4];
    float translation[3];
    float scale;
} gs_transform;
int gs_scene_transform(gs_scene* s, const gs_transform* t, uint64_t first, uint64_t count, void* stream);
int gs_transform_sh_matrices(const gs_transform* t, float out[83]);
int gs_transform_camera(const gs_transform* t, const gs_camera* in, gs_camera* out);

int gs_deactivate_vertices(const float* vertices, uint64_t n, float* records);
int gs_write_ply(const char* path, const float* records, uint64_t n);
typedef struct {
    float* means;
    float* log_scales;
    float* quats;
    float* opacity_logits;
    float* sh_dc;
    float* sh_rest;
    uint32_t sh_rest_coeffs;
} gs_device_arrays_out;
int gs_scene_to_device_arrays(const gs_scene* s, const gs_device_arrays_out* a, uint64_t first, uint64_t count, void* stream);
int gs_scene_download_records(const gs_scene* s, uint64_t first, uint64_t count, float* records);
int gs_scene_save_ply(const gs_scene* s, const char* path);

uint64_t gs_scene_num_vertices(const gs_scene* s);
int gs_scene_quantize_sh(gs_scene* s);
int gs_scene_sh_bits(const gs_scene* s);
int gs_scene_download_vertex_range(const gs_scene* s, uint64_t first, uint64_t count, float* vertices);
int gs_scene_download_vertices(const gs_scene* s, float* vertices);
int gs_scene_download_cov3d(const gs_scene* s, float* cov3d);
void gs_scene_destroy(gs_scene* s);


int gs_renderer_create(gs_scene* scene, gs_renderer** out);
void gs_renderer_destroy(gs_renderer* r);

int gs_camera_uniforms(const gs_camera* cam, uint32_t width, uint32_t height, gs_uniforms* out);

int gs_render(gs_renderer* r, const gs_uniforms* u, float* d_rgba, uint8_t* d_bgra);

int gs_render_host(gs_renderer* r, const gs_uniforms* u, float* h_rgba, uint8_t* h_bgra);

int gs_synchronize(gs_renderer* r);
int gs_set_timing(gs_renderer* r, int enabled);
int gs_set_frames_in_flight(gs_renderer* r, int frames);
int gs_set_sort_path(gs_renderer* r, int mode);
int gs_set_exp_mode(gs_renderer* r, int mode);
int gs_set_blend_contraction(gs_renderer* r, int enabled);
int gs_set_antialiased(gs_renderer* r, int enabled);
int gs_get_antialiased(gs_renderer* r);
int gs_set_graph_mode(gs_renderer* r, int enabled);
int gs_set_blend_lockstep(gs_renderer* r, int mode);
int gs_get_blend_lockstep(gs_renderer* r, int* settled);
int gs_get_timing_totals(gs_renderer* r, gs_frame_stats* sum, uint64_t* frames, int reset);
int gs_get_frame_intervals(gs_renderer* r, float* out_ms, uint64_t capacity, uint64_t* n_out, int reset);
int gs_get_stats(gs_renderer* r, gs_frame_stats* out);
int gs_poll_stats(gs_renderer* r, gs_frame_stats* out, uint64_t* frames_retired);
int gs_debug_download(gs_renderer* r, int stage, void* dst, uint64_t bytes);
typedef struct {
    const uint8_t* mask;
    uint64_t* weight;
    uint32_t* pixels;
    uint32_t* top_id;
} gs_contributions;
int gs_accumulate_contributions(gs_renderer* r, const gs_contributions* c);
#define GS_FEATURE_CHANNELS_MAX 256
typedef struct {
    const float* features;
    uint32_t     channels;
    float* out_features;
    float* out_alpha;
    float* out_depth;
    float* out_depth_median;
} gs_feature_maps;
int gs_blend_features(gs_renderer* r, const gs_feature_maps* m);
int gs_debug_expf_scan(int device, uint32_t first_bits, uint64_t count, uint64_t* block_sums, uint64_t blocks_capacity, double* guard);
int gs_debug_activation_expf_scan(int device, uint32_t first_bits, uint64_t count, uint64_t* block_sums, uint64_t blocks_capacity);
int gs_debug_alpha_cut_scan(int device, uint32_t first_bits, uint64_t count, uint64_t* mismatches, uint32_t* first_mismatch);
void* gs_renderer_stream(gs_renderer* r);

#define GS_DIST_ID_BYTES 128
typedef struct gs_dist gs_dist;
int gs_dist_unique_id(uint8_t id[GS_DIST_ID_BYTES]);
int gs_dist_create(const uint8_t id[GS_DIST_ID_BYTES], int rank, int world, int device, gs_dist** out);
int gs_dist_rank(const gs_dist* d);
int gs_dist_world(const gs_dist* d);
uint64_t gs_dist_pose_count(const gs_dist* d, uint64_t poses);
int gs_dist_broadcast_scene(gs_dist* d, gs_scene* mine , int root, gs_scene** out);
#define GS_DIST_COPY_ON_ROOT 1u
int gs_dist_broadcast_scene_ex(gs_dist* d, gs_scene* mine , int root, unsigned flags, gs_scene** out);
typedef struct {
    uint64_t ranks;
    uint64_t world;
    uint64_t checksum;
    uint64_t broadcast_bytes;
    double broadcast_ms;
    uint32_t checksums_equal;
    uint32_t rccl_version;
} gs_dist_report;
int gs_dist_verify(gs_dist* d, const gs_scene* scene, gs_dist_report* out);
void gs_dist_destroy(gs_dist* d);

#ifdef __cplusplus
}
#endif
#endif
```

Before: 4865.

## Fuse level-1 binning count and scatter into preprocess kernel

After: 5291 (median of 6 runs). 8.8% higher.

```diff
diff --git a/3dgs.cpp_amd/binding.py b/3dgs.cpp_amd/binding.py
--- a/3dgs.cpp_amd/binding.py
+++ b/3dgs.cpp_amd/binding.py
@@ -48,7 +48,7 @@
            "gs_scene_download_vertices", "gs_scene_download_cov3d",
            "gs_deactivate_vertices", "gs_write_ply", "gs_scene_to_device_arrays", "gs_scene_download_records", "gs_scene_save_ply",
            "gs_scene_destroy", "gs_renderer_create", "gs_renderer_destroy", "gs_camera_uniforms",
-           "gs_render", "gs_render_host", "gs_synchronize", "gs_set_timing", "gs_set_frames_in_flight", "gs_set_sort_path", "gs_set_exp_mode", "gs_set_graph_mode", "gs_set_blend_lockstep", "gs_get_blend_lockstep", "gs_set_blend_contraction", "gs_set_antialiased", "gs_get_antialiased", "gs_get_timing_totals",
+           "gs_render", "gs_render_host", "gs_synchronize", "gs_set_timing", "gs_set_frames_in_flight", "gs_set_sort_path", "gs_set_exp_mode", "gs_set_graph_mode", "gs_set_blend_lockstep", "gs_get_blend_lockstep", "gs_set_level1_fused", "gs_get_level1_fused", "gs_set_blend_contraction", "gs_set_antialiased", "gs_get_antialiased", "gs_get_timing_totals",
            "gs_get_frame_intervals", "gs_get_stats", "gs_poll_stats", "gs_debug_download", "gs_accumulate_contributions", "gs_blend_features", "gs_debug_expf_scan", "gs_debug_alpha_cut_scan", "gs_renderer_stream",
            "gs_dist_unique_id", "gs_dist_create", "gs_dist_rank", "gs_dist_world", "gs_dist_pose_count",
            "gs_dist_broadcast_scene", "gs_dist_broadcast_scene_ex", "gs_dist_verify", "gs_dist_destroy"]
@@ -534,6 +534,15 @@
             _check(now)
         return bool(now), bool(settled.value)
 
+    def set_level1_fused(self, mode):
+        _check(lib().gs_set_level1_fused(self._h, C.c_int(int(mode))))
+
+    def level1_fused(self):
+        now = lib().gs_get_level1_fused(self._h)
+        if now < 0:
+            _check(now)
+        return bool(now)
+
     def set_sort_path(self, mode):
         _check(lib().gs_set_sort_path(self._h, C.c_int(int(mode))))
 
diff --git a/3dgs.cpp_amd/csrc/gs_bin_l2.hip b/3dgs.cpp_amd/csrc/gs_bin_l2.hip
--- a/3dgs.cpp_amd/csrc/gs_bin_l2.hip
+++ b/3dgs.cpp_amd/csrc/gs_bin_l2.hip
@@ -28,7 +28,33 @@
     uint32_t slab_capacity;
     uint32_t epoch;
     uint64_t* stamps;
+    const uint32_t* l1_words;
+    uint32_t l1_cap;
 };
+
+__device__ __forceinline__ uint32_t bin_candidates(const BuildArgs& a, uint32_t bin) {
+    return a.l1_words ? a.l1_words[(size_t)(kL1FusedCursor0 + bin) * kL1FusedStride] : a.bin_count[bin];
+}
+__device__ __forceinline__ uint32_t bin_offset(const BuildArgs& a, uint32_t bin) {
+    return a.l1_words ? ((bin >> a.g.grid_shift) * a.g.bins_x + (bin & ((1u << a.g.grid_shift) - 1u))) * a.l1_cap : a.bin_count[kBinOffsets + bin];
+}
+__device__ __forceinline__ void bin_close_one_pass(const BuildArgs& a, uint32_t& c, int tid) {
+    if (!a.l1_words) return;
+    if (tid == 0 && c != 0) {
+        atomicAdd(&a.counters->bin_entries, c);
+        atomicMax(&a.counters->max_bin, c);
+    }
+    if (c > a.l1_cap) {
+        if (tid == 0) atomicOr(&a.counters->overflow, 1u);
+        c = 0;
+    }
+}
+__device__ __forceinline__ void one_pass_visible(const BuildArgs& a) {
+    if (!a.l1_words || blockIdx.x != 0 || threadIdx.x >= kVisRegions) return;
+    uint32_t v = a.l1_words[(size_t)threadIdx.x * kL1FusedStride];
+    for (int o = WAVE / 2; o != 0; o >>= 1) v += (uint32_t)__shfl_xor((int)v, o);
+    if ((threadIdx.x & (WAVE - 1)) == 0 && v != 0) atomicAdd(&a.counters->visible, v);
+}
 
 __device__ __forceinline__ uint32_t bin_local_box(const BinGrid& g, uint32_t bin, ushort4 box) {
     const int S = 1 << g.bin_shift;
@@ -66,6 +92,7 @@
 template <int R2, int THREADS, bool SORT>
 __global__ __launch_bounds__(THREADS) void k_bin_build(BuildArgs a) {
     frame_stamp(a.stamps, ST_L2);
+    one_pass_visible(a);
     BUILD_ROW(blockIdx.x);
     using L = BuildLayout<R2, THREADS, SORT>;
     constexpr int NW = L::NW, MAXC = L::MAXC, SS = L::SS, PER = kBuildSlots / NW;
@@ -84,8 +111,9 @@
     const uint32_t bin = ((blockIdx.x / a.g.bins_x) << a.g.grid_shift) | (blockIdx.x % a.g.bins_x);
     BUILD_T(0);
     uint32_t c, off;
-    c = a.bin_count[bin];
-    off = a.bin_count[kBinOffsets + bin];
+    c = bin_candidates(a, bin);
+    off = bin_offset(a, bin);
+    bin_close_one_pass(a, c, tid);
     if ((uint64_t)off + c > a.cand_capacity) c = 0;
     if (SORT && c > (uint32_t)MAXC) {
         if (tid == 0) atomicOr(&a.counters->overflow, 2u);
@@ -381,6 +409,7 @@
 
     BUILD_ROW(MODE == 2 ? 1023u : blockIdx.x);
     if constexpr (MODE != 2) frame_stamp(a.stamps, ST_L2);
+    if constexpr (MODE != 2) one_pass_visible(a);
     int tid = threadIdx.x, lane = tid & (WAVE - 1), w = tid / WAVE;
     auto screen_bin = [&](uint32_t i) { return ((i / a.g.bins_x) << a.g.grid_shift) | (i % a.g.bins_x); };
     uint32_t bin = screen_bin(MODE == 3 ? 0u : blockIdx.x);
@@ -388,8 +417,9 @@
     BUILD_T(0);
     uint32_t c_total = 0, off = 0;
     auto bin_extent = [&]() {
-        c_total = (uint32_t)__builtin_amdgcn_readfirstlane((int)a.bin_count[bin]);
-        off = (uint32_t)__builtin_amdgcn_readfirstlane((int)a.bin_count[kBinOffsets + bin]);
+        c_total = (uint32_t)__builtin_amdgcn_readfirstlane((int)bin_candidates(a, bin));
+        off = (uint32_t)__builtin_amdgcn_readfirstlane((int)bin_offset(a, bin));
+        bin_close_one_pass(a, c_total, tid);
         if ((uint64_t)off + c_total > a.cand_capacity) c_total = 0;
         if (c_total > kMaxInBin) {
             if (tid == 0) atomicOr(&a.counters->overflow, 2u);
@@ -1087,7 +1117,7 @@
         const uint32_t n_bins = a.g.bins_x * a.g.bins_y;
         {
             uint32_t* const cnt = smem;
-            const uint32_t mine = (uint32_t)tid < n_bins ? a.bin_count[screen_bin((uint32_t)tid)] : 0u;
+            const uint32_t mine = (uint32_t)tid < n_bins ? bin_candidates(a, screen_bin((uint32_t)tid)) : 0u;
             cnt[tid] = mine;
             if (tid == 0) q_planned = 0;
             __syncthreads();
@@ -1279,6 +1309,8 @@
     a.slab_capacity = b.slab_capacity;
     a.epoch = b.slab_epoch;
     a.stamps = b.stamps;
+    a.l1_words = b.l1_fused_words;
+    a.l1_cap = b.l1_fused_cap;
     const uint32_t bins = b.bins_x * b.bins_y;
     const bool sort = level < kBinSortLevels;
     if (sort && b.bin_shift <= 3) {
diff --git a/3dgs.cpp_amd/csrc/gs_blend.hip b/3dgs.cpp_amd/csrc/gs_blend.hip
--- a/3dgs.cpp_amd/csrc/gs_blend.hip
+++ b/3dgs.cpp_amd/csrc/gs_blend.hip
@@ -547,8 +547,11 @@
                        reinterpret_cast<uchar4*>(bgra), counters, host_counters, fp, av.vis_count, lockstep ? 1u : 0u, stamps);
 }
 
-__global__ __launch_bounds__(WAVE) void k_frame_end(uint64_t* __restrict__ stamps, uint64_t* host_stamps, const FrameParams* __restrict__ fp) {
+__global__ __launch_bounds__(WAVE) void k_frame_end(uint64_t* __restrict__ stamps, uint64_t* host_stamps, const FrameParams* __restrict__ fp,
+                                                   uint32_t* __restrict__ l1_words, uint32_t l1_counters) {
     if (fp) host_stamps = fp->host_stamps;
+    if (l1_words)
+        for (uint32_t k = threadIdx.x; k < l1_counters; k += WAVE) l1_words[(size_t)k * kL1FusedStride] = 0;
     const uint64_t now = wall_clock64();
     const int t = threadIdx.x;
     if (t < ST_COUNT) {
@@ -557,9 +560,9 @@
         if (host_stamps) host_stamps[t] = v;
     }
 }
-void launch_frame_end(uint64_t* stamps, uint64_t* host_stamps, const FrameParams* fp, hipStream_t s) {
+void launch_frame_end(uint64_t* stamps, uint64_t* host_stamps, const FrameParams* fp, uint32_t* l1_words, uint32_t l1_counters, hipStream_t s) {
     if (!stamps) return;
-    hipLaunchKernelGGL(k_frame_end, dim3(1), dim3(WAVE), 0, s, stamps, host_stamps, fp);
+    hipLaunchKernelGGL(k_frame_end, dim3(1), dim3(WAVE), 0, s, stamps, host_stamps, fp, l1_words, l1_counters);
 }
 
 void launch_blend(const uint32_t* ranges, const uint32_t* sorted_gid, const uint32_t* tile_order, const AttrView& av,
diff --git a/3dgs.cpp_amd/csrc/gs_depth_policy.h b/3dgs.cpp_amd/csrc/gs_depth_policy.h
--- a/3dgs.cpp_amd/csrc/gs_depth_policy.h
+++ b/3dgs.cpp_amd/csrc/gs_depth_policy.h
@@ -132,4 +132,55 @@
     }
 };
 
+struct L1FusedPolicy {
+    static constexpr uint32_t kHold = 32;
+    static constexpr uint32_t kGrowCeiling = 4;
+    static constexpr uint32_t kWideRatio = 8;
+
+    int mode = -1;
+    uint32_t hold = 0;
+    bool have_last = false;
+    uint32_t last_width = 0, last_height = 0, last_max_bin = 0, last_e1 = 0, last_v = 0;
+    int last_bin_shift = -1;
+
+    static uint32_t region_cap(uint32_t cand_capacity, uint32_t bins) { return bins ? cand_capacity / bins : 0u; }
+    static bool cap_suffices(uint32_t cap, uint32_t max_bin) { return 4ull * cap >= 5ull * max_bin; }
+    bool knows(uint32_t width, uint32_t height, int bin_shift) const {
+        return have_last && width == last_width && height == last_height && bin_shift == last_bin_shift;
+    }
+
+    enum Verdict { kEngage = 0, kSwitchedOff, kNotAnyOrder, kDenseRegime, kNoSpatialCopy, kHeld, kCapTooSmall, kWideSplats };
+    Verdict decide(bool any_order, bool planes_regime, bool spatial_copy, uint32_t width, uint32_t height, int bin_shift,
+                   uint32_t cand_capacity, uint32_t bins) const {
+        if (mode == 0) return kSwitchedOff;
+        if (!any_order) return kNotAnyOrder;
+        if (!planes_regime) return kDenseRegime;
+        if (hold != 0) return kHeld;
+        const uint32_t cap = region_cap(cand_capacity, bins);
+        if (cap == 0) return kCapTooSmall;
+        if (mode == 1) return kEngage;
+        if (!spatial_copy) return kNoSpatialCopy;
+        if (knows(width, height, bin_shift)) {
+            if ((uint64_t)last_e1 > (uint64_t)kWideRatio * last_v) return kWideSplats;
+            if (!cap_suffices(cap, last_max_bin)) return kCapTooSmall;
+        }
+        return kEngage;
+    }
+    uint32_t grow_to(Verdict v, uint32_t width, uint32_t height, int bin_shift, uint32_t cand_capacity, uint32_t bins,
+                     uint32_t default_cand_capacity) const {
+        if (v != kCapTooSmall || mode != -1 || !knows(width, height, bin_shift)) return 0;
+        const uint64_t cap = ((uint64_t)last_max_bin * 5 + 3) / 4 + last_max_bin / 4;
+        const uint64_t want = cap * bins;
+        if (want <= cand_capacity || want > (uint64_t)kGrowCeiling * default_cand_capacity) return 0;
+        return (uint32_t)want;
+    }
+    void frame_retired(uint32_t width, uint32_t height, int bin_shift, uint32_t max_bin, uint32_t e1, uint32_t v) {
+        if (hold != 0) --hold;
+        have_last = true;
+        last_width = width, last_height = height, last_bin_shift = bin_shift;
+        last_max_bin = max_bin, last_e1 = e1, last_v = v;
+    }
+    void region_overflowed() { hold = kHold; }
+};
+
 }
diff --git a/3dgs.cpp_amd/csrc/gs_kernels.h b/3dgs.cpp_amd/csrc/gs_kernels.h
--- a/3dgs.cpp_amd/csrc/gs_kernels.h
+++ b/3dgs.cpp_amd/csrc/gs_kernels.h
@@ -44,6 +44,16 @@
 constexpr uint32_t kVisRegions = 256, kVisCounterStride = 32;
 uint32_t vis_region_slots(uint32_t n);
 
+constexpr uint32_t kL1FusedStride = 32, kL1FusedCursor0 = kVisRegions, kL1FusedWords = (kVisRegions + 1024) * kL1FusedStride;
+struct L1Fused {
+    uint32_t* words;
+    uint32_t* cand;
+    uint32_t cap;
+    uint64_t* vis_mask;
+    uint32_t tiles_x, tiles_y, bins_x, bins_y;
+    int bin_shift, grid_shift;
+};
+
 struct Counters {
     uint32_t visible;
     uint32_t instances;
@@ -86,8 +96,8 @@
 void launch_scene_export(const gs_device_arrays_out& a, const float* blob, uint32_t stride, uint32_t first, uint32_t count, hipStream_t s);
 void launch_scene_export_records(float* records, const float* blob, uint32_t stride, uint32_t first, uint32_t count, hipStream_t s);
 void launch_preprocess(const SceneView& sv, const gs_uniforms& u, const AttrView& av, Counters* counters,
-                       const FrameParams* fp, uint64_t* stamps, bool antialiased, hipStream_t s);
-void launch_frame_end(uint64_t* stamps, uint64_t* host_stamps, const FrameParams* fp, hipStream_t s);
+                       const FrameParams* fp, uint64_t* stamps, bool antialiased, const L1Fused& lf, hipStream_t s);
+void launch_frame_end(uint64_t* stamps, uint64_t* host_stamps, const FrameParams* fp, uint32_t* l1_words, uint32_t l1_counters, hipStream_t s);
 
 struct RadixPass {
     const uint32_t* keys_in;
@@ -126,6 +136,8 @@
     Counters* counters;
     uint32_t capacity;
     uint32_t cand_capacity;
+    const uint32_t* l1_fused_words;
+    uint32_t l1_fused_cap;
     void* slabs;
     uint32_t slab_capacity;
     uint32_t slab_epoch;
@@ -135,6 +147,8 @@
     uint64_t* stamps;
 };
 void launch_vis_to_planes(const AttrView& av, uint32_t n, hipStream_t s);
+void launch_records_to_planes(const uint64_t* vis_mask, const uint32_t* perm, const AttrView& av, uint32_t n, uint32_t width, uint32_t height,
+                              hipStream_t s);
 uint32_t bin_level1_blocks(uint32_t n_items);
 uint32_t bin_level1_columns(uint32_t n_items);
 void bin_debug_occupancy();
diff --git a/3dgs.cpp_amd/csrc/gs_preprocess.hip b/3dgs.cpp_amd/csrc/gs_preprocess.hip
--- a/3dgs.cpp_amd/csrc/gs_preprocess.hip
+++ b/3dgs.cpp_amd/csrc/gs_preprocess.hip
@@ -1,4 +1,4 @@
-#include "gs_device.h"
+#include "gs_bin.h"
 
 namespace gs {
 
@@ -12,6 +12,12 @@
     Counters* counters;
     const FrameParams* fp;
     uint64_t* stamps;
+};
+
+template <int R1>
+struct PreBins {
+    uint32_t tbl[R1 ? 64 * R1 : 1];
+    uint32_t vis;
 };
 
 constexpr int kPrePlane = 68, kPreStage = 4 * kPrePlane + 16;
@@ -77,9 +83,9 @@
     __device__ __forceinline__ float operator()(int j, int k) const { return __half2float(__ushort_as_half(p[j * 3 + k])); }
 };
 
-template <bool AA>
+template <bool AA, int R1>
 __device__ __forceinline__ void preprocess_one(const SceneView& sv, const gs_uniforms& u, const AttrView& av, uint32_t i,
-                                               bool valid, float4* __restrict__ stage) {
+                                               bool valid, float4* __restrict__ stage, const L1Fused& lf, PreBins<R1>& bins) {
     const size_t N = sv.stride, NC = sv.n;
     const float* __restrict__ blob = sv.blob;
     const uint32_t lane = threadIdx.x & (WAVE - 1);
@@ -203,6 +209,41 @@
         const uint32_t region = (i / BLOCK) % kVisRegions;
         if (lane == 0 && m != 0)
             vis_base = region * av.vis_region_slots + atomicAdd(av.vis_count + region * kVisCounterStride, (uint32_t)__popcll(m));
+    }
+
+    uint32_t bb = 0;
+    uint32_t fbase[R1 ? (64 * R1) / BLOCK : 1];
+    if constexpr (R1 != 0) {
+        constexpr int NB = 64 * R1;
+        const int tid = threadIdx.x;
+        if (vis) {
+            const uint32_t x0 = (uint32_t)bx0 >> lf.bin_shift, y0 = (uint32_t)by0 >> lf.bin_shift;
+            const uint32_t x1 = (((uint32_t)bx1 - 1u) >> lf.bin_shift) + 1u, y1 = (((uint32_t)by1 - 1u) >> lf.bin_shift) + 1u;
+            bb = x0 | (y0 << 8) | (x1 << 16) | (y1 << 24);
+        }
+        __syncthreads();
+        {
+            const uint32_t x0 = bb & 255u, y0 = (bb >> 8) & 255u, x1 = (bb >> 16) & 255u, y1 = bb >> 24;
+            const bool big = (x1 - x0) * (y1 - y0) > kL1BigBox;
+            if (!big)
+                for (uint32_t y = y0; y < y1; ++y)
+                    for (uint32_t x = x0; x < x1; ++x) atomicAdd(&bins.tbl[(y << lf.grid_shift) | x], 1u);
+            for (uint64_t bm = __ballot(big); bm != 0; bm &= bm - 1) {
+                const uint32_t b1 = (uint32_t)__builtin_amdgcn_readlane((int)bb, __ffsll((unsigned long long)bm) - 1);
+                const uint32_t gx0 = b1 & 255u, gy0 = (b1 >> 8) & 255u, bw = ((b1 >> 16) & 255u) - gx0, cells = bw * ((b1 >> 24) - gy0);
+                for (uint32_t c = lane; c < cells; c += WAVE) atomicAdd(&bins.tbl[((gy0 + c / bw) << lf.grid_shift) | (gx0 + c % bw)], 1u);
+            }
+            const uint32_t nv = (uint32_t)__popcll(__ballot(vis));
+            if (lane == 0 && nv) atomicAdd(&bins.vis, nv);
+        }
+        __syncthreads();
+#pragma unroll
+        for (int k = 0; k < NB / BLOCK; ++k) {
+            const uint32_t b = (uint32_t)(k * BLOCK + tid), cnt = bins.tbl[b];
+            fbase[k] = cnt ? atomicAdd(lf.words + (size_t)(kL1FusedCursor0 + b) * kL1FusedStride, cnt) : 0u;
+        }
+        if (tid == 0 && bins.vis)
+            __hip_atomic_fetch_add(lf.words + (size_t)((i / BLOCK) % kVisRegions) * kL1FusedStride, bins.vis, __ATOMIC_RELAXED, __HIP_MEMORY_SCOPE_AGENT);
     }
 
     float rgb[3] = {0.0f, 0.0f, 0.0f};
@@ -245,14 +286,54 @@
             } else {
                 sh_to_rgb(ShFromLds{reinterpret_cast<const float*>(blk)}, x, y, z, rgb);
             }
-            if (!av.vis) {
+            if (!av.vis && R1 == 0) {
                 av.depth[oid] = depth;
                 av.aabb[oid] = make_ushort4((unsigned short)bx0, (unsigned short)by0, (unsigned short)bx1, (unsigned short)by1);
             }
         }
         __builtin_amdgcn_wave_barrier();
     }
-    if (valid && !av.vis) av.tiles[oid] = num_tiles;
+    if (R1 == 0 && valid && !av.vis) av.tiles[oid] = num_tiles;
+    if constexpr (R1 != 0) {
+        const uint64_t m = __ballot(vis);
+        if (lane == 0 && valid) lf.vis_mask[i / WAVE] = m;
+    }
+
+    if constexpr (R1 != 0) {
+        constexpr int NB = 64 * R1;
+#pragma unroll
+        for (int k = 0; k < NB / BLOCK; ++k) bins.tbl[k * BLOCK + (int)threadIdx.x] = fbase[k];
+        __syncthreads();
+        const BinGrid g{lf.tiles_x, lf.tiles_y, lf.bins_x, lf.bins_y, lf.bin_shift, lf.grid_shift};
+        auto emit = [&](uint32_t bin, uint32_t k, uint32_t gid, ushort4 box) {
+            const uint32_t pos = atomicAdd(&bins.tbl[bin], 1u);
+            if (pos < lf.cap) {
+                const uint32_t sb = (bin >> lf.grid_shift) * lf.bins_x + (bin & ((1u << lf.grid_shift) - 1u));
+                uint32_t* const rec = lf.cand + (size_t)kCandWords * ((size_t)sb * lf.cap + pos);
+                rec[0] = k;
+                rec[1] = gid;
+                rec[2] = bin_local_box16(g, bin, box);
+            }
+        };
+        const uint32_t x0 = bb & 255u, y0 = (bb >> 8) & 255u, x1 = (bb >> 16) & 255u, y1 = bb >> 24;
+        const ushort4 tb = make_ushort4((unsigned short)bx0, (unsigned short)by0, (unsigned short)bx1, (unsigned short)by1);
+        const uint32_t key = __float_as_uint(depth);
+        const bool big = (x1 - x0) * (y1 - y0) > kL1BigBox;
+        if (!big)
+            for (uint32_t y = y0; y < y1; ++y)
+                for (uint32_t x = x0; x < x1; ++x) emit((y << lf.grid_shift) | x, key, oid, tb);
+        for (uint64_t bm = __ballot(big); bm != 0; bm &= bm - 1) {
+            const int src = __ffsll((unsigned long long)bm) - 1;
+            const uint32_t b1 = (uint32_t)__builtin_amdgcn_readlane((int)bb, src);
+            const uint32_t gx0 = b1 & 255u, gy0 = (b1 >> 8) & 255u, bw = ((b1 >> 16) & 255u) - gx0, cells = bw * ((b1 >> 24) - gy0);
+            const uint32_t bkey = (uint32_t)__builtin_amdgcn_readlane((int)key, src), bgid = (uint32_t)__builtin_amdgcn_readlane((int)oid, src);
+            const uint32_t blo = (uint32_t)__builtin_amdgcn_readlane((int)((uint32_t)bx0 | ((uint32_t)by0 << 16)), src);
+            const uint32_t bhi = (uint32_t)__builtin_amdgcn_readlane((int)((uint32_t)bx1 | ((uint32_t)by1 << 16)), src);
+            const ushort4 bbox = make_ushort4((unsigned short)(blo & 0xFFFFu), (unsigned short)(blo >> 16), (unsigned short)(bhi & 0xFFFFu),
+                                              (unsigned short)(bhi >> 16));
+            for (uint32_t c = lane; c < cells; c += WAVE) emit(((gy0 + c / bw) << lf.grid_shift) | (gx0 + c % bw), bkey, bgid, bbox);
+        }
+    }
 
     const uint64_t vm = __ballot(vis);
     if (av.vis) {
@@ -286,9 +367,14 @@
     }
 }
 
-template <bool AA>
-__global__ __launch_bounds__(BLOCK) void k_preprocess(SceneView sv, PreUniforms pu, AttrView av) {
+template <bool AA, int R1>
+__global__ __launch_bounds__(BLOCK) void k_preprocess(SceneView sv, PreUniforms pu, AttrView av, L1Fused lf) {
     __shared__ float4 s_stage[BLOCK / WAVE][kPreWaveLds];
+    __shared__ PreBins<R1> s_bins;
+    if constexpr (R1 != 0) {
+        for (int b = threadIdx.x; b < 64 * R1; b += BLOCK) s_bins.tbl[b] = 0;
+        if (threadIdx.x == 0) s_bins.vis = 0;
+    }
     const gs_uniforms& u = pu.fp ? pu.fp->u : pu.u;
     const uint32_t i = blockIdx.x * BLOCK + threadIdx.x;
     frame_stamp(pu.stamps, ST_PREPROCESS);
@@ -304,20 +390,58 @@
         pu.counters->q_head = 0;
         pu.counters->q_bins_done = 0;
     }
-    preprocess_one<AA>(sv, u, av, i, i < sv.n, s_stage[threadIdx.x / WAVE]);
+    preprocess_one<AA, R1>(sv, u, av, i, i < sv.n, s_stage[threadIdx.x / WAVE], lf, s_bins);
+}
+
+__global__ __launch_bounds__(BLOCK) void k_records_to_planes(const uint64_t* __restrict__ vis_mask, const uint32_t* __restrict__ perm,
+                                                             const AttrRecord* __restrict__ rec, uint32_t n, uint32_t width, uint32_t height,
+                                                             uint32_t* __restrict__ tiles, float* __restrict__ depth, ushort4* __restrict__ aabb) {
+    const uint32_t j = blockIdx.x * BLOCK + threadIdx.x;
+    if (j >= n) return;
+    const uint32_t oid = perm ? perm[j] : j;
+    uint32_t nt = 0;
+    if ((vis_mask[j / WAVE] >> (j % WAVE)) & 1ull) {
+        const AttrRecord r = rec[oid];
+        const int tile_w = (int)((width + kTile - 1) / kTile), tile_h = (int)((height + kTile - 1) / kTile);
+        const float uvx = r.uv_rg.x, uvy = r.uv_rg.y, radii = r.depth_radius.y;
+        const int bx0 = clampi(f2i_sat((uvx - radii) / kTile), 0, tile_w);
+        const int by0 = clampi(f2i_sat((uvy - radii) / kTile), 0, tile_h);
+        const int bx1 = clampi(f2i_sat((uvx + radii + kTile - 1) / kTile), 0, tile_w);
+        const int by1 = clampi(f2i_sat((uvy + radii + kTile - 1) / kTile), 0, tile_h);
+        nt = (uint32_t)(bx1 - bx0) * (uint32_t)(by1 - by0);
+        depth[oid] = r.depth_radius.x;
+        aabb[oid] = make_ushort4((unsigned short)bx0, (unsigned short)by0, (unsigned short)bx1, (unsigned short)by1);
+    }
+    tiles[oid] = nt;
+}
+void launch_records_to_planes(const uint64_t* vis_mask, const uint32_t* perm, const AttrView& av, uint32_t n, uint32_t width, uint32_t height,
+                              hipStream_t s) {
+    if (n == 0) return;
+    hipLaunchKernelGGL(k_records_to_planes, dim3((n + BLOCK - 1) / BLOCK), dim3(BLOCK), 0, s, vis_mask, perm, av.rec, n, width, height, av.tiles,
+                       av.depth, av.aabb);
 }
 
 void launch_preprocess(const SceneView& sv, const gs_uniforms& u, const AttrView& av, Counters* counters,
-                       const FrameParams* fp, uint64_t* stamps, bool antialiased, hipStream_t s) {
+                       const FrameParams* fp, uint64_t* stamps, bool antialiased, const L1Fused& lf, hipStream_t s) {
     if (sv.n == 0) return;
     PreUniforms pu;
     pu.u = u;
     pu.counters = counters;
     pu.fp = fp;
     pu.stamps = stamps;
-    if (antialiased)
-        hipLaunchKernelGGL(k_preprocess<true>, dim3((sv.n + BLOCK - 1) / BLOCK), dim3(BLOCK), 0, s, sv, pu, av);
-    else
-        hipLaunchKernelGGL(k_preprocess<false>, dim3((sv.n + BLOCK - 1) / BLOCK), dim3(BLOCK), 0, s, sv, pu, av);
-}
-}
+    const dim3 grid((sv.n + BLOCK - 1) / BLOCK);
+    const int r1 = !lf.words ? 0 : (lf.grid_shift == 4 ? 4 : 16);
+#define GS_PRE_CASE(A, R)                                                                       \
+    if (antialiased == A && r1 == R) {                                                          \
+        hipLaunchKernelGGL((k_preprocess<A, R>), grid, dim3(BLOCK), 0, s, sv, pu, av, lf);      \
+        return;                                                                                 \
+    }
+    GS_PRE_CASE(false, 0)
+    GS_PRE_CASE(false, 4)
+    GS_PRE_CASE(false, 16)
+    GS_PRE_CASE(true, 0)
+    GS_PRE_CASE(true, 4)
+    GS_PRE_CASE(true, 16)
+#undef GS_PRE_CASE
+}
+}
diff --git a/3dgs.cpp_amd/csrc/gs_renderer.cpp b/3dgs.cpp_amd/csrc/gs_renderer.cpp
--- a/3dgs.cpp_amd/csrc/gs_renderer.cpp
+++ b/3dgs.cpp_amd/csrc/gs_renderer.cpp
@@ -21,12 +21,14 @@
     DevBuf<gs::AttrRecord> rec;
     DevBuf<uint4> vis;
     DevBuf<uint32_t> vis_count;
-    bool planes_stale = false;
+    int planes_stale = 0;
+    DevBuf<uint64_t> vis_mask;
     uint32_t vis_region_slots = 0;
     DevBuf<uint32_t> dkeys[2], dvals[2];
     DevBuf<uint32_t> block_hist, digit_total;
     DevBuf<uint32_t> l1_hist, bin_count;
     DevBuf<uint32_t> cand;
+    DevBuf<uint32_t> l1_words;
     DevBuf<uint32_t> sorted;
     DevBuf<uint32_t> ranges;
     DevBuf<uint8_t> slabs;
@@ -37,12 +39,12 @@
     hipGraphExec_t graph_execs[2] = {nullptr, nullptr};
     struct GraphKey {
         int level = -1, bin_shift = -1, hw_exp = 0, contract = 1;
-        bool antialiased = false, lockstep = false;
+        bool antialiased = false, lockstep = false, l1_fused = false;
         uint32_t width = 0, height = 0, capacity = 0, cand_capacity = 0;
         const void *tile_order = nullptr, *ranges = nullptr, *sh16 = nullptr;
         bool operator==(const GraphKey& o) const {
             return level == o.level && bin_shift == o.bin_shift && hw_exp == o.hw_exp && contract == o.contract &&
-                   antialiased == o.antialiased && lockstep == o.lockstep &&
+                   antialiased == o.antialiased && lockstep == o.lockstep && l1_fused == o.l1_fused &&
                    width == o.width && height == o.height && capacity == o.capacity && cand_capacity == o.cand_capacity &&
                    tile_order == o.tile_order && ranges == o.ranges && sh16 == o.sh16;
         }
@@ -70,6 +72,9 @@
         if (dense_lists) ensure_dense_lists();
         l1_hist.alloc(1025 * static_cast<size_t>(gs::bin_level1_columns(static_cast<uint32_t>(n))));
         bin_count.alloc(2048);
+        vis_mask.alloc((n + 63) / 64 + 1);
+        l1_words.alloc(gs::kL1FusedWords);
+        HIP_CHECK(hipMemset(l1_words.p, 0, l1_words.n * sizeof(uint32_t)));
         counters.alloc(1);
         stamps.alloc(gs::ST_COUNT);
         HIP_CHECK(hipMemset(stamps.p, 0, gs::ST_COUNT * sizeof(uint64_t)));
@@ -122,6 +127,8 @@
     int level = 0;
     int bin_shift = 3;
     bool lockstep = false;
+    bool l1_fused = false;
+    uint32_t l1_cap = 0;
     uint32_t tune_round = 0;
     int tune_shape = 0;
 };
@@ -138,6 +145,9 @@
     int num_sets = 1;
     uint32_t capacity = 0;
     uint32_t cand_capacity = 0;
+    uint32_t default_cand_capacity = 0;
+    L1FusedPolicy l1_policy;
+    bool last_l1_fused = false;
     FrameBuffers* last_set = nullptr;
     uint32_t last_width = 0, last_height = 0;
 
@@ -157,6 +167,8 @@
     bool antialiased = false;
     BlendTunerBank tuners;
     uint64_t dense_min = 4u << 20;
+    bool dense_for_spatial = std::getenv("GS_L1_DENSE_MIN") == nullptr;
+    bool wants_dense_lists() const { return scene->n >= dense_min || (dense_for_spatial && scene->perm.p); }
     bool debug_levels = std::getenv("GS_DEBUG_LEVELS") != nullptr;
     bool level2_queue = !(std::getenv("GS_L2_QUEUE") && std::atoi(std::getenv("GS_L2_QUEUE")) == 0);
     double stall_ms = std::getenv("GS_DEBUG_STALLS") ? std::atof(std::getenv("GS_DEBUG_STALLS")) : 0.0;
@@ -232,12 +244,13 @@
         if (const char* e = std::getenv("GS_INITIAL_CAND_CAPACITY")) want_cand = std::max<uint64_t>(256, std::strtoull(e, nullptr, 10));
         else if (std::getenv("GS_INITIAL_CAPACITY")) want_cand = std::min<uint64_t>(want_cand, want);
         cand_capacity = static_cast<uint32_t>(std::min<uint64_t>(want_cand, capacity));
-        sets[0].init(scene->n, capacity, cand_capacity, scene->n >= dense_min);
+        default_cand_capacity = cand_capacity;
+        sets[0].init(scene->n, capacity, cand_capacity, wants_dense_lists());
     }
 
     void set_num_sets(int k) {
         for (int i = 0; i < k; ++i)
-            if (!sets[i].ready) sets[i].init(scene->n, capacity, cand_capacity, scene->n >= dense_min);
+            if (!sets[i].ready) sets[i].init(scene->n, capacity, cand_capacity, wants_dense_lists());
         num_sets = k;
     }
 
@@ -301,6 +314,23 @@
                 HIP_CHECK(hipMemset(fb.slabs.p, 0, fb.slabs.n));
             }
         }
+        const bool fused_counters = n != 0 && u.width != 0 && u.height != 0;
+        auto l1_verdict = [&]() {
+            const BinGeometry g = bin_geometry(tx, ty);
+            const int at_level = policy.frame_level();
+            return l1_policy.decide(at_level < kGlobalLevel && g.bin_shift <= 3, n < dense_min, scene->perm.p != nullptr, u.width, u.height,
+                                    g.bin_shift, cand_capacity, g.bins_x * g.bins_y);
+        };
+        if (fused_counters) {
+            const BinGeometry g = bin_geometry(tx, ty);
+            if (l1_policy.grow_to(l1_verdict(), u.width, u.height, g.bin_shift, cand_capacity, g.bins_x * g.bins_y, default_cand_capacity) != 0) {
+                drain();
+                const BinGeometry g2 = bin_geometry(tx, ty);
+                const uint32_t grow = l1_policy.grow_to(l1_verdict(), u.width, u.height, g2.bin_shift, cand_capacity, g2.bins_x * g2.bins_y,
+                                                        default_cand_capacity);
+                if (grow > cand_capacity) set_cand_capacity(grow);
+            }
+        }
         last_set = &fb;
         last_width = u.width;
         last_height = u.height;
@@ -318,19 +348,22 @@
                           scene->sh_half ? scene->sh16.p : nullptr, scene->acut.p, scene->perm.p};
         gs::Counters* cnt = fb.counters.p;
         const bool l1_any_order = bin_local && geo.bin_shift <= 3;
-        const bool dense_list = l1_any_order && n != 0 && n >= dense_min && fb.vis.p && u.width != 0 && u.height != 0;
+        const bool l1_fused = fused_counters && l1_verdict() == L1FusedPolicy::kEngage;
+        const bool dense_list = l1_any_order && !l1_fused && n != 0 && wants_dense_lists() && fb.vis.p && u.width != 0 && u.height != 0;
         gs::AttrView av{fb.tiles.p, fb.depth.p, fb.aabb.p, fb.rec.p, dense_list ? fb.vis.p : nullptr, dense_list ? fb.vis_count.p : nullptr,
                         fb.vis_region_slots};
-        fb.planes_stale = dense_list;
-
-        const bool fused_counters = n != 0 && u.width != 0 && u.height != 0;
+        const uint32_t l1_cap = L1FusedPolicy::region_cap(cand_capacity, geo.bins_x * geo.bins_y);
+        const gs::L1Fused lf{l1_fused ? fb.l1_words.p : nullptr, fb.cand.p, l1_cap, fb.vis_mask.p, tx, ty, geo.bins_x, geo.bins_y, geo.bin_shift, geo.grid_shift};
+        fb.planes_stale = dense_list ? 1 : (l1_fused ? 2 : 0);
+        last_l1_fused = l1_fused;
+
         if (!fused_counters) {
             HIP_CHECK(hipMemsetAsync(cnt, 0, sizeof(gs::Counters), stream));
             HIP_CHECK(hipMemsetAsync(fb.ranges.p, 0, 2 * nt * sizeof(uint32_t), stream));
         }
         uint64_t* const stamps = fb.stamps.p;
         auto passes = [&](const gs::FrameParams* fp) {
-            gs::launch_preprocess(sv, u, av, cnt, fp, stamps, antialiased, stream);
+            gs::launch_preprocess(sv, u, av, cnt, fp, stamps, antialiased, lf, stream);
             lap(3);
             if (!bin_local && n != 0) {
                 const int blocks = std::max(1, std::min<int>(gs::kSortMaxBlocks, (n + gs::kSortTileKeys - 1) / gs::kSortTileKeys));
@@ -379,6 +412,8 @@
                 b.counters = cnt;
                 b.capacity = capacity;
                 b.cand_capacity = cand_capacity;
+                b.l1_fused_words = lf.words;
+                b.l1_fused_cap = l1_cap;
                 b.slabs = fb.slabs.p;
                 b.slab_capacity = fb.slabs.p ? gs::kSlabCapacity : 0u;
                 b.slab_epoch = 0;
@@ -393,15 +428,17 @@
                 b.bin_shift = geo.bin_shift;
                 b.grid_shift = geo.grid_shift;
                 b.stamps = stamps;
-                gs::launch_bin_level1_count(b, stream);
-                gs::launch_bin_level1_scatter(b, l1_any_order, stream);
+                if (!l1_fused) {
+                    gs::launch_bin_level1_count(b, stream);
+                    gs::launch_bin_level1_scatter(b, l1_any_order, stream);
+                }
                 lap(5);
                 gs::launch_bin_level2(b, lv, stream);
             }
             lap(6);
             gs::launch_blend(fb.ranges.p, fb.sorted.p, tile_order.p, av, u.width, u.height, d_rgba, d_bgra, cnt,
                              fused_counters ? sl.h_counters : nullptr, blend_exp_mode(), contract, fp, lockstep, stamps, stream);
-            gs::launch_frame_end(stamps, sl.h_stamps, fp, stream);
+            gs::launch_frame_end(stamps, sl.h_stamps, fp, lf.words, gs::kVisRegions + (1u << (2 * geo.grid_shift)), stream);
             lap(7);
         };
         depth_order = bin_local ? nullptr : fb.dvals[1].p;
@@ -411,7 +448,7 @@
             *sl.h_params = gs::FrameParams{u, d_rgba, d_bgra, sl.h_counters, sl.h_stamps};
             HIP_CHECK(hipMemcpyAsync(fb.params.p, sl.h_params, sizeof(gs::FrameParams), hipMemcpyHostToDevice, stream));
             const FrameBuffers::GraphKey key{lv, geo.bin_shift, blend_exp_mode(), contract ? 1 : 0,
-                                             antialiased, lockstep,
+                                             antialiased, lockstep, l1_fused,
                                              u.width, u.height, capacity, cand_capacity,
                                              tile_order.p, fb.ranges.p, sv.sh16};
             const int gi = lockstep ? 1 : 0;
@@ -443,6 +480,8 @@
         sl.level = lv;
         sl.bin_shift = geo.bin_shift;
         sl.lockstep = lockstep;
+        sl.l1_fused = l1_fused;
+        sl.l1_cap = l1_cap;
         sl.tune_round = tuner.round;
         sl.tune_shape = tune_shape;
         sl.u = u;
@@ -466,6 +505,7 @@
         }
         redo_chain = 0;
         policy.frame_retired(sl.level, sl.h_counters->max_bin, sl.bin_shift);
+        l1_policy.frame_retired(sl.u.width, sl.u.height, sl.bin_shift, sl.h_counters->max_bin, sl.h_counters->bin_entries, sl.h_counters->visible);
         last = frame_stats(sl);
         have_frame = true;
         const float v[7] = {last.ms_preprocess, last.ms_prefix_sum, last.ms_preprocess_sort, last.ms_sort,
@@ -493,6 +533,7 @@
             const gs::Counters& c = *q.h_counters;
             redo.push_back({q.u, q.rgba, q.bgra});
             ran.push_back({q.level, q.bin_shift, q.u.width, q.u.height, c.overflow, c.max_bin});
+            if (q.l1_fused && (c.overflow & 1u) && c.max_bin > q.l1_cap) l1_policy.region_overflowed();
             if (c.overflow & 1u) {
                 if (c.bin_entries > cand_capacity) need_cand = std::max<uint64_t>(need_cand, c.bin_entries);
                 else need = std::max<uint64_t>(need, c.instances);
@@ -555,9 +596,9 @@
         if (sl.timed) st.ms_total = span(gs::ST_PREPROCESS, gs::ST_END);
         if (sl.timed && timing) {
             const bool global = sl.level >= kGlobalLevel;
-            st.ms_preprocess = span(gs::ST_PREPROCESS, global ? gs::ST_ORDER : gs::ST_L1_COUNT);
-            st.ms_prefix_sum = span(gs::ST_L1_COUNT, gs::ST_L1_SCATTER);
-            st.ms_preprocess_sort = span(gs::ST_L1_SCATTER, gs::ST_L2);
+            st.ms_preprocess = span(gs::ST_PREPROCESS, global ? gs::ST_ORDER : (sl.l1_fused ? gs::ST_L2 : gs::ST_L1_COUNT));
+            st.ms_prefix_sum = sl.l1_fused ? 0.0f : span(gs::ST_L1_COUNT, gs::ST_L1_SCATTER);
+            st.ms_preprocess_sort = sl.l1_fused ? 0.0f : span(gs::ST_L1_SCATTER, gs::ST_L2);
             st.ms_sort = (global ? span(gs::ST_ORDER, gs::ST_L1_COUNT) : 0.0f) + span(gs::ST_L2, gs::ST_BLEND);
             st.ms_tile_boundary = 0.0f;
             st.ms_render = span(gs::ST_BLEND, gs::ST_END);
@@ -606,6 +647,7 @@
         r->scene = scene;
         if (const char* e = std::getenv("GS_L1_DENSE_MIN")) r->dense_min = std::strtoull(e, nullptr, 10);
         r->init();
+        if (const char* e = std::getenv("GS_L1_FUSED")) r->l1_policy.mode = std::atoi(e) < 0 ? -1 : (std::atoi(e) != 0 ? 1 : 0);
         if (const char* e = std::getenv("GS_GRAPH")) r->graph_mode = std::atoi(e) != 0;
         if (const char* e = std::getenv("GS_EXP_MODE")) r->exp_mode = std::min(3, std::max(0, std::atoi(e)));
         if (const char* e = std::getenv("GS_BLEND_CONTRACTION")) r->contract = std::atoi(e) != 0;
@@ -811,6 +853,24 @@
     return rc != 0 ? rc : now;
 }
 
+int gs_set_level1_fused(gs_renderer* r, int mode) {
+    return guarded([&] {
+        if (!r) throw Error(GS_ERR_INVALID, "null argument");
+        if (mode < -1 || mode > 1) throw Error(GS_ERR_INVALID, "level-1 fusion: -1 by rule, 0 off, 1 on");
+        r->drain();
+        r->l1_policy.mode = mode;
+    });
+}
+
+int gs_get_level1_fused(gs_renderer* r) {
+    int on = 0;
+    const int rc = guarded([&] {
+        if (!r) throw Error(GS_ERR_INVALID, "null argument");
+        on = r->last_l1_fused ? 1 : 0;
+    });
+    return rc != 0 ? rc : on;
+}
+
 int gs_set_graph_mode(gs_renderer* r, int enabled) {
     return guarded([&] {
         if (!r) throw Error(GS_ERR_INVALID, "renderer is null");
@@ -834,11 +894,12 @@
         uint64_t size = 0;
         if (r->last_set->planes_stale && (stage == GS_STAGE_TILES || stage == GS_STAGE_DEPTH || stage == GS_STAGE_AABB)) {
             FrameBuffers& fb = *r->last_set;
-            gs::launch_vis_to_planes(gs::AttrView{fb.tiles.p, fb.depth.p, fb.aabb.p, fb.rec.p, fb.vis.p, fb.vis_count.p, fb.vis_region_slots},
-                                     static_cast<uint32_t>(n), fb.stream);
+            const gs::AttrView pv{fb.tiles.p, fb.depth.p, fb.aabb.p, fb.rec.p, fb.vis.p, fb.vis_count.p, fb.vis_region_slots};
+            if (fb.planes_stale == 1) gs::launch_vis_to_planes(pv, static_cast<uint32_t>(n), fb.stream);
+            else gs::launch_records_to_planes(fb.vis_mask.p, r->scene->perm.p, pv, static_cast<uint32_t>(n), r->last_width, r->last_height, fb.stream);
             HIP_CHECK(hipGetLastError());
             HIP_CHECK(hipStreamSynchronize(fb.stream));
-            fb.planes_stale = false;
+            fb.planes_stale = 0;
         }
         switch (stage) {
             case GS_STAGE_TILES: src = r->last_set->tiles.p; size = n * 4; break;
diff --git a/3dgs.cpp_amd/csrc/gs_scene_host.cpp b/3dgs.cpp_amd/csrc/gs_scene_host.cpp
--- a/3dgs.cpp_amd/csrc/gs_scene_host.cpp
+++ b/3dgs.cpp_amd/csrc/gs_scene_host.cpp
@@ -41,7 +41,7 @@
     std::fprintf(stderr, "[gs3d] no memory for the scene's copy in spatial order: rendering from the blob as loaded\n");
 }
 void gs_scene::make_spatial_copy() {
-    uint64_t min_n = 4ull << 20;
+    uint64_t min_n = 1ull << 19;
     if (const char* e = std::getenv("GS_SPATIAL_MIN")) min_n = std::strtoull(e, nullptr, 10);
     if (n == 0 || n < min_n) return;
     const size_t st = gs::blob_stride(n);
diff --git a/include/gs3d_hip.h b/include/gs3d_hip.h
--- a/include/gs3d_hip.h
+++ b/include/gs3d_hip.h
@@ -160,6 +160,8 @@
 int gs_set_graph_mode(gs_renderer* r, int enabled);
 int gs_set_blend_lockstep(gs_renderer* r, int mode);
 int gs_get_blend_lockstep(gs_renderer* r, int* settled);
+int gs_set_level1_fused(gs_renderer* r, int mode);
+int gs_get_level1_fused(gs_renderer* r);
 int gs_get_timing_totals(gs_renderer* r, gs_frame_stats* sum, uint64_t* frames, int reset);
 int gs_get_frame_intervals(gs_renderer* r, float* out_ms, uint64_t capacity, uint64_t* n_out, int reset);
 int gs_get_stats(gs_renderer* r, gs_frame_stats* out);
```
